# wdc3iii/legged_gym_dev

Hardware: AMD Instinct MI355X
Metric: env-steps/sec (whole node), ANYmal-C flat 4096 envs per GPU (higher is better)
Workload: dtype f32

## Files before the change

### legged_gym_dev_amd/csrc/ppo_api.hip

```cpp
#include <cstdlib>
#include <cstring>
#include <string>
#include <vector>

#include "ppo_device.h"
#include "ppo_mlp_args.h"
#include "ppo_rnn.h"

void lg_set_error(const std::string &s);

extern "C" {
void ppok_gemm_fwd(const GemmArgs *g, int nz, hipStream_t s);
void ppok_gemm_dx(const GemmArgs *g, int nz, hipStream_t s);
void ppok_sync_planes(const PpoDev *P, hipStream_t s);
int ppok_mlp_fwd(const MlpArgs *g, const PpoDev *P, int mask, hipStream_t s);
int ppok_mlp_supported(const MlpArgs *g);
int64_t ppok_mlp_frag_elems(int K, int N);
void ppok_mlp_frag_build(const MlpArgs *g, hipStream_t s);
void ppok_gemm_dw(const GemmArgs *g, int nz, int splits, hipStream_t s);
void ppok_debug_set_xcd_remap(int v);
void ppok_act_sample(const PpoDev *P, const float *obs, const float *cobs, const float *mu, const float *val, int t,
                     int64_t cnt, int inject, hipStream_t s);
void ppok_process_step(const PpoDev *P, const float *rew, const uint8_t *dones, const uint8_t *tos, int t, hipStream_t s);
void ppok_gae(const PpoDev *P, const float *last_values, hipStream_t s);
void ppok_det_fold(const PpoDev *P, hipStream_t s);
void ppok_adv_normalize(const PpoDev *P, hipStream_t s);
void ppok_gather(const PpoDev *P, int mb, hipStream_t s);
void ppok_randperm(const PpoDev *P, int n, uint64_t update_idx, hipStream_t s);
void ppok_loss(const PpoDev *P, const float *mu, const float *v, float *dmu, float *dval, hipStream_t s);
int ppok_step(const PpoDev *P, int par, const PpoDev *G, int gather_mb, hipStream_t s);
size_t ppok_head_part_floats();
int ppok_head_fused(const PpoDev *P, int H3, const float *xa, const float *xc, float *dza, float *dzc, int64_t w_a, int64_t b_a,
                    int64_t w_c, int64_t b_c, int64_t b_prev_a, int64_t b_prev_c, hipStream_t s);
void ppok_lstm_fwd(const RnnStepArgs *a, int nz, hipStream_t s);
void ppok_lstm_bwd(const RnnBwdArgs *a, int nz, hipStream_t s);
void ppok_lstm_bias_grad(const PpoDev *P, const RnnBiasArgs *a, hipStream_t s);
void ppok_lstm_reset(float *h0, float *c0, float *h1, float *c1, const uint8_t *done, int N, int H, hipStream_t s);
}

struct Rnn {
    int H, mbs;
    int in_dim[2];
    int64_t w_ih[2], w_hh[2], b_ih[2], b_hh[2];
    float *h[2], *c[2];
    float *sv_h[2], *sv_c[2];
    float *tmp_h[2], *tmp_c[2];
    float *pg[2];
    float *hout[2], *cout[2], *hused[2], *cused[2], *dh[2];
    float *gates[2];
    float *dc[2];
};

struct Net {
    int nl;
    int dims[LG_PPO_MAX_LAYERS + 1];
    int64_t w_off[LG_PPO_MAX_LAYERS], b_off[LG_PPO_MAX_LAYERS];
    int64_t pl_off[LG_PPO_MAX_LAYERS];
    int pl_ld0;
    float *act[LG_PPO_MAX_LAYERS + 1];
    float *dz[LG_PPO_MAX_LAYERS + 1];
};

struct lg_comm;
struct lg_ctx;
extern "C" {
void lg_internal_defer_finalize(lg_ctx *c, int on);
hipStream_t lg_internal_stream(lg_ctx *c);
int lg_internal_finalize_pending(lg_ctx *c);
const DevParams *lg_internal_take_finalize(lg_ctx *c, int64_t *counter);
const DevParams *lg_internal_host_params(lg_ctx *c);
int lg_finalize(lg_ctx *c);
hipStream_t lg_comm_stream_(lg_comm *c);
hipEvent_t lg_comm_event_(lg_comm *c);
int lg_comm_group_allreduce_(lg_comm *c, float *const *bufs, const int64_t *counts, int n, hipStream_t s);
int lg_comm_allreduce_sum(lg_comm *c, float *buf, int64_t n, void *stream);
int lg_comm_broadcast(lg_comm *c, float *buf, int64_t n, int root, void *stream);
}

struct lg_ppo {
    lg_comm *comm;
    hipEvent_t ev_bucket;
    int comm_rc;
    int comm_timing;
    std::vector<hipEvent_t> comm_ev;
    size_t comm_ev_used;
    lg_ppo_cfg cfg;
    PpoDev dev;
    Net net[2];
    hipStream_t stream;
    hipStream_t side;
    hipEvent_t ev_dz, ev_side;
    int overlap;
    long long *det_buf;
    int act_code;
    int grads_dirty;
    lg_ctx *env;
    int pp_pending, pp_t, pp_use_tos;
    int params_dirty;
    int fused_act;
    MlpArgs mlp;
    int step, inject;
    int64_t act_count, update_count;
    int Mmax;
    std::vector<void *> allocs;
    int64_t perm_count;
    struct MbSet { float *obs, *critic_obs, *actions, *mu, *scalars; } mbset[2];
    int mb_cur, mb_ready, mb_last;
    lg_ppo_buffers pub;
    Rnn rnn;
};

template <typename T>
static bool palloc(lg_ppo *p, T **out, size_t n) {
    void *q = nullptr;
    size_t bytes = (n ? n : 1) * sizeof(T);
    if (hipMalloc(&q, bytes) != hipSuccess || hipMemset(q, 0, bytes) != hipSuccess) return false;
    p->allocs.push_back(q);
    *out = (T *)q;
    return true;
}
#define PA(ptr, n) do { if (!palloc(p, &(ptr), (n))) { lg_set_error("hipMalloc failed in lg_ppo_create"); lg_ppo_destroy(p); return -100; } } while (0)

static int launch_ok() {
    hipError_t e = hipGetLastError();
    if (e != hipSuccess) { lg_set_error(std::string("ppo kernel launch: ") + hipGetErrorString(e)); return -100; }
    return 0;
}

static void forward(lg_ppo *p, int M, const float *in0, const float *in1, int mask, int skip_head = 0, bool planes = false,
                    bool in_pad = false, hipStream_t on = nullptr, int l_begin = 0, int l_end = 1 << 30) {
    const hipStream_t fs = on ? on : p->stream;
    const float *in[2] = {in0, in1};
    const int in_ld[2] = {in_pad ? p->dev.Op : p->net[0].dims[0], in_pad ? p->dev.OCp : p->net[1].dims[0]};
    int sel[2], nz = 0;
    for (int z = 0; z < 2; ++z) if (mask & (1 << z)) sel[nz++] = z;
    const int nl = p->net[sel[0]].nl;
    for (int l = l_begin; l < nl - skip_head && l < l_end; ++l) {
        GemmArgs g;
        memset(&g, 0, sizeof(g));
        for (int k = 0; k < nz; ++k) {
            Net &n = p->net[sel[k]];
            g.A[k] = l == 0 ? in[sel[k]] : n.act[l];
            g.B[k] = p->dev.params + n.w_off[l];
            g.bias[k] = p->dev.params + n.b_off[l];
            g.Bpl[k] = planes ? p->dev.wpl + n.pl_off[l] : nullptr;
            g.C[k] = n.act[l + 1];
            g.M[k] = M; g.N[k] = n.dims[l + 1]; g.K[k] = n.dims[l];
            g.lda[k] = l == 0 ? in_ld[sel[k]] : n.dims[l]; g.ldb[k] = n.dims[l]; g.ldc[k] = n.dims[l + 1];
            if (l == 0 && in_pad && planes && n.pl_ld0 != n.dims[0]) { g.Kpl[k] = n.pl_ld0; g.ldbpl[k] = n.pl_ld0; }
            else if (l == 0 && n.pl_ld0 != n.dims[0]) g.Bpl[k] = nullptr;
        }
        g.elu = l < nl - 1 ? p->act_code : 0;
        g.pl_stride = p->dev.pl_stride;
        ppok_gemm_fwd(&g, nz, fs);
    }
}

static int bucket_extents(lg_ppo *p, int l, float **bufs, int64_t *counts) {
    int n = 0;
    for (int z = 0; z < 2; ++z) {
        Net &net = p->net[z];
        bufs[n] = p->dev.grads + net.w_off[l];
        counts[n++] = (int64_t)net.dims[l + 1] * net.dims[l] + net.dims[l + 1];
    }
    if (l == p->net[0].nl - 1) {
        bufs[n] = p->dev.grads + p->dev.off_std; counts[n++] = p->cfg.num_actions;
        bufs[n] = p->dev.grads + p->dev.num_params; counts[n++] = 2;
    }
    return n;
}
static void reduce_layer_bucket(lg_ppo *p, int l, hipStream_t ready_on) {
    float *bufs[4];
    int64_t counts[4];
    const int n = bucket_extents(p, l, bufs, counts);
    hipStream_t cs = lg_comm_stream_(p->comm);
    (void)hipEventRecord(p->ev_bucket, ready_on);
    (void)hipStreamWaitEvent(cs, p->ev_bucket, 0);
    const int rc = lg_comm_group_allreduce_(p->comm, bufs, counts, n, cs);
    if (rc && !p->comm_rc) p->comm_rc = rc;
}

static void backward(lg_ppo *p, int M, const float *in0, const float *in1, int skip_head = 0) {
    const float *in[2] = {in0, in1};
    auto det_args = [&](GemmArgs &g) {
        g.det_base = p->dev.grads; g.det64 = p->dev.det64; g.det_n = p->dev.num_params + 2;
    };
    const int nl = p->net[0].nl;
    for (int l = nl - 1 - skip_head; l >= 0; --l) {
        GemmArgs g;
        memset(&g, 0, sizeof(g));
        det_args(g);
        long tiles = 0;
        for (int z = 0; z < 2; ++z) {
            Net &n = p->net[z];
            g.A[z] = n.dz[l + 1]; g.lda[z] = n.dims[l + 1];
            g.B[z] = l == 0 ? in[z] : n.act[l]; g.ldb[z] = n.dims[l];
            g.C[z] = p->dev.grads + n.w_off[l]; g.ldc[z] = n.dims[l];
            g.M[z] = n.dims[l + 1]; g.N[z] = n.dims[l]; g.K[z] = M;
            if (l == 0 && !p->rnn.H) {
                const int ldp = z == 0 ? p->dev.Op : p->dev.OCp;
                g.ldb[z] = ldp;
                if (ldp != n.dims[0]) { g.N[z] = ldp; g.nstore[z] = n.dims[0]; }
            }
            const int tile = (g.M[z] > 64 && g.N[z] > 64) ? 128 : 64;
            long t = (long)((g.M[z] + tile - 1) / tile) * ((g.N[z] + tile - 1) / tile);
            tiles = t > tiles ? t : tiles;
        }
        constexpr int dw_target = 384;
        int splits = (int)((dw_target + tiles - 1) / tiles);
        int max_splits = M / 256 > 0 ? M / 256 : 1;
        if (splits > max_splits) splits = max_splits;
        if (splits >= 8) splits &= ~7;
        if (splits < 1) splits = 1;
        const bool on_side = p->overlap && l > 0;
        hipStream_t dw_stream = on_side ? p->side : p->stream;
        if (on_side) {
            (void)hipEventRecord(p->ev_dz, p->stream);
            (void)hipStreamWaitEvent(p->side, p->ev_dz, 0);
        }
        ppok_gemm_dw(&g, 2, splits, dw_stream);
        if (p->comm) reduce_layer_bucket(p, l, dw_stream);
        if (l > 0) {
            memset(&g, 0, sizeof(g));
            det_args(g);
            for (int z = 0; z < 2; ++z) {
                Net &n = p->net[z];
                g.A[z] = n.dz[l + 1]; g.lda[z] = n.dims[l + 1];
                g.B[z] = p->dev.params + n.w_off[l]; g.ldb[z] = n.dims[l];
                g.Bpl[z] = p->dev.wpl + n.pl_off[l];
                g.C[z] = n.dz[l]; g.ldc[z] = n.dims[l];
                g.aux[z] = n.act[l]; g.ldaux[z] = n.dims[l];
                g.colsum[z] = p->dev.grads + n.b_off[l - 1];
                g.M[z] = M; g.N[z] = n.dims[l]; g.K[z] = n.dims[l + 1];
            }
            g.elu = p->act_code;
            g.pl_stride = p->dev.pl_stride;
            ppok_gemm_dx(&g, 2, p->stream);
        }
    }
    if (p->rnn.H) {
        GemmArgs g;
        memset(&g, 0, sizeof(g));
        for (int z = 0; z < 2; ++z) {
            Net &n = p->net[z];
            g.A[z] = n.dz[1]; g.lda[z] = n.dims[1];
            g.B[z] = p->dev.params + n.w_off[0]; g.ldb[z] = n.dims[0];
            g.Bpl[z] = p->dev.wpl + n.pl_off[0];
            g.C[z] = p->rnn.dh[z]; g.ldc[z] = n.dims[0];
            g.aux[z] = p->rnn.dh[z]; g.ldaux[z] = n.dims[0];
            g.M[z] = M; g.N[z] = n.dims[0]; g.K[z] = n.dims[1];
        }
        g.elu = 0;
        g.pl_stride = p->dev.pl_stride;
        ppok_gemm_dx(&g, 2, p->stream);
    }
    if (p->overlap) {
        (void)hipEventRecord(p->ev_side, p->side);
        (void)hipStreamWaitEvent(p->stream, p->ev_side, 0);
    }
    if (p->comm) {
        const bool rec = p->comm_timing && p->comm_ev_used + 2 <= 2 * 4096;
        if (rec) {
            while (p->comm_ev.size() < p->comm_ev_used + 2) { hipEvent_t e; (void)hipEventCreate(&e); p->comm_ev.push_back(e); }
            (void)hipEventRecord(p->comm_ev[p->comm_ev_used], p->stream);
        }
        (void)hipEventRecord(lg_comm_event_(p->comm), lg_comm_stream_(p->comm));
        (void)hipStreamWaitEvent(p->stream, lg_comm_event_(p->comm), 0);
        if (rec) { (void)hipEventRecord(p->comm_ev[p->comm_ev_used + 1], p->stream); p->comm_ev_used += 2; }
    }
}

static void flush_rollout_epilogue(lg_ppo *p) {
    if (!p->env) return;
    (void)lg_finalize(p->env);
    if (p->pp_pending) {
        const lg_buffers &b = lg_internal_host_params(p->env)->buf;
        ppok_process_step(&p->dev, b.rew, b.reset, p->pp_use_tos ? b.extras_time_outs : nullptr, p->pp_t, p->stream);
        p->pp_pending = 0;
    }
}

static void rnn_net_params(lg_ppo *p, int z, RnnNetArgs &n) {
    const Rnn &q = p->rnn;
    n.Wih = p->dev.params + q.w_ih[z]; n.Whh = p->dev.params + q.w_hh[z];
    n.bih = p->dev.params + q.b_ih[z]; n.bhh = p->dev.params + q.b_hh[z];
}

static void rnn_live_step(lg_ppo *p, int mask, const float *x0, const float *x1, int t) {
    Rnn &q = p->rnn;
    const int N = p->cfg.num_envs, H = q.H;
    RnnStepArgs a;
    memset(&a, 0, sizeof(a));
    a.M = N; a.H = H; a.reload_all = 1;
    const float *x[2] = {x0, x1};
    int nz = 0;
    for (int z = 0; z < 2; ++z) {
        if (!(mask & (1 << z))) continue;
        RnnNetArgs &n = a.n[nz++];
        rnn_net_params(p, z, n);
        n.X = x[z]; n.ldx = q.in_dim[z]; n.K = q.in_dim[z];
        n.h_sv = t >= 0 ? q.sv_h[z] + (size_t)t * N * H : q.tmp_h[z];
        n.c_sv = t >= 0 ? q.sv_c[z] + (size_t)t * N * H : q.tmp_c[z];
        n.h_out = q.h[z]; n.c_out = q.c[z];
    }
    ppok_lstm_fwd(&a, nz, p->stream);
}

static void rnn_stash_live(lg_ppo *p, int mask, int t) {
    Rnn &q = p->rnn;
    const size_t nh = (size_t)p->cfg.num_envs * q.H;
    for (int z = 0; z < 2; ++z) {
        if (!(mask & (1 << z))) continue;
        float *dh = t >= 0 ? q.sv_h[z] + (size_t)t * nh : q.tmp_h[z];
        float *dc = t >= 0 ? q.sv_c[z] + (size_t)t * nh : q.tmp_c[z];
        (void)hipMemcpyAsync(dh, q.h[z], nh * sizeof(float), hipMemcpyDeviceToDevice, p->stream);
        (void)hipMemcpyAsync(dc, q.c[z], nh * sizeof(float), hipMemcpyDeviceToDevice, p->stream);
    }
}

static void rnn_forward_seq(lg_ppo *p, int mb) {
    Rnn &q = p->rnn;
    PpoDev &d = p->dev;
    const int T = d.T, N = d.N, mbs = q.mbs, H = q.H, R = d.mb_rows, e0 = mb * mbs;
    GemmArgs g;
    memset(&g, 0, sizeof(g));
    for (int z = 0; z < 2; ++z) {
        g.A[z] = z ? d.mb_critic_obs : d.mb_obs; g.lda[z] = z ? d.OCp : d.Op;
        g.B[z] = d.params + q.w_ih[z]; g.ldb[z] = q.in_dim[z];
        g.bias[z] = d.params + q.b_ih[z];
        g.C[z] = q.pg[z]; g.ldc[z] = 4 * H;
        g.M[z] = R; g.N[z] = 4 * H; g.K[z] = q.in_dim[z];
    }
    g.elu = 0;
    ppok_gemm_fwd(&g, 2, p->stream);
    for (int t = 0; t < T; ++t) {
        RnnStepArgs a;
        memset(&a, 0, sizeof(a));
        a.M = mbs; a.H = H;
        a.reload_all = t == 0;
        a.reload = t ? d.st_dones + (size_t)(t - 1) * N + e0 : nullptr;
        for (int z = 0; z < 2; ++z) {
            RnnNetArgs &n = a.n[z];
            rnn_net_params(p, z, n);
            const size_t r0 = (size_t)t * mbs, rp = (size_t)(t ? t - 1 : 0) * mbs;
            n.P = q.pg[z] + r0 * 4 * H; n.ldp = 4 * H;
            n.h_prev = t ? q.hout[z] + rp * H : nullptr; n.c_prev = t ? q.cout[z] + rp * H : nullptr;
            n.h_sv = q.sv_h[z] + ((size_t)t * N + e0) * H; n.c_sv = q.sv_c[z] + ((size_t)t * N + e0) * H;
            n.h_out = q.hout[z] + r0 * H; n.c_out = q.cout[z] + r0 * H;
            n.gates = q.gates[z] + r0 * 4 * H;
            n.h_used = q.hused[z] + r0 * H; n.c_used = q.cused[z] + r0 * H;
        }
        ppok_lstm_fwd(&a, 2, p->stream);
    }
}

static void rnn_backward_seq(lg_ppo *p, int mb) {
    Rnn &q = p->rnn;
    PpoDev &d = p->dev;
    const int T = d.T, N = d.N, mbs = q.mbs, H = q.H, R = d.mb_rows, e0 = mb * mbs;
    for (int z = 0; z < 2; ++z) (void)hipMemsetAsync(q.dc[z], 0, (size_t)mbs * H * sizeof(float), p->stream);
    for (int t = T - 1; t >= 0; --t) {
        RnnBwdArgs a;
        memset(&a, 0, sizeof(a));
        a.M = mbs; a.H = H;
        a.cut_next = t < T - 1 ? d.st_dones + (size_t)t * N + e0 : nullptr;
        a.cut = t ? d.st_dones + (size_t)(t - 1) * N + e0 : nullptr;
        a.cut_all = t == 0;
        for (int z = 0; z < 2; ++z) {
            RnnBwdNet &n = a.n[z];
            const size_t r0 = (size_t)t * mbs;
            n.dG_next = t < T - 1 ? q.pg[z] + (r0 + mbs) * 4 * H : nullptr;
            n.Whh = d.params + q.w_hh[z];
            n.dh_mlp = q.dh[z] + r0 * H;
            n.dc = q.dc[z];
            n.gates = q.gates[z] + r0 * 4 * H; n.c_t = q.cout[z] + r0 * H; n.c_used = q.cused[z] + r0 * H;
            n.dG = q.pg[z] + r0 * 4 * H;
        }
        ppok_lstm_bwd(&a, 2, p->stream);
    }
    for (int w = 0; w < 2; ++w) {
        GemmArgs g;
        memset(&g, 0, sizeof(g));
        g.det_base = d.grads; g.det64 = d.det64; g.det_n = d.num_params + 2;
        long tiles = 0;
        for (int z = 0; z < 2; ++z) {
            g.A[z] = q.pg[z]; g.lda[z] = 4 * H;
            g.M[z] = 4 * H; g.K[z] = R;
            if (w == 0) {
                const int ldp = z ? d.OCp : d.Op;
                g.B[z] = z ? d.mb_critic_obs : d.mb_obs; g.ldb[z] = ldp;
                g.C[z] = d.grads + q.w_ih[z]; g.ldc[z] = q.in_dim[z];
                g.N[z] = ldp;
                if (ldp != q.in_dim[z]) g.nstore[z] = q.in_dim[z];
            } else {
                g.B[z] = q.hused[z]; g.ldb[z] = H;
                g.C[z] = d.grads + q.w_hh[z]; g.ldc[z] = H;
                g.N[z] = H;
            }
            const int tile = (g.M[z] > 64 && g.N[z] > 64) ? 128 : 64;
            const long tz = (long)((g.M[z] + tile - 1) / tile) * ((g.N[z] + tile - 1) / tile);
            tiles = tz > tiles ? tz : tiles;
        }
        int splits = (int)((384 + tiles - 1) / tiles);
        const int max_splits = R / 256 > 0 ? R / 256 : 1;
        if (splits > max_splits) splits = max_splits;
        if (splits >= 8) splits &= ~7;
        if (splits < 1) splits = 1;
        ppok_gemm_dw(&g, 2, splits, p->stream);
    }
    RnnBiasArgs b;
    memset(&b, 0, sizeof(b));
    b.M = R; b.H = H;
    for (int z = 0; z < 2; ++z) { b.dG[z] = q.pg[z]; b.db_ih[z] = d.grads + q.b_ih[z]; b.db_hh[z] = d.grads + q.b_hh[z]; }
    ppok_lstm_bias_grad(&d, &b, p->stream);
}

extern "C" {

int lg_ppo_destroy(lg_ppo *p) {
    if (!p) return 0;
    if (p->env) { flush_rollout_epilogue(p); lg_internal_defer_finalize(p->env, 0); p->env = nullptr; }
    if (p->side) { (void)hipStreamSynchronize(p->side); (void)hipStreamDestroy(p->side); }
    if (p->ev_dz) (void)hipEventDestroy(p->ev_dz);
    if (p->ev_side) (void)hipEventDestroy(p->ev_side);
    if (p->ev_bucket) (void)hipEventDestroy(p->ev_bucket);
    for (hipEvent_t e : p->comm_ev) (void)hipEventDestroy(e);
    for (void *q : p->allocs) (void)hipFree(q);
    delete p;
    return 0;
}

static int ppo_create(const lg_ppo_cfg *cfg, const lg_ppo_rnn_cfg *rc, lg_ppo **out) {
    if (!cfg || !out) { lg_set_error("null argument"); return -1; }
    int ndev = 0;
    if (hipGetDeviceCount(&ndev) != hipSuccess || ndev == 0) { lg_set_error("no HIP device: no CPU fallback"); return -2; }
    if (cfg->activation < 0 || cfg->activation > 5) { lg_set_error("activation must be one of 0 elu, 1 selu, 2 relu (also rsl_rl's crelu), 3 lrelu, 4 tanh, 5 sigmoid"); return -3; }
    if (cfg->num_hidden < 1 || cfg->num_hidden > LG_MAX_HIDDEN || cfg->num_actions > LG_PPO_MAX_A) {
        lg_set_error("unsupported network size"); return -4;
    }
    const int N = cfg->num_envs, T = cfg->num_steps, A = cfg->num_actions, O = cfg->num_obs;
    const int OC = cfg->num_critic_obs > 0 ? cfg->num_critic_obs : O;
    if ((long)N * T % cfg->num_mini_batches != 0 && (long)N * T / cfg->num_mini_batches == 0) { lg_set_error("bad minibatch count"); return -5; }
    const int H = rc ? rc->hidden : 0;
    if (rc) {
        if (rc->type != 0) { lg_set_error("recurrent policy: only rnn_type 'lstm' (0) is implemented"); return -6; }
        if (rc->layers != 1) { lg_set_error("recurrent policy: only rnn_num_layers = 1 is implemented"); return -6; }
        if (H < 32 || H > 512 || H % 32) { lg_set_error("recurrent policy: rnn_hidden_size must be a multiple of 32 in [32, 512]"); return -6; }
    }
    lg_ppo *p = new lg_ppo();
    p->cfg = *cfg;
    memset(&p->rnn, 0, sizeof(p->rnn));
    p->stream = nullptr;
    p->act_code = cfg->activation + 1;
    p->fused_act = getenv("LG_FUSED_ACT") ? atoi(getenv("LG_FUSED_ACT")) : 1;
    p->overlap = getenv("LG_PPO_OVERLAP") ? atoi(getenv("LG_PPO_OVERLAP")) : 1;
    if (hipStreamCreateWithFlags(&p->side, hipStreamNonBlocking) != hipSuccess ||
        hipEventCreateWithFlags(&p->ev_dz, hipEventDisableTiming) != hipSuccess ||
        hipEventCreateWithFlags(&p->ev_side, hipEventDisableTiming) != hipSuccess ||
        hipEventCreateWithFlags(&p->ev_bucket, hipEventDisableTiming) != hipSuccess) {
        lg_set_error("stream/event creation failed"); delete p; return -100;
    }
    p->step = 0; p->inject = 0; p->act_count = 0; p->update_count = 0; p->params_dirty = 1;
    p->comm = nullptr; p->comm_rc = 0; p->comm_timing = 0; p->comm_ev_used = 0;
    p->env = nullptr; p->pp_pending = 0;
    if (getenv("LG_XCD_REMAP")) ppok_debug_set_xcd_remap(atoi(getenv("LG_XCD_REMAP")));
    p->perm_count = 0;
    const int R = (int)((long)N * T / cfg->num_mini_batches);
    p->Mmax = R > N ? R : N;

    int64_t off = 0;
    PpoDev &d = p->dev;
    memset(&d, 0, sizeof(d));
    d.off_std = (int)off; off += A;
    for (int z = 0; z < 2; ++z) {
        Net &n = p->net[z];
        n.nl = cfg->num_hidden + 1;
        n.dims[0] = H ? H : z == 0 ? O : OC;
        for (int l = 0; l < cfg->num_hidden; ++l) n.dims[l + 1] = z == 0 ? cfg->actor_hidden[l] : cfg->critic_hidden[l];
        n.dims[n.nl] = z == 0 ? A : 1;
        for (int l = 0; l < n.nl; ++l) {
            n.w_off[l] = off; off += (int64_t)n.dims[l + 1] * n.dims[l];
            n.b_off[l] = off; off += n.dims[l + 1];
        }
    }
    if (H) {
        Rnn &q = p->rnn;
        q.H = H; q.mbs = N / cfg->num_mini_batches;
        for (int z = 0; z < 2; ++z) {
            q.in_dim[z] = z == 0 ? O : OC;
            q.w_ih[z] = off; off += (int64_t)4 * H * q.in_dim[z];
            q.w_hh[z] = off; off += (int64_t)4 * H * H;
            q.b_ih[z] = off; off += 4 * H;
            q.b_hh[z] = off; off += 4 * H;
        }
        p->fused_act = 0;
    }
    d.num_params = off;
    int seg_ld[LG_PPO_MAX_SEG];
    {
        int64_t po = 0;
        d.nseg = 0;
        for (int z = 0; z < 2; ++z)
            for (int l = 0; l < p->net[z].nl; ++l) {
                Net &n = p->net[z];
                n.pl_off[l] = po;
                d.seg_off[d.nseg] = n.w_off[l]; d.seg_pl[d.nseg] = po;
                d.seg_rows[d.nseg] = n.dims[l + 1]; d.seg_cols[d.nseg] = n.dims[l];
                const int ld = l == 0 ? (n.dims[0] + 31) / 32 * 32 : n.dims[l];
                if (l == 0) n.pl_ld0 = ld;
                seg_ld[d.nseg] = ld;
                ++d.nseg;
                po += ((int64_t)n.dims[l + 1] * ld + 7) / 8 * 8;
            }
        d.pl_stride = po;
    }
    d.off_bias_actor_head = (int)p->net[0].b_off[p->net[0].nl - 1];
    d.off_bias_critic_head = (int)p->net[1].b_off[p->net[1].nl - 1];
    d.N = N; d.T = T; d.A = A; d.O = O; d.OC = OC; d.mb_rows = R;
    d.Op = (O + 31) / 32 * 32; d.OCp = (OC + 31) / 32 * 32;
    d.world = cfg->world_size > 0 ? cfg->world_size : 1;
    d.env_offset = 0;
    d.adaptive = cfg->adaptive_schedule; d.clipped_value = cfg->use_clipped_value_loss;
    d.seed = cfg->seed;
    d.gamma = cfg->gamma; d.lam = cfg->lam; d.clip = cfg->clip_param; d.value_coef = cfg->value_loss_coef;
    d.entropy_coef = cfg->entropy_coef; d.desired_kl = cfg->desired_kl; d.max_grad_norm = cfg->max_grad_norm;

    PA(d.params, off + 2); PA(d.grads, off + 2); PA(d.adam_m, off + 2); PA(d.adam_v, off + 2);
    {
        const int64_t pls = d.pl_stride;
        PA(d.wpl, (size_t)3 * pls + 8);
        PA(d.pl_dest, (size_t)off + 2);
        std::vector<int32_t> dest((size_t)off + 2, -1);
        for (int sg = 0; sg < d.nseg; ++sg)
            for (int64_t e = 0; e < (int64_t)d.seg_rows[sg] * d.seg_cols[sg]; ++e)
                dest[d.seg_off[sg] + e] = (int32_t)(d.seg_pl[sg] + (e / d.seg_cols[sg]) * seg_ld[sg] + e % d.seg_cols[sg]);
        (void)hipMemcpy(d.pl_dest, dest.data(), dest.size() * sizeof(int32_t), hipMemcpyHostToDevice);
    }
    const size_t TN = (size_t)T * N;
    PA(d.st_obs, TN * O);
    if (cfg->num_critic_obs > 0) PA(d.st_critic_obs, TN * OC); else d.st_critic_obs = d.st_obs;
    PA(d.st_actions, TN * A); PA(d.st_rewards, TN); PA(d.st_values, TN); PA(d.st_returns, TN); PA(d.st_adv, TN);
    PA(d.st_log_prob, TN); PA(d.st_mu, TN * A); PA(d.st_sigma, A); PA(d.st_dones, TN);
    PA(d.act_actions, (size_t)N * A); PA(d.act_values, N); PA(d.act_log_prob, N); PA(d.act_mu, (size_t)N * A);
    PA(d.stats, 8); PA(d.loss_acc, 4); PA(d.noise, (size_t)N * A); PA(d.perm, TN); PA(d.adv_partial, 4);
    for (int k = 0; k < 2; ++k) {
        lg_ppo::MbSet &m = p->mbset[k];
        PA(m.obs, (size_t)R * d.Op);
        if (cfg->num_critic_obs > 0) PA(m.critic_obs, (size_t)R * d.OCp); else m.critic_obs = m.obs;
        PA(m.actions, (size_t)R * A); PA(m.mu, (size_t)R * A); PA(m.scalars, (size_t)R * 4);
    }
    p->mb_cur = 0; p->mb_ready = -1; p->mb_last = -1;
    d.mb_obs = p->mbset[0].obs; d.mb_critic_obs = p->mbset[0].critic_obs; d.mb_actions = p->mbset[0].actions;
    d.mb_mu = p->mbset[0].mu; d.mb_scalars = p->mbset[0].scalars;
    PA(d.head_part, ppok_head_part_floats());
    PA(d.cur_reward_sum, N); PA(d.cur_episode_len, N); PA(d.ep_stats, 4); PA(d.ep_ring, 200); PA(d.ep_ring_count, 1);
    for (int z = 0; z < 2; ++z) {
        Net &n = p->net[z];
        n.act[0] = nullptr; n.dz[0] = nullptr;
        for (int l = 1; l <= n.nl; ++l) { PA(n.act[l], (size_t)p->Mmax * n.dims[l]); PA(n.dz[l], (size_t)p->Mmax * n.dims[l]); }
    }
    if (H) {
        Rnn &q = p->rnn;
        const size_t NH = (size_t)N * H, Rr = (size_t)R;
        for (int z = 0; z < 2; ++z) {
            PA(q.h[z], NH); PA(q.c[z], NH); PA(q.sv_h[z], TN * H); PA(q.sv_c[z], TN * H); PA(q.tmp_h[z], NH); PA(q.tmp_c[z], NH);
            PA(q.pg[z], Rr * 4 * H); PA(q.gates[z], Rr * 4 * H);
            PA(q.hout[z], Rr * H); PA(q.cout[z], Rr * H); PA(q.hused[z], Rr * H); PA(q.cused[z], Rr * H); PA(q.dh[z], Rr * H);
            PA(q.dc[z], (size_t)q.mbs * H);
        }
        std::vector<int32_t> perm(TN);
        for (int mb = 0; N % cfg->num_mini_batches == 0 && mb < cfg->num_mini_batches; ++mb)
            for (int t = 0; t < T; ++t)
                for (int e = 0; e < q.mbs; ++e) perm[(size_t)mb * R + (size_t)t * q.mbs + e] = (int32_t)((size_t)t * N + (size_t)mb * q.mbs + e);
        (void)hipMemcpy(d.perm, perm.data(), TN * sizeof(int32_t), hipMemcpyHostToDevice);
    }
    if (p->fused_act) {
        MlpArgs &g = p->mlp;
        memset(&g, 0, sizeof(g));
        g.params = d.params; g.M = N; g.nl = p->net[0].nl; g.act = p->act_code;
        int64_t tot = 0;
        if (p->net[0].nl != p->net[1].nl) p->fused_act = 0;
        for (int z = 0; z < 2 && p->fused_act; ++z) {
            Net &n = p->net[z];
            for (int l = 0; l <= n.nl; ++l) g.dims[z][l] = n.dims[l];
            for (int l = 0; l < n.nl; ++l) {
                g.w_off[z][l] = n.w_off[l]; g.b_off[z][l] = n.b_off[l]; g.frag_off[z][l] = tot;
                tot += ppok_mlp_frag_elems(n.dims[l], n.dims[l + 1]);
            }
        }
        if (p->fused_act && ppok_mlp_supported(&g) != 0) p->fused_act = 0;
        if (p->fused_act) { uint16_t *wf = nullptr; PA(wf, (size_t)tot); g.wfrag = wf; }
    }
    {
        std::vector<float> h(A, cfg->init_noise_std);
        (void)hipMemcpy(d.params + d.off_std, h.data(), sizeof(float) * A, hipMemcpyHostToDevice);
        float lr = cfg->learning_rate;
        (void)hipMemcpy(d.stats, &lr, sizeof(float), hipMemcpyHostToDevice);
    }
    lg_ppo_buffers &b = p->pub;
    memset(&b, 0, sizeof(b));
    b.params = d.params; b.grads = d.grads; b.adam_m = d.adam_m; b.adam_v = d.adam_v;
    b.obs = d.st_obs; b.critic_obs = d.st_critic_obs; b.actions = d.st_actions; b.rewards = d.st_rewards;
    b.values = d.st_values; b.returns = d.st_returns; b.advantages = d.st_adv; b.log_prob = d.st_log_prob;
    b.mu = d.st_mu; b.sigma = d.st_sigma; b.dones = d.st_dones;
    b.act_actions = d.act_actions; b.act_values = d.act_values; b.act_log_prob = d.act_log_prob; b.act_mu = d.act_mu;
    b.stats = d.stats; b.noise = d.noise; b.perm = d.perm; b.adv_partial = d.adv_partial;
    b.cur_reward_sum = d.cur_reward_sum; b.cur_episode_len = d.cur_episode_len; b.ep_stats = d.ep_stats;
    b.ep_ring = d.ep_ring; b.ep_ring_count = d.ep_ring_count;
    b.num_params = off; b.num_reduce = off + 2;
    if (hipDeviceSynchronize() != hipSuccess) { lg_set_error("device sync failed in lg_ppo_create"); lg_ppo_destroy(p); return -100; }
    *out = p;
    return 0;
}

int lg_ppo_create(const lg_ppo_cfg *cfg, lg_ppo **out) { return ppo_create(cfg, nullptr, out); }
int lg_ppo_create_recurrent(const lg_ppo_cfg *cfg, const lg_ppo_rnn_cfg *rnn, lg_ppo **out) {
    if (!rnn) { lg_set_error("null argument"); return -1; }
    return ppo_create(cfg, rnn, out);
}
int lg_ppo_get_rnn_buffers(lg_ppo *p, lg_ppo_rnn_buffers *out) {
    if (!p->rnn.H) { lg_set_error("lg_ppo_get_rnn_buffers: not a recurrent learner"); return -15; }
    for (int z = 0; z < 2; ++z) {
        out->h[z] = p->rnn.h[z]; out->c[z] = p->rnn.c[z]; out->saved_h[z] = p->rnn.sv_h[z]; out->saved_c[z] = p->rnn.sv_c[z];
    }
    out->hidden = p->rnn.H;
    return 0;
}
int lg_ppo_reset_hidden(lg_ppo *p, const uint8_t *dones) {
    if (!p->rnn.H) { lg_set_error("lg_ppo_reset_hidden: not a recurrent learner"); return -15; }
    flush_rollout_epilogue(p);
    const Rnn &q = p->rnn;
    ppok_lstm_reset(q.h[0], q.c[0], q.h[1], q.c[1], dones, p->cfg.num_envs, q.H, p->stream);
    return launch_ok();
}
int lg_ppo_get_buffers(lg_ppo *p, lg_ppo_buffers *out) { *out = p->pub; return 0; }
int lg_ppo_set_stream(lg_ppo *p, void *s) { p->stream = (hipStream_t)s; return 0; }
int lg_ppo_inject_noise(lg_ppo *p, int enable) { p->inject = enable; return 0; }
int lg_ppo_debug_set_overlap(lg_ppo *p, int v) { p->overlap = v; return 0; }
int lg_ppo_debug_set_fused_act(lg_ppo *p, int v) { p->fused_act = v && p->mlp.wfrag; return 0; }
int lg_ppo_debug_get_fused_act(lg_ppo *p) { return p->fused_act; }
int lg_ppo_debug_set_act_count(lg_ppo *p, long long v) { p->act_count = v; return 0; }

int lg_ppo_param_layout(lg_ppo *p, int64_t *offsets, int64_t *shapes, int max_entries) {
    int k = 0;
    auto put = [&](int64_t o, int64_t r, int64_t c) {
        if (k < max_entries) { offsets[k] = o; shapes[2 * k] = r; shapes[2 * k + 1] = c; }
        ++k;
    };
    put(p->dev.off_std, p->cfg.num_actions, 0);
    for (int z = 0; z < 2; ++z)
        for (int l = 0; l < p->net[z].nl; ++l) {
            put(p->net[z].w_off[l], p->net[z].dims[l + 1], p->net[z].dims[l]);
            put(p->net[z].b_off[l], p->net[z].dims[l + 1], 0);
        }
    const Rnn &q = p->rnn;
    for (int z = 0; q.H && z < 2; ++z) {
        put(q.w_ih[z], 4 * q.H, q.in_dim[z]);
        put(q.w_hh[z], 4 * q.H, q.H);
        put(q.b_ih[z], 4 * q.H, 0);
        put(q.b_hh[z], 4 * q.H, 0);
    }
    return k;
}

int lg_ppo_attach_env(lg_ppo *p, lg_ctx *env) {
    flush_rollout_epilogue(p);
    if (p->env) lg_internal_defer_finalize(p->env, 0);
    p->env = nullptr;
    if (env) {
        if (lg_internal_host_params(env)->cfg.num_envs != p->cfg.num_envs) { lg_set_error("lg_ppo_attach_env: env and learner differ in num_envs"); return -12; }
        if (lg_internal_stream(env) != p->stream) { lg_set_error("lg_ppo_attach_env: env and learner must run on the same stream (lg_set_stream / lg_ppo_set_stream)"); return -12; }
        p->env = env;
        lg_internal_defer_finalize(env, 1);
    }
    return launch_ok();
}

int lg_ppo_act(lg_ppo *p, const float *obs, const float *critic_obs) {
    if (p->step >= p->cfg.num_steps) { lg_set_error("Rollout buffer overflow"); return -10; }
    const float *cobs = critic_obs ? critic_obs : obs;
    int fused = -1;
    const bool dirty = p->params_dirty != 0 || p->step == 0;
    if (p->fused_act) {
        MlpArgs &g = p->mlp;
        g.in[0] = obs; g.in[1] = cobs;
        g.out[0] = p->net[0].act[p->net[0].nl]; g.out[1] = p->net[1].act[p->net[1].nl];
        if (dirty) ppok_mlp_frag_build(&g, p->stream);
        g.sample = 1; g.t = p->step; g.inject = p->inject; g.act_count = p->act_count;
        g.pp = 0;
        const int N = p->cfg.num_envs;
        const bool fits = (N + 255) / 256 + 1 <= (N + 31) / 32;
        if (p->env && p->pp_pending && fits) {
            g.pp = lg_internal_finalize_pending(p->env) ? 2 : 1;
            g.pp_t = p->pp_t; g.pp_use_tos = p->pp_use_tos;
            g.pp_env = lg_internal_take_finalize(p->env, &g.pp_counter);
            p->pp_pending = 0;
        } else flush_rollout_epilogue(p);
        fused = ppok_mlp_fwd(&g, &p->dev, 3, p->stream);
        if (fused != 0 && g.pp) { lg_set_error("fused act launch refused with a rollout epilogue attached"); return -13; }
        if (fused == 0) {
            p->act_count++;
            const int rc = launch_ok();
            if (rc == 0) p->params_dirty = 0;
            return rc;
        }
    }
    if (!p->fused_act) flush_rollout_epilogue(p);
    if (fused != 0) {
        if (dirty) ppok_sync_planes(&p->dev, p->stream);
        const float *in0 = obs, *in1 = cobs;
        if (p->rnn.H) {
            rnn_stash_live(p, 3, p->step);
            rnn_live_step(p, 3, obs, cobs, p->step);
            in0 = p->rnn.h[0]; in1 = p->rnn.h[1];
        }
        forward(p, p->cfg.num_envs, in0, in1, 3, 0, true);
    }
    ppok_act_sample(&p->dev, obs, cobs, p->net[0].act[p->net[0].nl], p->net[1].act[p->net[1].nl], p->step, p->act_count,
                    p->inject, p->stream);
    p->act_count++;
    const int rc = launch_ok();
    if (rc == 0) p->params_dirty = 0;
    return rc;
}

int lg_ppo_process_env_step(lg_ppo *p, const float *rew, const uint8_t *dones, const uint8_t *time_outs) {
    if (p->step >= p->cfg.num_steps) { lg_set_error("Rollout buffer overflow"); return -10; }
    if (p->env) {
        const lg_buffers &b = lg_internal_host_params(p->env)->buf;
        if (p->fused_act && !p->pp_pending && rew == b.rew && dones == b.reset && (!time_outs || time_outs == b.extras_time_outs)) {
            p->pp_pending = 1; p->pp_t = p->step; p->pp_use_tos = time_outs != nullptr;
            p->step++;
            return 0;
        }
        flush_rollout_epilogue(p);
    }
    ppok_process_step(&p->dev, rew, dones, time_outs, p->step, p->stream);
    if (p->rnn.H) ppok_lstm_reset(p->rnn.h[0], p->rnn.c[0], p->rnn.h[1], p->rnn.c[1], dones, p->cfg.num_envs, p->rnn.H, p->stream);
    p->step++;
    return launch_ok();
}

int lg_ppo_compute_returns(lg_ppo *p, const float *last_critic_obs) {
    flush_rollout_epilogue(p);
    if (p->rnn.H) {
        rnn_stash_live(p, 2, -1);
        rnn_live_step(p, 2, nullptr, last_critic_obs, -1);
        forward(p, p->cfg.num_envs, nullptr, p->rnn.h[1], 2);
    } else
        forward(p, p->cfg.num_envs, nullptr, last_critic_obs, 2);
    ppok_gae(&p->dev, p->net[1].act[p->net[1].nl], p->stream);
    return launch_ok();
}

int lg_ppo_normalize_advantages(lg_ppo *p) {
    ppok_adv_normalize(&p->dev, p->stream);
    return launch_ok();
}

static int rnn_update_refused(const lg_ppo *p) {
    if (!p->rnn.H || p->cfg.num_envs % p->cfg.num_mini_batches == 0) return 0;
    lg_set_error("recurrent policy: the update needs num_envs to be a multiple of num_mini_batches (its minibatches are whole envs)");
    return 1;
}

int lg_ppo_begin_update(lg_ppo *p) {
    if (rnn_update_refused(p)) return -6;
    flush_rollout_epilogue(p);
    const size_t n = (size_t)p->dev.mb_rows * p->cfg.num_mini_batches;
    if (!p->rnn.H) ppok_randperm(&p->dev, (int)n, (uint64_t)p->perm_count++, p->stream);
    p->mb_ready = -1;
    (void)hipMemsetAsync(p->dev.stats + 2, 0, 2 * sizeof(float), p->stream);
    (void)hipMemsetAsync(p->dev.stats + 5, 0, sizeof(float), p->stream);
    (void)hipMemsetAsync(p->dev.loss_acc, 0, 4 * sizeof(float), p->stream);
    p->grads_dirty = 1;
    ppok_sync_planes(&p->dev, p->stream);
    return launch_ok();
}

int lg_ppo_minibatch_backward(lg_ppo *p, int epoch, int mb) {
    (void)epoch;
    if (rnn_update_refused(p)) return -6;
    PpoDev &d = p->dev;
    const int R = d.mb_rows;
    if (p->grads_dirty) (void)hipMemsetAsync(d.grads, 0, (size_t)(d.num_params + 2) * sizeof(float), p->stream);
    p->grads_dirty = 1;
    auto use_set = [&](PpoDev &dev, int k) {
        const lg_ppo::MbSet &m = p->mbset[k];
        dev.mb_obs = m.obs; dev.mb_critic_obs = m.critic_obs; dev.mb_actions = m.actions; dev.mb_mu = m.mu; dev.mb_scalars = m.scalars;
    };
    if (p->mb_ready == mb) {
        p->mb_cur ^= 1;
        use_set(d, p->mb_cur);
    } else {
        ppok_gather(&d, mb, p->stream);
    }
    p->mb_ready = -1;
    p->mb_last = mb;
    Net &na = p->net[0], &nc = p->net[1];
    const int nl = na.nl, H3 = na.dims[nl - 1];
    const bool fuse = p->act_code == 1 && nl >= 2 && nc.dims[nl - 1] == H3 && (H3 == 128 || H3 == 64 || H3 == 32);
    if (p->rnn.H) {
        rnn_forward_seq(p, mb);
        forward(p, R, p->rnn.hout[0], p->rnn.hout[1], 3, fuse ? 1 : 0, true, false);
    } else
        forward(p, R, d.mb_obs, d.mb_critic_obs, 3, fuse ? 1 : 0, true, true);
    if (fuse) {
        ppok_head_fused(&d, H3, na.act[nl - 1], nc.act[nl - 1], na.dz[nl - 1], nc.dz[nl - 1], na.w_off[nl - 1], na.b_off[nl - 1],
                        nc.w_off[nl - 1], nc.b_off[nl - 1], na.b_off[nl - 2], nc.b_off[nl - 2], p->stream);
    } else {
        ppok_loss(&d, na.act[na.nl], nc.act[nc.nl], na.dz[na.nl], nc.dz[nc.nl], p->stream);
    }
    if (fuse && p->comm) reduce_layer_bucket(p, nl - 1, p->stream);
    if (p->rnn.H) {
        backward(p, R, p->rnn.hout[0], p->rnn.hout[1], fuse ? 1 : 0);
        rnn_backward_seq(p, mb);
    } else
        backward(p, R, d.mb_obs, d.mb_critic_obs, fuse ? 1 : 0);
    if (d.det64) ppok_det_fold(&d, p->stream);
    if (p->comm_rc) { const int rc = p->comm_rc; p->comm_rc = 0; return rc; }
    return launch_ok();
}

int lg_ppo_minibatch_step(lg_ppo *p) {
    int next = -1;
    PpoDev other = p->dev;
    if (p->cfg.num_mini_batches > 1 && p->mb_last >= 0) {
        next = (p->mb_last + 1) % p->cfg.num_mini_batches;
        const lg_ppo::MbSet &m = p->mbset[p->mb_cur ^ 1];
        other.mb_obs = m.obs; other.mb_critic_obs = m.critic_obs; other.mb_actions = m.actions; other.mb_mu = m.mu; other.mb_scalars = m.scalars;
    }
    if (ppok_step(&p->dev, (int)(p->update_count & 1), &other, next, p->stream)) p->mb_ready = next;
    p->mb_last = -1;
    p->grads_dirty = 0;
    p->params_dirty = 1;
    p->update_count++;
    return launch_ok();
}

int lg_ppo_end_update(lg_ppo *p) { p->step = 0; return 0; }

int lg_ppo_set_comm(lg_ppo *p, lg_comm *c) {
    if (c && p->rnn.H) { lg_set_error("lg_ppo_set_comm: the per-layer gradient buckets do not cover the LSTM of a recurrent learner; reduce the whole gradient buffer between lg_ppo_minibatch_backward and lg_ppo_minibatch_step instead"); return -14; }
    if (c && p->dev.det64) { lg_set_error("gradient buckets inside the backward pass cannot be combined with deterministic mode"); return -14; }
    p->comm = c;
    return 0;
}
int lg_ppo_comm_timing(lg_ppo *p, int enable) { p->comm_timing = enable ? 1 : 0; return 0; }
int lg_ppo_comm_wait_ms(lg_ppo *p, double *ms_total, int64_t *minibatches) {
    if (!ms_total || !minibatches) { lg_set_error("null argument"); return -1; }
    (void)hipStreamSynchronize(p->stream);
    double sum = 0.0;
    for (size_t k = 0; k + 1 < p->comm_ev_used; k += 2) {
        float ms = 0.f;
        if (hipEventElapsedTime(&ms, p->comm_ev[k], p->comm_ev[k + 1]) == hipSuccess) sum += ms;
    }
    *ms_total = sum; *minibatches = (int64_t)(p->comm_ev_used / 2);
    p->comm_ev_used = 0;
    return 0;
}
int lg_ppo_allreduce_adv_moments(lg_ppo *p, lg_comm *c) { return lg_comm_allreduce_sum(c, p->dev.adv_partial, 4, p->stream); }
int lg_ppo_broadcast_params(lg_ppo *p, lg_comm *c, int root) {
    p->params_dirty = 1;
    return lg_comm_broadcast(c, p->dev.params, p->dev.num_params + 2, root, p->stream);
}
int lg_ppo_params_changed(lg_ppo *p) { p->params_dirty = 1; return 0; }

int lg_ppo_set_deterministic(lg_ppo *p, int on) {
    if (on && p->comm) { lg_set_error("deterministic mode cannot be combined with gradient buckets reduced inside the backward pass (lg_ppo_set_comm)"); return -14; }
    if (on && !p->det_buf) {
        const size_t n = (size_t)p->dev.num_params + 10;
        void *q = nullptr;
        if (hipMalloc(&q, n * sizeof(long long)) != hipSuccess || hipMemset(q, 0, n * sizeof(long long)) != hipSuccess) {
            lg_set_error("hipMalloc failed in lg_ppo_set_deterministic"); return -100;
        }
        p->allocs.push_back(q);
        p->det_buf = (long long *)q;
    }
    if (!on && p->dev.det64) ppok_det_fold(&p->dev, p->stream);
    p->dev.det64 = on ? p->det_buf : nullptr;
    return launch_ok();
}

int lg_ppo_debug_bucket_extents(lg_ppo *p, int l, int64_t *offsets, int64_t *counts) {
    if (l < 0 || l >= p->net[0].nl) return -1;
    float *bufs[4];
    const int n = bucket_extents(p, l, bufs, counts);
    for (int k = 0; k < n; ++k) offsets[k] = bufs[k] - p->dev.grads;
    return n;
}

int lg_ppo_act_inference(lg_ppo *p, const float *obs, float *actions_out, int64_t rows) {
    if (rows > p->Mmax) { lg_set_error("too many rows for act_inference"); return -11; }
    if (p->rnn.H) {
        if (rows != p->cfg.num_envs) { lg_set_error("act_inference of a recurrent learner takes exactly num_envs rows"); return -11; }
        rnn_stash_live(p, 1, -1);
        rnn_live_step(p, 1, obs, nullptr, -1);
        obs = p->rnn.h[0];
    }
    forward(p, (int)rows, obs, nullptr, 1);
    Net &na = p->net[0];
    if (hipMemcpyAsync(actions_out, na.act[na.nl], (size_t)rows * p->cfg.num_actions * sizeof(float), hipMemcpyDeviceToDevice,
                       p->stream) != hipSuccess) { lg_set_error("copy failed"); return -100; }
    return launch_ok();
}

}
```

### legged_gym_dev_amd/csrc/ppo_device.h

```cpp
#pragma once
#include "lg_device.h"

#define LG_PPO_MAX_A 16
#define LG_PPO_MAX_LAYERS (LG_MAX_HIDDEN + 1)

struct GemmArgs {
    const float *A[2], *B[2], *bias[2], *aux[2];
    float *C[2], *colsum[2];
    int M[2], N[2], K[2], lda[2], ldb[2], ldc[2], ldaux[2];
    int elu;
    const uint16_t *Bpl[2];
    int64_t pl_stride;
    int Kpl[2], ldbpl[2];
    int nstore[2];
    const float *det_base;
    long long *det64;
    int64_t det_n;
};

#define LG_PPO_MAX_SEG (2 * LG_PPO_MAX_LAYERS)

struct PpoDev {
    int N, T, A, O, OC, mb_rows, world, env_offset;
    int adaptive, clipped_value;
    uint64_t seed;
    float gamma, lam, clip, value_coef, entropy_coef, desired_kl, max_grad_norm;
    int64_t num_params;
    int off_std, off_bias_actor_head, off_bias_critic_head;
    float *params, *grads, *adam_m, *adam_v;
    float *st_obs, *st_critic_obs, *st_actions, *st_rewards, *st_values, *st_returns, *st_adv, *st_log_prob, *st_mu, *st_sigma;
    uint8_t *st_dones;
    float *act_actions, *act_values, *act_log_prob, *act_mu;
    float *stats;
    float *loss_acc;
    float *noise;
    int32_t *perm;
    float *adv_partial;
    float *mb_obs, *mb_critic_obs, *mb_actions, *mb_mu, *mb_scalars;
    int Op, OCp;
    float *cur_reward_sum, *cur_episode_len, *ep_stats, *ep_ring;
    int32_t *ep_ring_count;
    float *head_part;
    uint16_t *wpl;
    int32_t *pl_dest;
    int64_t pl_stride;
    int nseg;
    int64_t seg_off[LG_PPO_MAX_SEG], seg_pl[LG_PPO_MAX_SEG];
    int seg_rows[LG_PPO_MAX_SEG], seg_cols[LG_PPO_MAX_SEG];
    long long *det64;
};

#define LG_DET_SCALE 1099511627776.0
__device__ __forceinline__ void det_add64(long long *q, float v) {
    atomicAdd(reinterpret_cast<unsigned long long *>(q), (unsigned long long)__double2ll_rn((double)v * LG_DET_SCALE));
}
__device__ __forceinline__ void acc_add(const PpoDev &P, float *p, float v) {
    if (!P.det64) { atomicAdd(p, v); return; }
    long long i;
    if (p >= P.grads && p < P.grads + P.num_params + 2) i = p - P.grads;
    else if (p >= P.loss_acc && p < P.loss_acc + 4) i = P.num_params + 2 + (p - P.loss_acc);
    else i = P.num_params + 6 + (p - P.adv_partial);
    det_add64(P.det64 + i, v);
}
__device__ __forceinline__ void acc_add(const GemmArgs &g, float *p, float v) {
    if (g.det64 && p >= g.det_base && p < g.det_base + g.det_n) det_add64(g.det64 + (p - g.det_base), v);
    else atomicAdd(p, v);
}

__device__ __forceinline__ void process_step_body(const PpoDev &P, float rew, bool done, bool to, int t, int i) {
    float r = rew;
    r += P.gamma * (P.st_values[(size_t)t * P.N + i] * (to ? 1.0f : 0.0f));
    P.st_rewards[(size_t)t * P.N + i] = r;
    P.st_dones[(size_t)t * P.N + i] = done ? 1 : 0;
    const float cr = P.cur_reward_sum[i] + rew, cl = P.cur_episode_len[i] + 1.0f;
    if (done) {
        atomicAdd(&P.ep_stats[0], cr);
        atomicAdd(&P.ep_stats[1], cl);
        atomicAdd(&P.ep_stats[2], 1.0f);
        const int slot = (int)((unsigned)atomicAdd(P.ep_ring_count, 1) % 100u);
        P.ep_ring[slot] = cr;
        P.ep_ring[100 + slot] = cl;
        P.cur_reward_sum[i] = 0.f;
        P.cur_episode_len[i] = 0.f;
    } else {
        P.cur_reward_sum[i] = cr;
        P.cur_episode_len[i] = cl;
    }
}

__device__ __forceinline__ float philox_normal(uint64_t seed, uint32_t env, uint64_t step, uint32_t a) {
    uint32_t c[4] = {env, (uint32_t)step, a, 0x5eedu};
    philox4x32((uint32_t)seed, (uint32_t)(seed >> 32), c);
    float u1 = ((float)(c[0] >> 8) + 1.0f) * (1.0f / 16777216.0f);
    float u2 = (float)(c[1] >> 8) * (1.0f / 16777216.0f);
    return sqrtf(-2.0f * logf(u1)) * cosf(6.283185307179586f * u2);
}
```

### legged_gym_dev_amd/csrc/ppo_kernels.hip

```cpp
#include <cstdlib>
#include <cstring>
#include <type_traits>

#include "ppo_device.h"

typedef float f32x16 __attribute__((ext_vector_type(16)));

#define SELU_L 1.0507009873554804934193349852946f
#define SELU_LA (1.0507009873554804934193349852946f * 1.6732632423543772848170429916717f)
__device__ __forceinline__ float act_fwd(int code, float v) {
    switch (code) {
    case 1: return v > 0.f ? v : __expf(v) - 1.0f;
    case 2: return v > 0.f ? SELU_L * v : SELU_LA * (__expf(v) - 1.0f);
    case 3: return fmaxf(v, 0.f);
    case 4: return v > 0.f ? v : 0.01f * v;
    case 5: return 2.0f * __frcp_rn(1.0f + __expf(-2.0f * v)) - 1.0f;
    case 6: return __frcp_rn(1.0f + __expf(-v));
    default: return v;
    }
}
__device__ __forceinline__ float act_bwd(int code, float a) {
    switch (code) {
    case 1: return a > 0.f ? 1.0f : a + 1.0f;
    case 2: return a > 0.f ? SELU_L : a + SELU_LA;
    case 3: return a > 0.f ? 1.0f : 0.f;
    case 4: return a > 0.f ? 1.0f : 0.01f;
    case 5: return 1.0f - a * a;
    case 6: return a * (1.0f - a);
    default: return 1.0f;
    }
}

static __device__ int g_xcd_remap = 1;
__device__ __forceinline__ void xcd_tile(int lin, int inner, int outer, int &o, int &i) {
    if (g_xcd_remap && (outer & 7) == 0) {
        const int c = lin & 7, j = lin >> 3;
        o = c + 8 * (j / inner);
        i = j % inner;
    } else {
        o = lin / inner;
        i = lin % inner;
    }
}

#define BK 32

template <bool RC, int ROWS, bool VEC, bool KSEQ = false, int NT = 256, bool FULL = false>
__device__ __forceinline__ void stage_load(const float *__restrict__ src, int ld, int row0, int red0, int nrows, int nred,
                                           float4 (&regs)[ROWS * BK / 4 / NT], unsigned &mask) {
    constexpr int NV = ROWS * BK / 4 / NT;
    const int tid = threadIdx.x & (NT - 1);
    const int row_lim = RC ? nrows : nred, col_lim = RC ? nred : nrows;
    mask = 0u;
#pragma unroll
    for (int v = 0; v < NV; ++v) {
        const int idx = tid + v * NT;
        int r, c;
        if (RC) { c = idx & (BK / 4 - 1); r = idx / (BK / 4); }
        else if (KSEQ) { c = tid & (ROWS / 4 - 1); r = NV * (tid / (ROWS / 4)) + v; }
        else { c = idx & (ROWS / 4 - 1); r = idx / (ROWS / 4); }
        const int grow = RC ? row0 + r : red0 + r;
        const int gcol = RC ? red0 + 4 * c : row0 + 4 * c;
        if (FULL) {
            regs[v] = *reinterpret_cast<const float4 *>(src + (size_t)grow * ld + gcol);
            mask = ~0u;
        } else if (VEC) {
            const int rc_ = min(grow, row_lim - 1), cc_ = min(gcol, col_lim - 4);
            regs[v] = *reinterpret_cast<const float4 *>(src + (size_t)rc_ * ld + cc_);
            mask |= (grow < row_lim && gcol < col_lim) ? (1u << v) : 0u;
        } else {
            const int rc_ = min(grow, row_lim - 1);
            const float *p = src + (size_t)rc_ * ld;
            const bool rin = grow < row_lim;
            float e[4];
#pragma unroll
            for (int q = 0; q < 4; ++q) {
                const int cc_ = min(gcol + q, col_lim - 1);
                const float x = p[cc_];
                e[q] = (rin && gcol + q < col_lim) ? x : 0.f;
            }
            regs[v] = make_float4(e[0], e[1], e[2], e[3]);
            mask |= 1u << v;
        }
    }
}
template <bool RC, int ROWS>
__device__ __forceinline__ void stage_store(float *__restrict__ lds, const float4 (&regs_in)[ROWS * BK / 4 / 256], unsigned mask) {
    constexpr int NV = ROWS * BK / 4 / 256;
    const int tid = threadIdx.x;
#pragma unroll
    for (int v = 0; v < NV; ++v) {
        int idx = tid + v * 256;
        const bool in = (mask >> v) & 1u;
        float4 regs[1];
        regs[0] = make_float4(in ? regs_in[v].x : 0.f, in ? regs_in[v].y : 0.f, in ? regs_in[v].z : 0.f, in ? regs_in[v].w : 0.f);
        if (RC) {
            int c = idx & (BK / 4 - 1), r = idx / (BK / 4);
            float *d = lds + r * (BK + 1) + 4 * c;
            d[0] = regs[0].x; d[1] = regs[0].y; d[2] = regs[0].z; d[3] = regs[0].w;
        } else {
            int c = idx & (ROWS / 4 - 1), r = idx / (ROWS / 4);
            *reinterpret_cast<float4 *>(lds + r * (ROWS + 4) + 4 * c) = regs[0];
        }
    }
}
template <bool RC, int ROWS>
__device__ __forceinline__ float frag(const float *__restrict__ lds, int row, int k) {
    return RC ? lds[row * (BK + 1) + k] : lds[k * (ROWS + 4) + row];
}
template <bool RC, int ROWS>
constexpr int tile_floats() { return RC ? ROWS * (BK + 1) : BK * (ROWS + 4); }

template <bool A_RC, bool B_RC, int TM, int TN, bool VEC, bool DBUF>
__device__ __forceinline__ void gemm_mainloop(const float *__restrict__ A, const float *__restrict__ B, int lda, int ldb, int m0, int n0,
                                              int M, int N, int k_begin, int k_end, float *__restrict__ lds, int wm, int wn, int li, int lk,
                                              f32x16 (&acc)[TM][TN]) {
    constexpr int BM = 64 * TM, BN = 64 * TN;
    constexpr int AF = tile_floats<A_RC, BM>(), BF = tile_floats<B_RC, BN>();
    float4 ra[BM * BK / 4 / 256], rb[BN * BK / 4 / 256];
    unsigned ma, mb_;
    stage_load<A_RC, BM, VEC>(A, lda, m0, k_begin, M, k_end, ra, ma);
    stage_load<B_RC, BN, VEC>(B, ldb, n0, k_begin, N, k_end, rb, mb_);
    stage_store<A_RC, BM>(lds, ra, ma);
    stage_store<B_RC, BN>(lds + AF, rb, mb_);
    __syncthreads();
    int cur = 0;
    for (int k0 = k_begin; k0 < k_end; k0 += BK) {
        const bool more = k0 + BK < k_end;
        if (more) {
            stage_load<A_RC, BM, VEC>(A, lda, m0, k0 + BK, M, k_end, ra, ma);
            stage_load<B_RC, BN, VEC>(B, ldb, n0, k0 + BK, N, k_end, rb, mb_);
        }
        const float *as = lds + (DBUF ? cur : 0) * (AF + BF), *bs = as + AF;
        constexpr int GS = 4, NG = BK / 2 / GS;
        float av[2][GS][TM], bv[2][GS][TN];
#pragma unroll
        for (int s = 0; s < GS; ++s) {
#pragma unroll
            for (int a = 0; a < TM; ++a) av[0][s][a] = frag<A_RC, BM>(as, wm + 32 * a + li, 2 * s + lk);
#pragma unroll
            for (int b = 0; b < TN; ++b) bv[0][s][b] = frag<B_RC, BN>(bs, wn + 32 * b + li, 2 * s + lk);
        }
#pragma unroll
        for (int gq = 0; gq < NG; ++gq) {
            if (gq + 1 < NG) {
#pragma unroll
                for (int s = 0; s < GS; ++s) {
                    const int ks = 2 * ((gq + 1) * GS + s) + lk;
#pragma unroll
                    for (int a = 0; a < TM; ++a) av[(gq + 1) & 1][s][a] = frag<A_RC, BM>(as, wm + 32 * a + li, ks);
#pragma unroll
                    for (int b = 0; b < TN; ++b) bv[(gq + 1) & 1][s][b] = frag<B_RC, BN>(bs, wn + 32 * b + li, ks);
                }
            }
#pragma unroll
            for (int s = 0; s < GS; ++s)
#pragma unroll
                for (int a = 0; a < TM; ++a)
#pragma unroll
                    for (int b = 0; b < TN; ++b)
                        acc[a][b] = __builtin_amdgcn_mfma_f32_32x32x2f32(av[gq & 1][s][a], bv[gq & 1][s][b], acc[a][b], 0, 0, 0);
        }
        if (!DBUF) __syncthreads();
        if (more) {
            stage_store<A_RC, BM>(lds + (DBUF ? (cur ^ 1) : 0) * (AF + BF), ra, ma);
            stage_store<B_RC, BN>(lds + (DBUF ? (cur ^ 1) : 0) * (AF + BF) + AF, rb, mb_);
        }
        __syncthreads();
        cur ^= 1;
    }

}


typedef __bf16 bf16x8 __attribute__((ext_vector_type(8)));
#define X6_ROWB 80
__device__ __forceinline__ void lds_barrier() { asm volatile("s_waitcnt lgkmcnt(0)\n\ts_barrier" ::: "memory"); }

__device__ __forceinline__ uint32_t cvt_pk_bf16(float a, float b) {
    uint32_t r;
    asm("v_cvt_pk_bf16_f32 %0, %1, %2" : "=v"(r) : "v"(a), "v"(b));
    return r;
}
__device__ __forceinline__ void split2(float x0, float x1, uint32_t &h, uint32_t &m, uint32_t &l) {
    typedef float f32x2 __attribute__((ext_vector_type(2)));
    h = cvt_pk_bf16(x0, x1);
    f32x2 r = f32x2{x0, x1} - f32x2{__uint_as_float(h << 16), __uint_as_float(h & 0xffff0000u)};
    m = cvt_pk_bf16(r.x, r.y);
    r -= f32x2{__uint_as_float(m << 16), __uint_as_float(m & 0xffff0000u)};
    l = cvt_pk_bf16(r.x, r.y);
}
template <int ROWS>
__device__ __forceinline__ int x6_prow(int r) { return (r & 3) * (ROWS / 4 + 4) + (r >> 2); }
template <int ROWS>
constexpr int x6_plane_bytes() { return (ROWS + 16) * X6_ROWB; }

template <bool RC, int ROWS, int NT, bool FULL = false>
__device__ __forceinline__ void stage_store_x6(unsigned char *__restrict__ lds, const float4 (&regs)[ROWS * BK / 4 / NT], unsigned mask) {
    constexpr int NV = ROWS * BK / 4 / NT;
    constexpr int PL = x6_plane_bytes<ROWS>();
    const int tid = threadIdx.x & (NT - 1);
    if constexpr (RC) {
#pragma unroll
        for (int v = 0; v < NV; ++v) {
            const int idx = tid + v * NT;
            const int c = idx & (BK / 4 - 1), r = idx / (BK / 4);
            const bool in = FULL || ((mask >> v) & 1u);
            const float x0 = in ? regs[v].x : 0.f, x1 = in ? regs[v].y : 0.f, x2 = in ? regs[v].z : 0.f, x3 = in ? regs[v].w : 0.f;
            uint32_t h0, m0, l0, h1, m1, l1;
            split2(x0, x1, h0, m0, l0);
            split2(x2, x3, h1, m1, l1);
            unsigned char *d = lds + x6_prow<ROWS>(r) * X6_ROWB + 8 * c;
            *reinterpret_cast<uint2 *>(d) = make_uint2(h0, h1);
            *reinterpret_cast<uint2 *>(d + PL) = make_uint2(m0, m1);
            *reinterpret_cast<uint2 *>(d + 2 * PL) = make_uint2(l0, l1);
        }
    } else {
        const int c = tid & (ROWS / 4 - 1), kg = tid / (ROWS / 4);
        float e[4][NV];
#pragma unroll
        for (int v = 0; v < NV; ++v) {
            const bool in = FULL || ((mask >> v) & 1u);
            e[0][v] = in ? regs[v].x : 0.f; e[1][v] = in ? regs[v].y : 0.f;
            e[2][v] = in ? regs[v].z : 0.f; e[3][v] = in ? regs[v].w : 0.f;
        }
#pragma unroll
        for (int q = 0; q < 4; ++q) {
            unsigned char *d = lds + (q * (ROWS / 4 + 4) + c) * X6_ROWB + 2 * NV * kg;
            if (NV == 4) {
                uint32_t h0, m0, l0, h1, m1, l1;
                split2(e[q][0], e[q][1], h0, m0, l0);
                split2(e[q][2 % NV], e[q][3 % NV], h1, m1, l1);
                *reinterpret_cast<uint2 *>(d) = make_uint2(h0, h1);
                *reinterpret_cast<uint2 *>(d + PL) = make_uint2(m0, m1);
                *reinterpret_cast<uint2 *>(d + 2 * PL) = make_uint2(l0, l1);
            } else {
                static_assert(NV == 4 || NV == 2, "tile/threads combination");
                uint32_t h0, m0, l0;
                split2(e[q][0], e[q][1 % NV], h0, m0, l0);
                *reinterpret_cast<uint32_t *>(d) = h0;
                *reinterpret_cast<uint32_t *>(d + PL) = m0;
                *reinterpret_cast<uint32_t *>(d + 2 * PL) = l0;
            }
        }
    }
}

template <int ROWS, int NT>
__device__ __forceinline__ void stage_load_pl(const uint16_t *__restrict__ src, int64_t pl_stride, int ld, int row0, int red0, int nrows,
                                              int nred, uint4 (&regs)[ROWS * 12 / NT], unsigned &mask) {
    constexpr int NV = ROWS * 12 / NT;
    mask = 0u;
#pragma unroll
    for (int v = 0; v < NV; ++v) {
        const int c = (threadIdx.x & (NT - 1)) + v * NT;
        const int pl = c / (ROWS * 4), r = (c >> 2) % ROWS, q = c & 3;
        const int grow = row0 + r, gk = red0 + 8 * q;
        const int rc_ = min(grow, nrows - 1), kc_ = min(gk, nred - 8);
        regs[v] = *reinterpret_cast<const uint4 *>(src + pl * pl_stride + (size_t)rc_ * ld + kc_);
        mask |= (grow < nrows && gk < nred) ? (1u << v) : 0u;
    }
}
template <int ROWS, int NT>
__device__ __forceinline__ void stage_store_pl(unsigned char *__restrict__ lds, const uint4 (&regs)[ROWS * 12 / NT], unsigned mask) {
    constexpr int NV = ROWS * 12 / NT;
    constexpr int PL = x6_plane_bytes<ROWS>();
#pragma unroll
    for (int v = 0; v < NV; ++v) {
        const int c = (threadIdx.x & (NT - 1)) + v * NT;
        const int pl = c / (ROWS * 4), r = (c >> 2) % ROWS, q = c & 3;
        const bool in = (mask >> v) & 1u;
        const uint4 x = in ? regs[v] : make_uint4(0u, 0u, 0u, 0u);
        *reinterpret_cast<uint4 *>(lds + pl * PL + x6_prow<ROWS>(r) * X6_ROWB + 16 * q) = x;
    }
}

constexpr int PLT_SUB = 576;
typedef short s16x4 __attribute__((ext_vector_type(4)));
template <int BN>
__device__ __forceinline__ int plt_off(int row, int ch) {
    return (BN / 32 * PLT_SUB) * (row >> 3) + PLT_SUB * (ch >> 2) + 64 * (row & 7) + 16 * ((ch & 3) ^ ((row >> 2) & 3));
}
template <int BN>
constexpr int plt_plane_bytes() { return BK / 8 * (BN / 32) * PLT_SUB; }

template <int BN, int NT>
__device__ __forceinline__ void stage_load_plt(const uint16_t *__restrict__ src, int64_t pl_stride, int ld, int n0, int red0, int ncols,
                                               int nred, uint4 (&regs)[BK * BN / 8 * 3 / NT], unsigned &mask) {
    constexpr int CPR = BN / 8, NV = BK * CPR * 3 / NT;
    mask = 0u;
#pragma unroll
    for (int v = 0; v < NV; ++v) {
        const int c = (threadIdx.x & (NT - 1)) + v * NT;
        const int pl = c / (BK * CPR), k = (c / CPR) % BK, ch = c % CPR;
        const int gk = red0 + k, gn = n0 + 8 * ch;
        const int kc_ = min(gk, nred - 1), nc_ = min(gn, ncols - 8);
        regs[v] = *reinterpret_cast<const uint4 *>(src + pl * pl_stride + (size_t)kc_ * ld + nc_);
        mask |= (gk < nred && gn < ncols) ? (1u << v) : 0u;
    }
}
template <int BN, int NT>
__device__ __forceinline__ void stage_store_plt(unsigned char *__restrict__ lds, const uint4 (&regs)[BK * BN / 8 * 3 / NT], unsigned mask) {
    constexpr int CPR = BN / 8, NV = BK * CPR * 3 / NT;
#pragma unroll
    for (int v = 0; v < NV; ++v) {
        const int c = (threadIdx.x & (NT - 1)) + v * NT;
        const int pl = c / (BK * CPR), k = (c / CPR) % BK, ch = c % CPR;
        const bool in = (mask >> v) & 1u;
        const uint4 x = in ? regs[v] : make_uint4(0u, 0u, 0u, 0u);
        *reinterpret_cast<uint4 *>(lds + pl * plt_plane_bytes<BN>() + plt_off<BN>(k, ch)) = x;
    }
}
__device__ __forceinline__ s16x4 lds_read_tr16(const unsigned char *p) {
    return __builtin_amdgcn_ds_read_tr16_b64_v4i16((s16x4 __attribute__((address_space(3))) *)p);
}

template <bool A_RC, bool B_RC, int TM, int TN, int WGM, int WGN, bool VEC, bool FULL = false, int B_PL = 0>
__device__ __forceinline__ void gemm_mainloop_x6(const float *__restrict__ A, const float *__restrict__ B, int lda, int ldb, int m0, int n0,
                                                 int M, int N, int k_begin, int k_end, unsigned char *__restrict__ lds, int wm, int wn, int li,
                                                 int lk, f32x16 (&acc)[TM][TN], const uint16_t *__restrict__ Bpl = nullptr,
                                                 int64_t pl_stride = 0) {
    constexpr int BM = 32 * TM * WGM, BN = 32 * TN * WGN, NT = 64 * WGM * WGN;
    constexpr int APL = x6_plane_bytes<BM>(), BPL = B_PL == 2 ? plt_plane_bytes<BN>() : x6_plane_bytes<BN>();
    constexpr int NVA = BM * BK / 4 / NT, NVB = BN * BK / 4 / NT;
    constexpr int PD = 2;
    constexpr int NVP = B_PL ? BN * 12 / NT : 1;
    struct Regs { float4 a[NVA], b[NVB]; uint4 p[NVP]; unsigned ma = 0, mb = 0; };
    Regs R[PD];
    unsigned char *lds_b = lds + 3 * APL;
    auto load_tile = [&](Regs &r, int k) {
        stage_load<A_RC, BM, VEC, true, NT, FULL>(A, lda, m0, k, M, k_end, r.a, r.ma);
        if constexpr (B_PL == 2) stage_load_plt<BN, NT>(Bpl, pl_stride, ldb, n0, k, N, k_end, r.p, r.mb);
        else if constexpr (B_PL == 1) stage_load_pl<BN, NT>(Bpl, pl_stride, ldb, n0, k, N, k_end, r.p, r.mb);
        else stage_load<B_RC, BN, VEC, true, NT, FULL>(B, ldb, n0, k, N, k_end, r.b, r.mb);
    };
    auto store_tile = [&](Regs &r) {
        stage_store_x6<A_RC, BM, NT, FULL>(lds, r.a, r.ma);
        if constexpr (B_PL == 2) stage_store_plt<BN, NT>(lds_b, r.p, r.mb);
        else if constexpr (B_PL == 1) stage_store_pl<BN, NT>(lds_b, r.p, r.mb);
        else stage_store_x6<B_RC, BN, NT, FULL>(lds_b, r.b, r.mb);
    };
    load_tile(R[0], k_begin);
#pragma unroll
    for (int d = 1; d < PD; ++d)
        if (k_begin + d * BK < k_end) load_tile(R[d], k_begin + d * BK);
    store_tile(R[0]);
    lds_barrier();
    const unsigned char *fa = lds + x6_prow<BM>(wm + li) * X6_ROWB + 16 * lk;
    const unsigned char *fb = lds_b + x6_prow<BN>(wn + li) * X6_ROWB + 16 * lk;
    const int tg = (threadIdx.x >> 4) & 3, tq = (threadIdx.x >> 2) & 3, tp = threadIdx.x & 3;
    const unsigned char *ft[2];
#pragma unroll
    for (int h = 0; h < 2; ++h)
        ft[h] = lds_b + (BN / 32 * PLT_SUB) * (tg >> 1) + PLT_SUB * (wn / 32) + 64 * (4 * h + tq) +
                16 * ((2 * (tg & 1) + (tp >> 1)) ^ (2 * (tg >> 1) + h)) + 8 * (tp & 1);
    auto read_b = [&](int b, int p, int s) -> bf16x8 {
        if constexpr (B_PL == 2) {
            const int o = PLT_SUB * b + p * BPL + (BN / 32 * PLT_SUB) * 2 * s;
            const s16x4 lo = lds_read_tr16(ft[0] + o), hi = lds_read_tr16(ft[1] + o);
            typedef short s16x8 __attribute__((ext_vector_type(8)));
            const s16x8 v = {lo[0], lo[1], lo[2], lo[3], hi[0], hi[1], hi[2], hi[3]};
            return __builtin_bit_cast(bf16x8, v);
        } else {
            return *reinterpret_cast<const bf16x8 *>(fb + b * 8 * X6_ROWB + p * BPL + s * 32);
        }
    };

    auto body = [&](int k0, Regs &x, Regs &y) {
        if (k0 + PD * BK < k_end) load_tile(y, k0 + PD * BK);
        bf16x8 av[2][TM][3], bv[2][TN][3];
#pragma unroll
        for (int a = 0; a < TM; ++a)
#pragma unroll
            for (int p = 0; p < 3; ++p) av[0][a][p] = *reinterpret_cast<const bf16x8 *>(fa + a * 8 * X6_ROWB + p * APL);
#pragma unroll
        for (int b = 0; b < TN; ++b)
#pragma unroll
            for (int p = 0; p < 3; ++p) bv[0][b][p] = read_b(b, p, 0);
#pragma unroll
        for (int s = 0; s < BK / 16; ++s) {
            if (s + 1 < BK / 16) {
#pragma unroll
                for (int a = 0; a < TM; ++a)
#pragma unroll
                    for (int p = 0; p < 3; ++p)
                        av[(s + 1) & 1][a][p] = *reinterpret_cast<const bf16x8 *>(fa + a * 8 * X6_ROWB + p * APL + (s + 1) * 32);
#pragma unroll
                for (int b = 0; b < TN; ++b)
#pragma unroll
                    for (int p = 0; p < 3; ++p)
                        bv[(s + 1) & 1][b][p] = read_b(b, p, s + 1);
            }
#pragma unroll
            for (int a = 0; a < TM; ++a)
#pragma unroll
                for (int b = 0; b < TN; ++b) {
                    const bf16x8 *x = av[s & 1][a], *y = bv[s & 1][b];
                    f32x16 c = acc[a][b];
                    c = __builtin_amdgcn_mfma_f32_32x32x16_bf16(x[1], y[1], c, 0, 0, 0);
                    c = __builtin_amdgcn_mfma_f32_32x32x16_bf16(x[0], y[2], c, 0, 0, 0);
                    c = __builtin_amdgcn_mfma_f32_32x32x16_bf16(x[2], y[0], c, 0, 0, 0);
                    c = __builtin_amdgcn_mfma_f32_32x32x16_bf16(x[0], y[1], c, 0, 0, 0);
                    c = __builtin_amdgcn_mfma_f32_32x32x16_bf16(x[1], y[0], c, 0, 0, 0);
                    c = __builtin_amdgcn_mfma_f32_32x32x16_bf16(x[0], y[0], c, 0, 0, 0);
                    acc[a][b] = c;
                }
        }
        lds_barrier();
        if (k0 + BK < k_end) store_tile(x);
        lds_barrier();
    };
    for (int k0 = k_begin; k0 < k_end; k0 += PD * BK) {
#pragma unroll
        for (int d = 0; d < PD; ++d)
            if (d == 0 || k0 + d * BK < k_end) body(k0 + d * BK, R[(d + 1) % PD], R[d]);
    }
}

template <int EPI, int TM, int TN, int BM, int BN, int ACT>
__device__ __forceinline__ void gemm_epilogue(const GemmArgs &g, int z, int M, int N, int m0, int n0, int wm, int wn, int li, int lk, int ldc,
                                              f32x16 (&acc)[TM][TN]) {
    float *__restrict__ C = g.C[z];
    const bool interior = (m0 + BM <= M) && (n0 + BN <= N);
    const int elu = g.elu;
    if (interior) {
#pragma unroll
        for (int b = 0; b < TN; ++b) {
            const int n = n0 + wn + 32 * b + li;
            float csum = 0.f;
            const float bias = (EPI == 0 && g.bias[z]) ? g.bias[z][n] : 0.f;
#pragma unroll
            for (int a = 0; a < TM; ++a) {
                const int mb = m0 + wm + 32 * a + 4 * lk;
                float aux[16];
                if (EPI == 1) {
#pragma unroll
                    for (int r = 0; r < 16; ++r)
                        aux[r] = g.aux[z][(size_t)(mb + (r & 3) + 8 * (r >> 2)) * g.ldaux[z] + n];
                }
#pragma unroll
                for (int r = 0; r < 16; ++r) {
                    float *cp = &C[(size_t)(mb + (r & 3) + 8 * (r >> 2)) * ldc + n];
                    float v = acc[a][b][r];
                    if (EPI == 0) {
                        v += bias;
                        v = (ACT == 1 ? (v > 0.f ? v : __expf(v) - 1.0f) : ACT == 0 ? v : act_fwd(elu, v));
                        *cp = v;
                    } else if (EPI == 1) {
                        v *= (ACT == 1 ? (aux[r] > 0.f ? 1.0f : aux[r] + 1.0f) : ACT == 0 ? 1.0f : act_bwd(elu, aux[r]));
                        *cp = v;
                        csum += v;
                    } else {
                        acc_add(g, cp, v);
                    }
                }
            }
            if (EPI == 1 && g.colsum[z]) {
                csum += __shfl_xor(csum, 32);
                if (lk == 0) acc_add(g, &g.colsum[z][n], csum);
            }
        }
        return;
    }
#pragma unroll
    for (int b = 0; b < TN; ++b) {
        const int n = n0 + wn + 32 * b + li;
        float csum = 0.f;
        const float bias = (EPI == 0 && g.bias[z] && n < N) ? g.bias[z][n] : 0.f;
#pragma unroll
        for (int a = 0; a < TM; ++a)
#pragma unroll
            for (int r = 0; r < 16; ++r) {
                const int m = m0 + wm + 32 * a + (r & 3) + 8 * (r >> 2) + 4 * lk;
                if (m < M && n < N) {
                    float v = acc[a][b][r];
                    if (EPI == 0) {
                        v += bias;
                        v = (ACT == 1 ? (v > 0.f ? v : __expf(v) - 1.0f) : ACT == 0 ? v : act_fwd(elu, v));
                        C[(size_t)m * ldc + n] = v;
                    } else if (EPI == 1) {
                        const float act = g.aux[z][(size_t)m * g.ldaux[z] + n];
                        v *= (ACT == 1 ? (act > 0.f ? 1.0f : act + 1.0f) : ACT == 0 ? 1.0f : act_bwd(elu, act));
                        C[(size_t)m * ldc + n] = v;
                        csum += v;
                    } else {
                        acc_add(g, &C[(size_t)m * ldc + n], v);
                    }
                }
            }
        if (EPI == 1 && g.colsum[z]) {
            csum += __shfl_xor(csum, 32);
            if (lk == 0 && n < N) acc_add(g, &g.colsum[z][n], csum);
        }
    }
}

template <bool A_RC, bool B_RC, int EPI, int TM, int TN, bool DBUF, bool X6 = false, int WGM = 2, int WGN = 2, int B_PL = 0>
__global__ void __launch_bounds__(64 * WGM * WGN, X6 ? (WGM * WGN == 8 ? 4 : 2) : 1) k_gemm(GemmArgs g) {
    static_assert(B_PL == 0 || (X6 && (B_PL == 1) == B_RC), "weight planes feed the split-bf16 mainloop: [n][k] planes as the reduction-"
                  "contiguous operand (1), the same planes read along their rows through the transposing LDS read (2)");
    constexpr int BM = 32 * TM * WGM, BN = 32 * TN * WGN;
    static_assert(X6 || (WGM == 2 && WGN == 2), "the fp32-input mainloop is written for 2x2 waves");
    const int z = blockIdx.z;
    const int M = g.M[z], N = g.N[z], K = g.K[z];
    const int tiles_n = (N + BN - 1) / BN, tiles_m = (M + BM - 1) / BM;
    if ((int)blockIdx.x >= tiles_n * tiles_m) return;
    int tm, tn;
    if (EPI == 2) { tm = blockIdx.x / tiles_n; tn = blockIdx.x % tiles_n; }
    else xcd_tile((int)blockIdx.x, tiles_n, tiles_m, tm, tn);
    const int m0 = tm * BM, n0 = tn * BN;
    int k_begin = 0, k_end = K;
    if (EPI == 2) {
        int per = ((K + gridDim.y - 1) / gridDim.y + BK - 1) / BK * BK;
        k_begin = blockIdx.y * per;
        k_end = min(K, k_begin + per);
        if (k_begin >= k_end) return;
    }
    const float *__restrict__ A = g.A[z];
    const float *__restrict__ B = g.B[z];
    const int lda = g.lda[z], ldb = g.ldb[z], ldc = g.ldc[z];
    const bool a_vec = (lda & 3) == 0 && ((uintptr_t)A & 15) == 0 && (((A_RC ? k_end : M) & 3) == 0) && (A_RC ? k_end : M) >= 4;
    const bool b_vec = (ldb & 3) == 0 && ((uintptr_t)B & 15) == 0 && (((B_RC ? k_end : N) & 3) == 0) && (B_RC ? k_end : N) >= 4;

    constexpr int AF = tile_floats<A_RC, BM>(), BF = tile_floats<B_RC, BN>();
    constexpr int LDS_BYTES = X6 ? 3 * (x6_plane_bytes<BM>() + (B_PL == 2 ? plt_plane_bytes<BN>() : x6_plane_bytes<BN>()))
                                 : (DBUF ? 2 : 1) * (AF + BF) * 4;
    __shared__ __attribute__((aligned(16))) unsigned char lds_raw[LDS_BYTES];
    float *lds = reinterpret_cast<float *>(lds_raw);

    const int wave = threadIdx.x >> 6, lane = threadIdx.x & 63;
    const int wm = (wave / WGN) * 32 * TM, wn = (wave % WGN) * 32 * TN;
    const int li = lane & 31, lk = lane >> 5;

    f32x16 acc[TM][TN];
#pragma unroll
    for (int a = 0; a < TM; ++a)
#pragma unroll
        for (int b = 0; b < TN; ++b)
#pragma unroll
            for (int r = 0; r < 16; ++r) acc[a][b][r] = 0.f;

    if (X6) {
        const bool full = a_vec && b_vec && m0 + BM <= M && n0 + BN <= N && ((k_end - k_begin) % BK) == 0;
        if (B_PL) {
            const bool fullp = a_vec && m0 + BM <= M && n0 + BN <= N && ((k_end - k_begin) % BK) == 0;
            if (fullp) gemm_mainloop_x6<A_RC, B_RC, TM, TN, WGM, WGN, true, true, B_PL>(A, B, lda, ldb, m0, n0, M, N, k_begin, k_end, lds_raw, wm, wn, li, lk, acc, g.Bpl[z], g.pl_stride);
            else if (a_vec) gemm_mainloop_x6<A_RC, B_RC, TM, TN, WGM, WGN, true, false, B_PL>(A, B, lda, ldb, m0, n0, M, N, k_begin, k_end, lds_raw, wm, wn, li, lk, acc, g.Bpl[z], g.pl_stride);
            else gemm_mainloop_x6<A_RC, B_RC, TM, TN, WGM, WGN, false, false, B_PL>(A, B, lda, ldb, m0, n0, M, N, k_begin, k_end, lds_raw, wm, wn, li, lk, acc, g.Bpl[z], g.pl_stride);
        } else
        if (full) gemm_mainloop_x6<A_RC, B_RC, TM, TN, WGM, WGN, true, true>(A, B, lda, ldb, m0, n0, M, N, k_begin, k_end, lds_raw, wm, wn, li, lk, acc);
        else if (a_vec && b_vec) gemm_mainloop_x6<A_RC, B_RC, TM, TN, WGM, WGN, true>(A, B, lda, ldb, m0, n0, M, N, k_begin, k_end, lds_raw, wm, wn, li, lk, acc);
        else gemm_mainloop_x6<A_RC, B_RC, TM, TN, WGM, WGN, false>(A, B, lda, ldb, m0, n0, M, N, k_begin, k_end, lds_raw, wm, wn, li, lk, acc);
    } else {
        if (a_vec && b_vec) gemm_mainloop<A_RC, B_RC, TM, TN, true, DBUF>(A, B, lda, ldb, m0, n0, M, N, k_begin, k_end, lds, wm, wn, li, lk, acc);
        else gemm_mainloop<A_RC, B_RC, TM, TN, false, DBUF>(A, B, lda, ldb, m0, n0, M, N, k_begin, k_end, lds, wm, wn, li, lk, acc);
    }

    if (EPI == 2 || g.elu == 1) gemm_epilogue<EPI, TM, TN, BM, BN, 1>(g, z, M, N, m0, n0, wm, wn, li, lk, ldc, acc);
    else if (g.elu == 0) gemm_epilogue<EPI, TM, TN, BM, BN, 0>(g, z, M, N, m0, n0, wm, wn, li, lk, ldc, acc);
    else gemm_epilogue<EPI, TM, TN, BM, BN, -1>(g, z, M, N, m0, n0, wm, wn, li, lk, ldc, acc);
}

template <int ROWS, int NT>
__device__ __forceinline__ void stage_store_x6t(unsigned char *__restrict__ lds, const float4 (&regs)[ROWS * BK / 4 / NT], unsigned mask) {
    constexpr int NV = ROWS * BK / 4 / NT, PL = plt_plane_bytes<ROWS>();
#pragma unroll
    for (int v = 0; v < NV; ++v) {
        const int idx = threadIdx.x + v * NT;
        const int c = idx & (ROWS / 4 - 1), r = idx / (ROWS / 4);
        const bool in = (mask >> v) & 1u;
        const float x0 = in ? regs[v].x : 0.f, x1 = in ? regs[v].y : 0.f, x2 = in ? regs[v].z : 0.f, x3 = in ? regs[v].w : 0.f;
        uint32_t h0, m0, l0, h1, m1, l1;
        split2(x0, x1, h0, m0, l0);
        split2(x2, x3, h1, m1, l1);
        unsigned char *d = lds + plt_off<ROWS>(r, c >> 1) + 8 * (c & 1);
        *reinterpret_cast<uint2 *>(d) = make_uint2(h0, h1);
        *reinterpret_cast<uint2 *>(d + PL) = make_uint2(m0, m1);
        *reinterpret_cast<uint2 *>(d + 2 * PL) = make_uint2(l0, l1);
    }
}

template <int TM, int TN, int WGM, int WGN, int PD = 2>
__global__ void __launch_bounds__(64 * WGM * WGN, WGM * WGN == 8 ? 4 : 2) k_gemm_dw_t(GemmArgs g) {
    constexpr int BM = 32 * TM * WGM, BN = 32 * TN * WGN, NT = 64 * WGM * WGN;
    constexpr int APL = plt_plane_bytes<BM>(), BPL = plt_plane_bytes<BN>();
    constexpr int NVA = BM * BK / 4 / NT, NVB = BN * BK / 4 / NT;
    const int z = blockIdx.z;
    const int M = g.M[z], N = g.N[z], K = g.K[z];
    const int tiles_n = (N + BN - 1) / BN, tiles_m = (M + BM - 1) / BM;
    if ((int)blockIdx.x >= tiles_n * tiles_m) return;
    int slice, tile;
    xcd_tile((int)(blockIdx.x + gridDim.x * blockIdx.y), (int)gridDim.x, (int)gridDim.y, slice, tile);
    const int m0 = (tile / tiles_n) * BM, n0 = (tile % tiles_n) * BN;
    const int per = ((K + gridDim.y - 1) / gridDim.y + BK - 1) / BK * BK;
    const int k_begin = slice * per, k_end = min(K, k_begin + per);
    if (k_begin >= k_end) return;
    const float *__restrict__ A = g.A[z];
    const float *__restrict__ B = g.B[z];
    const int lda = g.lda[z], ldb = g.ldb[z], ldc = g.ldc[z];
    __shared__ __attribute__((aligned(16))) unsigned char lds[3 * (APL + BPL)];
    unsigned char *lds_b = lds + 3 * APL;
    const int wave = threadIdx.x >> 6, lane = threadIdx.x & 63;
    const int wm = (wave / WGN) * 32 * TM, wn = (wave % WGN) * 32 * TN;
    const int li = lane & 31, lk = lane >> 5;
    f32x16 acc[TM][TN];
#pragma unroll
    for (int a = 0; a < TM; ++a)
#pragma unroll
        for (int b = 0; b < TN; ++b)
#pragma unroll
            for (int r = 0; r < 16; ++r) acc[a][b][r] = 0.f;
    const int tg = (threadIdx.x >> 4) & 3, tq = (threadIdx.x >> 2) & 3, tp = threadIdx.x & 3;
    const unsigned char *fa[2], *fb[2];
#pragma unroll
    for (int h = 0; h < 2; ++h) {
        const int lane_off = 64 * (4 * h + tq) + 16 * ((2 * (tg & 1) + (tp >> 1)) ^ (2 * (tg >> 1) + h)) + 8 * (tp & 1);
        fa[h] = lds + (BM / 32 * PLT_SUB) * (tg >> 1) + PLT_SUB * (wm / 32) + lane_off;
        fb[h] = lds_b + (BN / 32 * PLT_SUB) * (tg >> 1) + PLT_SUB * (wn / 32) + lane_off;
    }
    auto frag = [&](const unsigned char *const (&f)[2], int o) -> bf16x8 {
        const s16x4 lo = lds_read_tr16(f[0] + o), hi = lds_read_tr16(f[1] + o);
        typedef short s16x8 __attribute__((ext_vector_type(8)));
        const s16x8 v = {lo[0], lo[1], lo[2], lo[3], hi[0], hi[1], hi[2], hi[3]};
        return __builtin_bit_cast(bf16x8, v);
    };
    const bool a_vec = (lda & 3) == 0 && ((uintptr_t)A & 15) == 0 && (M & 3) == 0 && M >= 4;
    const bool b_vec = (ldb & 3) == 0 && ((uintptr_t)B & 15) == 0 && (N & 3) == 0 && N >= 4;
    auto run = [&](auto vec) {
        constexpr bool VEC = decltype(vec)::value;
        float4 ra[PD][NVA], rb[PD][NVB];
        unsigned ma[PD], mb[PD];
    #pragma unroll
        for (int d = 0; d < PD; ++d) { ma[d] = 0u; mb[d] = 0u; }
        auto load = [&](int k0, float4 (&xa)[NVA], float4 (&xb)[NVB], unsigned &xma, unsigned &xmb) {
            stage_load<false, BM, VEC, false, NT>(A, lda, m0, k0, M, k_end, xa, xma);
            stage_load<false, BN, VEC, false, NT>(B, ldb, n0, k0, N, k_end, xb, xmb);
        };
    #pragma unroll
        for (int d = 0; d < PD; ++d)
            if (d == 0 || k_begin + d * BK < k_end) load(k_begin + d * BK, ra[d], rb[d], ma[d], mb[d]);
        stage_store_x6t<BM, NT>(lds, ra[0], ma[0]);
        stage_store_x6t<BN, NT>(lds_b, rb[0], mb[0]);
        lds_barrier();
        auto body = [&](int k0, float4 (&ca)[NVA], float4 (&cb)[NVB], unsigned &cma, unsigned &cmb, float4 (&na)[NVA], float4 (&nb)[NVB],
                        unsigned &nma, unsigned &nmb) {
            if (k0 + PD * BK < k_end) load(k0 + PD * BK, ca, cb, cma, cmb);
    #pragma unroll
            for (int s = 0; s < BK / 16; ++s) {
                bf16x8 av[TM][3], bv[TN][3];
    #pragma unroll
                for (int a = 0; a < TM; ++a)
    #pragma unroll
                    for (int p = 0; p < 3; ++p) av[a][p] = frag(fa, PLT_SUB * a + p * APL + (BM / 32 * PLT_SUB) * 2 * s);
    #pragma unroll
                for (int b = 0; b < TN; ++b)
    #pragma unroll
                    for (int p = 0; p < 3; ++p) bv[b][p] = frag(fb, PLT_SUB * b + p * BPL + (BN / 32 * PLT_SUB) * 2 * s);
    #pragma unroll
                for (int a = 0; a < TM; ++a)
    #pragma unroll
                    for (int b = 0; b < TN; ++b) {
                        const bf16x8 *x = av[a], *y = bv[b];
                        f32x16 c = acc[a][b];
                        c = __builtin_amdgcn_mfma_f32_32x32x16_bf16(x[1], y[1], c, 0, 0, 0);
                        c = __builtin_amdgcn_mfma_f32_32x32x16_bf16(x[0], y[2], c, 0, 0, 0);
                        c = __builtin_amdgcn_mfma_f32_32x32x16_bf16(x[2], y[0], c, 0, 0, 0);
                        c = __builtin_amdgcn_mfma_f32_32x32x16_bf16(x[0], y[1], c, 0, 0, 0);
                        c = __builtin_amdgcn_mfma_f32_32x32x16_bf16(x[1], y[0], c, 0, 0, 0);
                        c = __builtin_amdgcn_mfma_f32_32x32x16_bf16(x[0], y[0], c, 0, 0, 0);
                        acc[a][b] = c;
                    }
            }
            lds_barrier();
            if (k0 + BK < k_end) {
                stage_store_x6t<BM, NT>(lds, na, nma);
                stage_store_x6t<BN, NT>(lds_b, nb, nmb);
            }
            lds_barrier();
        };
        for (int k0 = k_begin; k0 < k_end; k0 += PD * BK) {
    #pragma unroll
            for (int d = 0; d < PD; ++d)
                if (d == 0 || k0 + d * BK < k_end)
                    body(k0 + d * BK, ra[d], rb[d], ma[d], mb[d], ra[(d + 1) % PD], rb[(d + 1) % PD], ma[(d + 1) % PD], mb[(d + 1) % PD]);
        }
    };
    if (a_vec && b_vec) run(std::true_type{});
    else run(std::false_type{});
    gemm_epilogue<2, TM, TN, BM, BN, 1>(g, z, M, g.nstore[z] ? g.nstore[z] : N, m0, n0, wm, wn, li, lk, ldc, acc);
}

extern "C" void ppok_debug_set_xcd_remap(int v) { (void)hipMemcpyToSymbol(HIP_SYMBOL(g_xcd_remap), &v, sizeof(int)); }
static int g_gemm_x6 = 1;
extern "C" void ppok_debug_set_x6(int v) { g_gemm_x6 = v != 0; }

#include "ppo_gemm_glds.h"

template <int EPI, bool B_RC = true, int PL = 1>
static void launch_gemm_pl(const GemmArgs &g, int nz, hipStream_t s) {
    int maxM = 0, maxN = 0;
    for (int z = 0; z < nz; ++z) { maxM = g.M[z] > maxM ? g.M[z] : maxM; maxN = g.N[z] > maxN ? g.N[z] : maxN; }
    if constexpr (EPI == 0) {
        if (maxM > 64 && glds_ok<PL>(g, nz)) {
            dim3 grid((unsigned)(((maxM + GLDS_BM - 1) / GLDS_BM) * (maxN / GLDS_BN)), 1, nz);
            hipLaunchKernelGGL((k_gemm_glds<EPI, PL>), grid, dim3(256), 0, s, g);
            return;
        }
    }
    const long big_tiles = (long)((maxM + 127) / 128) * ((maxN + 127) / 128);
    if (big_tiles >= 192 && maxN > 64 && maxM > 64) {
        dim3 grid((unsigned)big_tiles, 1, nz);
        hipLaunchKernelGGL((k_gemm<true, B_RC, EPI, 2, 1, false, true, 2, 4, PL>), grid, dim3(512), 0, s, g);
    } else {
        dim3 grid((unsigned)(((maxM + 63) / 64) * ((maxN + 63) / 64)), 1, nz);
        hipLaunchKernelGGL((k_gemm<true, B_RC, EPI, 1, 1, false, true, 2, 2, PL>), grid, dim3(256), 0, s, g);
    }
}
static bool planes_ok(const GemmArgs &g, int nz) {
    if (!g_gemm_x6) return false;
    for (int z = 0; z < nz; ++z)
        if (!g.Bpl[z] || (g.ldb[z] & 7) || (g.K[z] & 7) || g.K[z] < 8 || ((uintptr_t)g.Bpl[z] & 15) || (g.pl_stride & 7)) return false;
    return true;
}

template <bool A_RC, bool B_RC, int EPI, bool X6>
static void launch_gemm(const GemmArgs &g, int nz, int splits, hipStream_t s) {
    int maxM = 0, maxN = 0;
    for (int z = 0; z < nz; ++z) { maxM = g.M[z] > maxM ? g.M[z] : maxM; maxN = g.N[z] > maxN ? g.N[z] : maxN; }
    const long big_tiles = (long)((maxM + 127) / 128) * ((maxN + 127) / 128);
    if (big_tiles * splits >= 192 && maxN > 64 && maxM > 64) {
        dim3 grid((unsigned)big_tiles, splits, nz);
        if constexpr (X6) hipLaunchKernelGGL((k_gemm<A_RC, B_RC, EPI, 2, 1, false, true, 2, 4>), grid, dim3(512), 0, s, g);
        else hipLaunchKernelGGL((k_gemm<A_RC, B_RC, EPI, 2, 2, false>), grid, dim3(256), 0, s, g);
    } else {
        dim3 grid((unsigned)(((maxM + 63) / 64) * ((maxN + 63) / 64)), splits, nz);
        if constexpr (X6) hipLaunchKernelGGL((k_gemm<A_RC, B_RC, EPI, 1, 1, false, true>), grid, dim3(256), 0, s, g);
        else hipLaunchKernelGGL((k_gemm<A_RC, B_RC, EPI, 1, 1, true>), grid, dim3(256), 0, s, g);
    }
}
static bool planes_t_ok(const GemmArgs &g, int nz) {
    if (!g_gemm_x6) return false;
    for (int z = 0; z < nz; ++z)
        if (!g.Bpl[z] || (g.ldb[z] & 7) || (g.N[z] & 7) || g.N[z] < 8 || ((uintptr_t)g.Bpl[z] & 15) || (g.pl_stride & 7)) return false;
    return true;
}
extern "C" void ppok_gemm_fwd(const GemmArgs *g, int nz, hipStream_t s) {
    GemmArgs gp = *g;
    for (int z = 0; z < nz; ++z) {
        if (g->Kpl[z]) gp.K[z] = g->Kpl[z];
        if (g->ldbpl[z]) gp.ldb[z] = g->ldbpl[z];
    }
    if (planes_ok(gp, nz)) launch_gemm_pl<0>(gp, nz, s);
    else if (g_gemm_x6) launch_gemm<true, true, 0, true>(*g, nz, 1, s);
    else launch_gemm<true, true, 0, false>(*g, nz, 1, s);
}
extern "C" void ppok_gemm_dx(const GemmArgs *g, int nz, hipStream_t s) {
    if (planes_t_ok(*g, nz)) launch_gemm_pl<1, false, 2>(*g, nz, s);
    else if (g_gemm_x6) launch_gemm<true, false, 1, true>(*g, nz, 1, s);
    else launch_gemm<true, false, 1, false>(*g, nz, 1, s);
}
extern "C" void ppok_gemm_dw(const GemmArgs *g, int nz, int splits, hipStream_t s) {
    if (!g_gemm_x6) {
        GemmArgs gt = *g;
        for (int z = 0; z < nz; ++z) if (g->nstore[z]) gt.N[z] = g->nstore[z];
        launch_gemm<false, false, 2, false>(gt, nz, splits, s);
        return;
    }
    int maxM = 0, maxN = 0;
    for (int z = 0; z < nz; ++z) { maxM = g->M[z] > maxM ? g->M[z] : maxM; maxN = g->N[z] > maxN ? g->N[z] : maxN; }
    const long big_tiles = (long)((maxM + 127) / 128) * ((maxN + 127) / 128);
    if (big_tiles * splits >= 192 && maxN > 64 && maxM > 64) {
        hipLaunchKernelGGL((k_gemm_dw_t<2, 1, 2, 4>), dim3((unsigned)big_tiles, splits, nz), dim3(512), 0, s, *g);
    } else {
        const unsigned tiles = ((maxM + 63) / 64) * ((maxN + 63) / 64);
        hipLaunchKernelGGL((k_gemm_dw_t<1, 1, 2, 2>), dim3(tiles, splits, nz), dim3(256), 0, s, *g);
    }
}

__global__ void k_act_sample(PpoDev P, const float *__restrict__ obs, const float *__restrict__ critic_obs,
                             const float *__restrict__ mu, const float *__restrict__ val, int t, int64_t act_count, int inject) {
    const int i = blockIdx.x * blockDim.x + threadIdx.x;
    const int N = P.N, A = P.A, O = P.O;
    if (t >= 0) {
        const size_t tot = (size_t)N * O, step = (size_t)gridDim.x * blockDim.x;
        for (size_t k = i; k < tot; k += step) P.st_obs[(size_t)t * tot + k] = obs[k];
        if (P.st_critic_obs != P.st_obs) {
            const size_t totc = (size_t)N * P.OC;
            for (size_t k = i; k < totc; k += step) P.st_critic_obs[(size_t)t * totc + k] = critic_obs[k];
        }
    }
    const float *std = P.params + P.off_std;
    if (i < A && t == 0) P.st_sigma[i] = std[i];
    if (i >= N) return;
    float lp = 0.f;
    for (int a = 0; a < A; ++a) {
        float m = mu[(size_t)i * A + a], s = std[a];
        float z = inject ? P.noise[(size_t)i * A + a] : philox_normal(P.seed, (uint32_t)(P.env_offset + i), (uint64_t)act_count, a);
        float act = m + s * z;
        lp += -((act - m) * (act - m)) / (2.0f * s * s) - logf(s) - 0.9189385332046727f;
        P.act_actions[(size_t)i * A + a] = act;
        P.act_mu[(size_t)i * A + a] = m;
        if (t >= 0) {
            P.st_actions[((size_t)t * N + i) * A + a] = act;
            P.st_mu[((size_t)t * N + i) * A + a] = m;
        }
    }
    const float v = val[i];
    P.act_values[i] = v;
    P.act_log_prob[i] = lp;
    if (t >= 0) {
        P.st_values[(size_t)t * N + i] = v;
        P.st_log_prob[(size_t)t * N + i] = lp;
    }
}

__global__ void k_process_step(PpoDev P, const float *__restrict__ rew, const uint8_t *__restrict__ dones,
                               const uint8_t *__restrict__ time_outs, int t) {
    const int i = blockIdx.x * blockDim.x + threadIdx.x;
    if (i >= P.N) return;
    process_step_body(P, rew[i], dones[i] != 0, time_outs && time_outs[i], t, i);
}

__global__ void __launch_bounds__(256) k_gae(PpoDev P, const float *__restrict__ last_values) {
    const int i = blockIdx.x * blockDim.x + threadIdx.x;
    const int N = P.N, T = P.T;
    float s1 = 0.f, s2 = 0.f;
    if (i < N) {
        float adv = 0.f, next_v = last_values[i];
        for (int t = T - 1; t >= 0; --t) {
            const size_t k = (size_t)t * N + i;
            const float nnt = 1.0f - (P.st_dones[k] ? 1.0f : 0.0f);
            const float v = P.st_values[k];
            const float delta = P.st_rewards[k] + nnt * P.gamma * next_v - v;
            adv = delta + nnt * P.gamma * P.lam * adv;
            const float ret = adv + v;
            P.st_returns[k] = ret;
            const float a = ret - v;
            P.st_adv[k] = a;
            s1 += a; s2 += a * a;
            next_v = v;
        }
    }
    __shared__ float r1[256], r2[256];
    r1[threadIdx.x] = s1; r2[threadIdx.x] = s2;
    __syncthreads();
    for (int w = 128; w > 0; w >>= 1) {
        if ((int)threadIdx.x < w) { r1[threadIdx.x] += r1[threadIdx.x + w]; r2[threadIdx.x] += r2[threadIdx.x + w]; }
        __syncthreads();
    }
    if (threadIdx.x == 0) {
        acc_add(P, &P.adv_partial[0], r1[0]);
        acc_add(P, &P.adv_partial[1], r2[0]);
        if (blockIdx.x == 0) P.adv_partial[2] = (float)((size_t)N * T);
    }
}
__global__ void k_adv_normalize(PpoDev P) {
    const size_t n = (size_t)P.N * P.T;
    const float cnt = P.adv_partial[2], mean = P.adv_partial[0] / cnt;
    const float var = fmaxf((P.adv_partial[1] - cnt * mean * mean) / fmaxf(cnt - 1.0f, 1.0f), 0.f);
    const float inv = 1.0f / (sqrtf(var) + 1e-8f);
    for (size_t k = blockIdx.x * (size_t)blockDim.x + threadIdx.x; k < n; k += (size_t)gridDim.x * blockDim.x)
        P.st_adv[k] = (P.st_adv[k] - mean) * inv;
    if (blockIdx.x == 0 && threadIdx.x == 0) { P.stats[6] = mean; P.stats[7] = sqrtf(var); }
}

__global__ void __launch_bounds__(256) k_randperm(PpoDev P, int n, int half_bits, uint64_t update_idx) {
    const int i = blockIdx.x * 256 + threadIdx.x;
    if (i >= n) return;
    const uint32_t mask = (1u << half_bits) - 1u;
    uint32_t x = (uint32_t)i;
    do {
        uint32_t l = x >> half_bits, r = x & mask;
#pragma unroll 1
        for (int round = 0; round < 6; ++round) {
            uint32_t c[4] = {r, (uint32_t)round, (uint32_t)update_idx, (uint32_t)(update_idx >> 32) ^ 0x9e3779b9u};
            philox4x32((uint32_t)P.seed, (uint32_t)(P.seed >> 32), c);
            const uint32_t t = l ^ (c[0] & mask);
            l = r; r = t;
        }
        x = (l << half_bits) | r;
    } while (x >= (uint32_t)n);
    P.perm[i] = (int32_t)x;
}

__global__ void k_gather(PpoDev P, int mb) {
    const int R = P.mb_rows, A = P.A, O = P.O;
    const int r = blockIdx.x;
    if (r >= R) return;
    const int src = P.perm[(size_t)mb * R + r];
    for (int k = threadIdx.x; k < O; k += blockDim.x) P.mb_obs[(size_t)r * P.Op + k] = P.st_obs[(size_t)src * O + k];
    if (P.st_critic_obs != P.st_obs)
        for (int k = threadIdx.x; k < P.OC; k += blockDim.x) P.mb_critic_obs[(size_t)r * P.OCp + k] = P.st_critic_obs[(size_t)src * P.OC + k];
    if ((int)threadIdx.x < A) {
        P.mb_actions[(size_t)r * A + threadIdx.x] = P.st_actions[(size_t)src * A + threadIdx.x];
        P.mb_mu[(size_t)r * A + threadIdx.x] = P.st_mu[(size_t)src * A + threadIdx.x];
    }
    if (threadIdx.x == 0) {
        P.mb_scalars[(size_t)r * 4 + 0] = P.st_values[src];
        P.mb_scalars[(size_t)r * 4 + 1] = P.st_returns[src];
        P.mb_scalars[(size_t)r * 4 + 2] = P.st_adv[src];
        P.mb_scalars[(size_t)r * 4 + 3] = P.st_log_prob[src];
    }
}

__device__ __forceinline__ void gather4_block(const PpoDev &P, int mb, int vblock) {
    const int R = P.mb_rows, A4 = P.A / 4;
    const int gid = vblock * 256 + threadIdx.x;
    const int r = gid >> 5, j = gid & 31;
    if (r >= R) return;
    const int src = P.perm[(size_t)mb * R + r];
    const bool own_critic = P.st_critic_obs != P.st_obs;
    const int O4 = (P.O & 3) ? 0 : P.O / 4, OC4 = (own_critic && !(P.OC & 3)) ? P.OC / 4 : 0;
    auto row_copy = [&](const float *__restrict__ from, float *__restrict__ to, int n) {
        for (int k0 = j; k0 < n; k0 += 256) {
            float v[8];
#pragma unroll
            for (int u = 0; u < 8; ++u) v[u] = from[min(k0 + 32 * u, n - 1)];
#pragma unroll
            for (int u = 0; u < 8; ++u)
                if (k0 + 32 * u < n) to[k0 + 32 * u] = v[u];
        }
    };
    if (P.O & 3) row_copy(P.st_obs + (size_t)src * P.O, P.mb_obs + (size_t)r * P.Op, P.O);
    if (own_critic && (P.OC & 3)) row_copy(P.st_critic_obs + (size_t)src * P.OC, P.mb_critic_obs + (size_t)r * P.OCp, P.OC);
    for (int k = j; k < O4 + OC4 + 2 * A4 + 1; k += 32) {
        if (k < O4) reinterpret_cast<float4 *>(P.mb_obs)[(size_t)r * (P.Op / 4) + k] = reinterpret_cast<const float4 *>(P.st_obs)[(size_t)src * O4 + k];
        else if (k < O4 + OC4) reinterpret_cast<float4 *>(P.mb_critic_obs)[(size_t)r * (P.OCp / 4) + (k - O4)] = reinterpret_cast<const float4 *>(P.st_critic_obs)[(size_t)src * OC4 + (k - O4)];
        else if (k < O4 + OC4 + A4) reinterpret_cast<float4 *>(P.mb_actions)[(size_t)r * A4 + (k - O4 - OC4)] = reinterpret_cast<const float4 *>(P.st_actions)[(size_t)src * A4 + (k - O4 - OC4)];
        else if (k < O4 + OC4 + 2 * A4) reinterpret_cast<float4 *>(P.mb_mu)[(size_t)r * A4 + (k - O4 - OC4 - A4)] = reinterpret_cast<const float4 *>(P.st_mu)[(size_t)src * A4 + (k - O4 - OC4 - A4)];
        else reinterpret_cast<float4 *>(P.mb_scalars)[r] = make_float4(P.st_values[src], P.st_returns[src], P.st_adv[src], P.st_log_prob[src]);
    }
}
__global__ void __launch_bounds__(256) k_gather4(PpoDev P, int mb) { gather4_block(P, mb, blockIdx.x); }

__global__ void __launch_bounds__(256) k_loss(PpoDev P, const float *__restrict__ mu_new, const float *__restrict__ v_new,
                                              float *__restrict__ dmu, float *__restrict__ dval) {
    const int R = P.mb_rows, A = P.A;
    const int r = blockIdx.x * blockDim.x + threadIdx.x;
    const float *std = P.params + P.off_std;
    const float invR = 1.0f / (float)R;
    constexpr int MA = LG_PPO_MAX_A;
    float part[2 * MA + 4];
#pragma unroll
    for (int k = 0; k < 2 * MA + 4; ++k) part[k] = 0.f;
    __shared__ float s_logs[MA], s_logr[MA];
    if ((int)threadIdx.x < A) {
        const float s = std[threadIdx.x], so = P.st_sigma[threadIdx.x];
        s_logs[threadIdx.x] = logf(s);
        s_logr[threadIdx.x] = logf(s / so + 1.e-5f);
    }
    __syncthreads();
    if (r < R) {
        const float4 sc = reinterpret_cast<const float4 *>(P.mb_scalars)[r];
        const float v_old = sc.x, ret = sc.y, adv = sc.z, lp_old = sc.w;
        float lp = 0.f, kl = 0.f, dd[MA];
#pragma unroll
        for (int a = 0; a < MA; ++a) {
            dd[a] = 0.f;
            if (a < A) {
                const float s = std[a], so = P.st_sigma[a];
                const float m = mu_new[(size_t)r * A + a], mo = P.mb_mu[(size_t)r * A + a];
                const float d = P.mb_actions[(size_t)r * A + a] - m;
                dd[a] = d;
                lp += -(d * d) / (2.0f * s * s) - s_logs[a] - 0.9189385332046727f;
                kl += s_logr[a] + (so * so + (mo - m) * (mo - m)) / (2.0f * s * s) - 0.5f;
            }
        }
        const float ratio = expf(lp - lp_old);
        const float rc = fminf(fmaxf(ratio, 1.0f - P.clip), 1.0f + P.clip);
        const float s1 = -adv * ratio, s2 = -adv * rc;
        const float dl_dlp = (s1 >= s2 ? -adv : 0.0f) * ratio * invR;
#pragma unroll
        for (int a = 0; a < MA; ++a)
            if (a < A) {
                const float s = std[a], d = dd[a];
                const float g = dl_dlp * d / (s * s);
                dmu[(size_t)r * A + a] = g;
                part[MA + a] = g;
                part[a] = dl_dlp * (d * d / (s * s * s) - 1.0f / s) - P.entropy_coef * invR / s;
            }
        const float v = v_new[r];
        float lv, dv;
        if (P.clipped_value) {
            const float dvv = v - v_old;
            const float vc = v_old + fminf(fmaxf(dvv, -P.clip), P.clip);
            const float l1 = (v - ret) * (v - ret), l2 = (vc - ret) * (vc - ret);
            const float inside = (dvv >= -P.clip && dvv <= P.clip) ? 1.0f : 0.0f;
            lv = fmaxf(l1, l2);
            if (l1 > l2) dv = 2.0f * (v - ret);
            else if (l1 < l2) dv = 2.0f * (vc - ret) * inside;
            else dv = (v - ret) + (vc - ret) * inside;
        } else {
            lv = (ret - v) * (ret - v);
            dv = 2.0f * (v - ret);
        }
        dv *= P.value_coef * invR;
        dval[r] = dv;
        part[2 * MA] = dv;
        part[2 * MA + 1] = kl;
        part[2 * MA + 2] = lv;
        part[2 * MA + 3] = fmaxf(s1, s2);
    }
    __shared__ float red[4][2 * MA + 4];
#pragma unroll
    for (int k = 0; k < 2 * MA + 4; ++k) {
        if (k >= 2 * MA || (k % MA) < A) {
            float v = part[k];
#pragma unroll
            for (int m = 32; m > 0; m >>= 1) v += __shfl_xor(v, m);
            if ((threadIdx.x & 63) == 0) red[threadIdx.x >> 6][k] = v;
        }
    }
    __syncthreads();
    const int k = threadIdx.x;
    if (k < 2 * MA + 4 && (k >= 2 * MA || (k % MA) < A)) {
        const float v = ((red[0][k] + red[1][k]) + red[2][k]) + red[3][k];
        if (k < MA) acc_add(P, &P.grads[P.off_std + k], v);
        else if (k < 2 * MA) acc_add(P, &P.grads[P.off_bias_actor_head + (k - MA)], v);
        else if (k == 2 * MA) acc_add(P, &P.grads[P.off_bias_critic_head], v);
        else if (k == 2 * MA + 1) acc_add(P, &P.grads[P.num_params], v);
        else if (k == 2 * MA + 2) acc_add(P, &P.loss_acc[0], v);
        else acc_add(P, &P.loss_acc[1], v);
    }
}

#define HEAD_ROWS 64
#define HEAD_GRID 192
#define HEAD_NET_GRID 384
#define HEAD_PART_STRIDE(H3) ((LG_PPO_MAX_A + 1) * (H3) + 2 * LG_PPO_MAX_A + 4)
template <int H3>
__global__ void __launch_bounds__(256) k_head_fused(PpoDev P, const float *__restrict__ xa_g, const float *__restrict__ xc_g,
                                                    float *__restrict__ dza_g, float *__restrict__ dzc_g, int64_t w_a, int64_t b_a,
                                                    int64_t w_c, int64_t b_c, int64_t b_prev_a, int64_t b_prev_c) {
    constexpr int MA = LG_PPO_MAX_A, LDX = H3 + 1, NH = 256 / H3;
    const int R = P.mb_rows, A = P.A, tid = threadIdx.x;
    __shared__ float xa[HEAD_ROWS * LDX], xc[HEAD_ROWS * LDX];
    __shared__ float wa[MA * H3], wc[H3];
    __shared__ float mus[HEAD_ROWS][MA + 1], dmus[HEAD_ROWS][MA + 1];
    __shared__ float red[2 * MA + 4], s_so2[MA], s_i2s2[MA], s_is2[MA], s_is[MA], s_lgs[MA], s_klc[MA];
    if (tid < MA) {
        const float sg = tid < A ? P.params[P.off_std + tid] : 1.f, so = tid < A ? P.st_sigma[tid] : 1.f;
        s_so2[tid] = so * so; s_i2s2[tid] = 1.0f / (2.0f * sg * sg); s_is2[tid] = 1.0f / (sg * sg); s_is[tid] = 1.0f / sg;
        s_lgs[tid] = logf(sg) + 0.9189385332046727f; s_klc[tid] = logf(sg / so + 1.e-5f) - 0.5f;
    }
    for (int i = tid; i < A * H3; i += 256) wa[i] = P.params[w_a + i];
    for (int i = tid; i < H3; i += 256) wc[i] = P.params[w_c + i];
    if (tid < 2 * MA + 4) red[tid] = 0.f;
    const int c = tid % H3, half = tid / H3;
    float dwa[MA], dwc = 0.f, dba = 0.f, dbc = 0.f, part[2 * MA + 4];
#pragma unroll
    for (int a = 0; a < MA; ++a) dwa[a] = 0.f;
#pragma unroll
    for (int k = 0; k < 2 * MA + 4; ++k) part[k] = 0.f;
    const int ntiles = (R + HEAD_ROWS - 1) / HEAD_ROWS;
    for (int tile = blockIdx.x; tile < ntiles; tile += gridDim.x) {
        const int r0 = tile * HEAD_ROWS;
        __syncthreads();
        {
            constexpr int NV = HEAD_ROWS * H3 / 4 / 256;
            float4 va[NV], vc[NV];
#pragma unroll
            for (int v = 0; v < NV; ++v) {
                const int i = tid + v * 256, r = i / (H3 / 4), c4 = i % (H3 / 4);
                const size_t row = (size_t)min(r0 + r, R - 1);
                va[v] = *reinterpret_cast<const float4 *>(xa_g + row * H3 + 4 * c4);
                vc[v] = *reinterpret_cast<const float4 *>(xc_g + row * H3 + 4 * c4);
            }
            __builtin_amdgcn_sched_barrier(0);
#pragma unroll
            for (int v = 0; v < NV; ++v) {
                const int i = tid + v * 256, r = i / (H3 / 4), c4 = i % (H3 / 4);
                float *da = xa + r * LDX + 4 * c4, *dc = xc + r * LDX + 4 * c4;
                da[0] = va[v].x; da[1] = va[v].y; da[2] = va[v].z; da[3] = va[v].w;
                dc[0] = vc[v].x; dc[1] = vc[v].y; dc[2] = vc[v].z; dc[3] = vc[v].w;
            }
        }
        __syncthreads();
        {
            const int r = tid & 63, w = tid >> 6;
            const float *x = xa + r * LDX;
            float o0 = 0.f, o1 = 0.f, o2 = 0.f, o3 = 0.f;
            const float *w0 = wa + (w < A ? w : 0) * H3, *w1 = wa + (w + 4 < A ? w + 4 : 0) * H3;
            const float *w2 = wa + (w + 8 < A ? w + 8 : 0) * H3, *w3 = wa + (w + 12 < A ? w + 12 : 0) * H3;
#pragma unroll 8
            for (int k = 0; k < H3; ++k) {
                const float xv = x[k];
                o0 += xv * w0[k]; o1 += xv * w1[k]; o2 += xv * w2[k]; o3 += xv * w3[k];
            }
            if (w < A) mus[r][w] = o0 + P.params[b_a + w];
            if (w + 4 < A) mus[r][w + 4] = o1 + P.params[b_a + w + 4];
            if (w + 8 < A) mus[r][w + 8] = o2 + P.params[b_a + w + 8];
            if (w + 12 < A) mus[r][w + 12] = o3 + P.params[b_a + w + 12];
            if (w == 3) {
                float sacc = P.params[b_c];
                const float *y = xc + r * LDX;
#pragma unroll 8
                for (int k = 0; k < H3; ++k) sacc += y[k] * wc[k];
                mus[r][MA] = sacc;
            }
        }
        __syncthreads();
        if (tid < HEAD_ROWS) {
            const int r = r0 + tid;
            const float invR = 1.0f / (float)R;
            float dvl = 0.f;
#pragma unroll
            for (int a = 0; a < MA; ++a) dmus[tid][a] = 0.f;
            const size_t rr = (size_t)min(r, R - 1);
            const float4 sc = reinterpret_cast<const float4 *>(P.mb_scalars)[rr];
            float act_r[MA], mo_r[MA];
#pragma unroll
            for (int a = 0; a < MA; ++a) {
                const int ac = min(a, A - 1);
                act_r[a] = P.mb_actions[rr * A + ac];
                mo_r[a] = P.mb_mu[rr * A + ac];
            }
            if (r < R) {
                const float v_old = sc.x, ret = sc.y, adv = sc.z, lp_old = sc.w;
                float lp = 0.f, kl = 0.f, dd[MA];
#pragma unroll
                for (int a = 0; a < MA; ++a) {
                    dd[a] = 0.f;
                    if (a < A) {
                        const float m = mus[tid][a], mo = mo_r[a];
                        const float d = act_r[a] - m;
                        dd[a] = d;
                        lp += -(d * d) * s_i2s2[a] - s_lgs[a];
                        kl += s_klc[a] + (s_so2[a] + (mo - m) * (mo - m)) * s_i2s2[a];
                    }
                }
                const float ratio = expf(lp - lp_old);
                const float rc = fminf(fmaxf(ratio, 1.0f - P.clip), 1.0f + P.clip);
                const float s1 = -adv * ratio, s2 = -adv * rc;
                const float dl_dlp = (s1 >= s2 ? -adv : 0.0f) * ratio * invR;
#pragma unroll
                for (int a = 0; a < MA; ++a)
                    if (a < A) {
                        const float d = dd[a];
                        const float g = dl_dlp * d * s_is2[a];
                        dmus[tid][a] = g;
                        part[MA + a] += g;
                        part[a] += dl_dlp * (d * d * s_is2[a] * s_is[a] - s_is[a]) - P.entropy_coef * invR * s_is[a];
                    }
                const float v = mus[tid][MA];
                float lv, dv;
                if (P.clipped_value) {
                    const float dvv = v - v_old;
                    const float vc = v_old + fminf(fmaxf(dvv, -P.clip), P.clip);
                    const float l1 = (v - ret) * (v - ret), l2 = (vc - ret) * (vc - ret);
                    const float inside = (dvv >= -P.clip && dvv <= P.clip) ? 1.0f : 0.0f;
                    lv = fmaxf(l1, l2);
                    if (l1 > l2) dv = 2.0f * (v - ret);
                    else if (l1 < l2) dv = 2.0f * (vc - ret) * inside;
                    else dv = (v - ret) + (vc - ret) * inside;
                } else {
                    lv = (ret - v) * (ret - v);
                    dv = 2.0f * (v - ret);
                }
                dvl = dv * P.value_coef * invR;
                part[2 * MA] += dvl;
                part[2 * MA + 1] += kl;
                part[2 * MA + 2] += lv;
                part[2 * MA + 3] += fmaxf(s1, s2);
            }
            dmus[tid][MA] = dvl;
        }
        __syncthreads();
        if (half < NH) {
            float wcol[MA];
#pragma unroll
            for (int a = 0; a < MA; ++a) wcol[a] = a < A ? wa[a * H3 + c] : 0.f;
            const float wcc = wc[c];
            for (int r = half; r < HEAD_ROWS && r0 + r < R; r += NH) {
                float g = 0.f;
                const float x = xa[r * LDX + c], y = xc[r * LDX + c];
#pragma unroll
                for (int a = 0; a < MA; ++a) {
                    const float dm = dmus[r][a];
                    g += dm * wcol[a];
                    dwa[a] += dm * x;
                }
                const float dz = g * (x > 0.f ? 1.0f : x + 1.0f);
                const float dv = dmus[r][MA];
                const float dzc = dv * wcc * (y > 0.f ? 1.0f : y + 1.0f);
                dza_g[(size_t)(r0 + r) * H3 + c] = dz;
                dzc_g[(size_t)(r0 + r) * H3 + c] = dzc;
                dwc += dv * y;
                dba += dz;
                dbc += dzc;
            }
        }
    }
    __shared__ float ptmp[(2 * MA + 4) * HEAD_ROWS];
    if (tid < HEAD_ROWS) {
#pragma unroll
        for (int k = 0; k < 2 * MA + 4; ++k) ptmp[k * HEAD_ROWS + tid] = part[k];
    }
    __syncthreads();
    if (tid < 2 * MA + 4 && (tid >= 2 * MA || (tid % MA) < A)) {
        const int k = tid;
        float v = 0.f;
        for (int r = 0; r < HEAD_ROWS; ++r) v += ptmp[k * HEAD_ROWS + r];
        if (k < MA) acc_add(P, &P.grads[P.off_std + k], v);
        else if (k < 2 * MA) acc_add(P, &P.grads[b_a + (k - MA)], v);
        else if (k == 2 * MA) acc_add(P, &P.grads[b_c], v);
        else if (k == 2 * MA + 1) acc_add(P, &P.grads[P.num_params], v);
        else if (k == 2 * MA + 2) acc_add(P, &P.loss_acc[0], v);
        else acc_add(P, &P.loss_acc[1], v);
    }
    float *acc = xa;
    __syncthreads();
    if (half < NH) {
#pragma unroll
        for (int a = 0; a < MA; ++a) acc[(a * NH + half) * H3 + c] = dwa[a];
        acc[((MA + 0) * NH + half) * H3 + c] = dwc;
        acc[((MA + 1) * NH + half) * H3 + c] = dba;
        acc[((MA + 2) * NH + half) * H3 + c] = dbc;
    }
    __syncthreads();
    for (int i = tid; i < (MA + 3) * H3; i += 256) {
        const int q = i / H3, cc = i % H3;
        float v = 0.f;
        for (int h = 0; h < NH; ++h) v += acc[(q * NH + h) * H3 + cc];
        if (q < MA) { if (q < A) acc_add(P, &P.grads[w_a + (int64_t)q * H3 + cc], v); }
        else if (q == MA) acc_add(P, &P.grads[w_c + cc], v);
        else if (q == MA + 1) acc_add(P, &P.grads[b_prev_a + cc], v);
        else acc_add(P, &P.grads[b_prev_c + cc], v);
    }
}

template <int H3, int NA>
__global__ void __launch_bounds__(256, 3) k_head_net(PpoDev P, const float *__restrict__ xa_g, const float *__restrict__ xc_g,
                                                     float *__restrict__ dza_g, float *__restrict__ dzc_g, const float *__restrict__ wa_g,
                                                     const float *__restrict__ wc_g, int64_t b_a, int64_t b_c) {
    static_assert(H3 == 128, "lane = columns (lane, lane + 64); wave = a quarter of k");
    static_assert(NA <= LG_PPO_MAX_A, "NA = the action count the register arrays are sized for (>= P.A); the scratch row keeps LG_PPO_MAX_A slots");
    constexpr int MA = LG_PPO_MAX_A, LDX = H3 + 1, NWV = 4, KQ = H3 / NWV;
    const int R = P.mb_rows, A = P.A, tid = threadIdx.x, lane = tid & 63;
    const int wv = __builtin_amdgcn_readfirstlane(tid >> 6);
    const bool actor = blockIdx.y == 0;
    const float *__restrict__ x_g = actor ? xa_g : xc_g;
    const float *__restrict__ w_g = actor ? wa_g : wc_g;
    float *__restrict__ dz_g = actor ? dza_g : dzc_g;
    const int nout = actor ? A : 1;
    constexpr int OP = NA + 1, NBUF = HEAD_ROWS * LDX + NWV * HEAD_ROWS * OP;
    __shared__ float buf[NBUF];
    __shared__ float s_am[2 * HEAD_ROWS * NA];
    __shared__ float s_so2[MA], s_i2s2[MA], s_is2[MA], s_is[MA], s_lgs[MA], s_klc[MA], s_bias[MA];
    float *x = buf, *outs_p = buf + HEAD_ROWS * LDX;
    if (tid < MA) {
        const float sg = tid < A ? P.params[P.off_std + tid] : 1.f, so = tid < A ? P.st_sigma[tid] : 1.f;
        s_so2[tid] = so * so; s_i2s2[tid] = 1.0f / (2.0f * sg * sg); s_is2[tid] = 1.0f / (sg * sg); s_is[tid] = 1.0f / sg;
        s_lgs[tid] = logf(sg) + 0.9189385332046727f; s_klc[tid] = logf(sg / so + 1.e-5f) - 0.5f;
        s_bias[tid] = tid < nout ? P.params[(actor ? b_a : b_c) + tid] : 0.f;
    }
    float wcol0[NA], wcol1[NA];
#pragma unroll
    for (int a = 0; a < NA; ++a) {
        wcol0[a] = a < nout ? w_g[a * H3 + lane] : 0.f;
        wcol1[a] = a < nout ? w_g[a * H3 + lane + 64] : 0.f;
    }
    float dw0[NA], dw1[NA], db0 = 0.f, db1 = 0.f, part[2 * MA + 4];
#pragma unroll
    for (int a = 0; a < NA; ++a) { dw0[a] = 0.f; dw1[a] = 0.f; }
#pragma unroll
    for (int k = 0; k < 2 * MA + 4; ++k) part[k] = 0.f;
    const int ntiles = (R + HEAD_ROWS - 1) / HEAD_ROWS;
    const float invR = 1.0f / (float)R;
#ifdef LG_HEAD_STAMPS
    unsigned long long ts[8]; ts[0] = __builtin_amdgcn_s_memrealtime();
#define HSTAMP(k) ts[k] = __builtin_amdgcn_s_memrealtime()
#else
#define HSTAMP(k) do { } while (0)
#endif
    for (int tile = blockIdx.x; tile < ntiles; tile += gridDim.x) {
        const int r0 = tile * HEAD_ROWS;
        const int r = r0 + lane;
        const size_t rr = (size_t)min(r, R - 1);
        const float4 sc = reinterpret_cast<const float4 *>(P.mb_scalars)[rr];
        __syncthreads();
        if (actor) {
            const size_t base = (size_t)r0 * A, lim = (size_t)R * A;
            for (int i = tid; i < HEAD_ROWS * A; i += 256) {
                const size_t g = base + i < lim ? base + i : lim - 1;
                s_am[i] = P.mb_actions[g];
                s_am[HEAD_ROWS * NA + i] = P.mb_mu[g];
            }
        }
        {
            constexpr int NV = HEAD_ROWS * H3 / 4 / 256;
            float4 vx[NV];
#pragma unroll
            for (int v = 0; v < NV; ++v) {
                const int i = tid + v * 256, rw = i / (H3 / 4), c4 = i % (H3 / 4);
                vx[v] = *reinterpret_cast<const float4 *>(x_g + (size_t)min(r0 + rw, R - 1) * H3 + 4 * c4);
            }
            __builtin_amdgcn_sched_barrier(0);
#pragma unroll
            for (int v = 0; v < NV; ++v) {
                const int i = tid + v * 256, rw = i / (H3 / 4), c4 = i % (H3 / 4);
                float *d = x + rw * LDX + 4 * c4;
                d[0] = vx[v].x; d[1] = vx[v].y; d[2] = vx[v].z; d[3] = vx[v].w;
            }
        }
        __syncthreads();
        HSTAMP(1);
        {
            const float *xr = x + lane * LDX + KQ * wv;
            const float *__restrict__ wq = w_g + KQ * wv;
            float xv[KQ];
#pragma unroll
            for (int j = 0; j < KQ; ++j) xv[j] = xr[j];
#pragma unroll
            for (int a = 0; a < NA; ++a)
                if (a < nout) {
                    float o = 0.f;
#pragma unroll
                    for (int j = 0; j < KQ; ++j) o = __builtin_fmaf(xv[j], wq[a * H3 + j], o);
                    outs_p[(wv * HEAD_ROWS + lane) * OP + a] = o;
                }
        }
        __syncthreads();
        HSTAMP(2);
        float dout[NA];
#pragma unroll
        for (int a = 0; a < NA; ++a) dout[a] = 0.f;
        {
            float outv[NA];
#pragma unroll
            for (int a = 0; a < NA; ++a) {
                outv[a] = 0.f;
                if (a < nout) {
                    const float *op = outs_p + lane * OP + a;
                    constexpr int QS = HEAD_ROWS * OP;
                    outv[a] = (op[0] + op[QS]) + (op[2 * QS] + op[3 * QS]);
                }
            }
            const bool sums = wv == 0;
            if (actor) {
                if (r < R) {
                    const float adv = sc.z, lp_old = sc.w;
                    float lp = 0.f, kl = 0.f, dd[NA];
#pragma unroll
                    for (int a = 0; a < NA; ++a) {
                        dd[a] = 0.f;
                        if (a < A) {
                            const float m = outv[a] + s_bias[a], mo = s_am[HEAD_ROWS * NA + lane * A + a];
                            const float d = s_am[lane * A + a] - m;
                            dd[a] = d;
                            lp += -(d * d) * s_i2s2[a] - s_lgs[a];
                            kl += s_klc[a] + (s_so2[a] + (mo - m) * (mo - m)) * s_i2s2[a];
                        }
                    }
                    const float ratio = expf(lp - lp_old);
                    const float rc = fminf(fmaxf(ratio, 1.0f - P.clip), 1.0f + P.clip);
                    const float s1 = -adv * ratio, s2 = -adv * rc;
                    const float dl_dlp = (s1 >= s2 ? -adv : 0.0f) * ratio * invR;
#pragma unroll
                    for (int a = 0; a < NA; ++a)
                        if (a < A) {
                            const float d = dd[a];
                            const float g = dl_dlp * d * s_is2[a];
                            dout[a] = g;
                            if (sums) {
                                part[MA + a] += g;
                                part[a] += dl_dlp * (d * d * s_is2[a] * s_is[a] - s_is[a]) - P.entropy_coef * invR * s_is[a];
                            }
                        }
                    if (sums) { part[2 * MA + 1] += kl; part[2 * MA + 3] += fmaxf(s1, s2); }
                }
            } else if (r < R) {
                const float v_old = sc.x, ret = sc.y;
                const float v = s_bias[0] + outv[0];
                float lv, dv;
                if (P.clipped_value) {
                    const float dvv = v - v_old;
                    const float vc = v_old + fminf(fmaxf(dvv, -P.clip), P.clip);
                    const float l1 = (v - ret) * (v - ret), l2 = (vc - ret) * (vc - ret);
                    const float inside = (dvv >= -P.clip && dvv <= P.clip) ? 1.0f : 0.0f;
                    lv = fmaxf(l1, l2);
                    if (l1 > l2) dv = 2.0f * (v - ret);
                    else if (l1 < l2) dv = 2.0f * (vc - ret) * inside;
                    else dv = (v - ret) + (vc - ret) * inside;
                } else {
                    lv = (ret - v) * (ret - v);
                    dv = 2.0f * (v - ret);
                }
                const float dvl = dv * P.value_coef * invR;
                dout[0] = dvl;
                if (sums) { part[2 * MA] += dvl; part[2 * MA + 2] += lv; }
            }
        }
        HSTAMP(3);
        auto backward = [&](auto full) {
            for (int rw = wv; rw < HEAD_ROWS && r0 + rw < R; rw += NWV) {
                const float xv0 = x[rw * LDX + lane], xv1 = x[rw * LDX + lane + 64];
                float g0 = 0.f, g1 = 0.f;
#pragma unroll
                for (int a = 0; a < NA; ++a)
                    if (decltype(full)::value || a < nout) {
                        const float sa = __builtin_bit_cast(float, __builtin_amdgcn_readlane(__builtin_bit_cast(int, dout[a]), rw));
                        g0 = __builtin_fmaf(sa, wcol0[a], g0); g1 = __builtin_fmaf(sa, wcol1[a], g1);
                        dw0[a] = __builtin_fmaf(sa, xv0, dw0[a]); dw1[a] = __builtin_fmaf(sa, xv1, dw1[a]);
                    }
                const float dz0 = g0 * (xv0 > 0.f ? 1.0f : xv0 + 1.0f), dz1 = g1 * (xv1 > 0.f ? 1.0f : xv1 + 1.0f);
                float *dzr = dz_g + (size_t)(r0 + rw) * H3;
                dzr[lane] = dz0; dzr[lane + 64] = dz1;
                db0 += dz0; db1 += dz1;
            }
        };
        if (nout == NA) backward(std::true_type{}); else backward(std::false_type{});
        HSTAMP(4);
    }
    float *acc = buf, *ptmp = buf + (MA + 1) * NWV * H3;
    static_assert((MA + 1) * NWV * H3 + (2 * MA + 4) * HEAD_ROWS <= NBUF, "sums fit in the tile buffer");
    __syncthreads();
#pragma unroll
    for (int a = 0; a < MA; ++a) {
        acc[(a * NWV + wv) * H3 + lane] = a < NA ? dw0[a < NA ? a : 0] : 0.f;
        acc[(a * NWV + wv) * H3 + lane + 64] = a < NA ? dw1[a < NA ? a : 0] : 0.f;
    }
    acc[(MA * NWV + wv) * H3 + lane] = db0;
    acc[(MA * NWV + wv) * H3 + lane + 64] = db1;
    if (tid < HEAD_ROWS) {
#pragma unroll
        for (int k = 0; k < 2 * MA + 4; ++k) ptmp[k * HEAD_ROWS + tid] = part[k];
    }
    float *__restrict__ prow = P.head_part + ((size_t)blockIdx.y * gridDim.x + blockIdx.x) * HEAD_PART_STRIDE(H3);
    __syncthreads();
    if (tid < 2 * MA + 4) {
        float v = 0.f;
        for (int rw = 0; rw < HEAD_ROWS; ++rw) v += ptmp[tid * HEAD_ROWS + rw];
        prow[(MA + 1) * H3 + tid] = v;
    }
    for (int i = tid; i < (MA + 1) * H3; i += 256) {
        const int q = i / H3, cc = i % H3;
        const float *ap = acc + q * NWV * H3 + cc;
        prow[i] = (ap[0] + ap[H3]) + (ap[2 * H3] + ap[3 * H3]);
    }
#ifdef LG_HEAD_STAMPS
    HSTAMP(5);
    if (tid == 0 && (blockIdx.x % 97) == 0)
        printf("head wg %d net %d: stage %llu fwd %llu loss %llu bwd %llu sums %llu (x10 ns) start %llu\n", blockIdx.x, blockIdx.y, ts[1] - ts[0], ts[2] - ts[1],
               ts[3] - ts[2], ts[4] - ts[3], ts[5] - ts[4], ts[0] % 100000ull);
#endif
}

#define HEAD_FIN_CHUNKS 16
template <int H3>
__global__ void __launch_bounds__(256) k_head_finish(PpoDev P, int nrows, int64_t w_a, int64_t b_a, int64_t w_c, int64_t b_c, int64_t b_prev_a,
                                                     int64_t b_prev_c) {
    constexpr int MA = LG_PPO_MAX_A, NW = (MA + 1) * H3, NTOT = NW + 2 * MA + 4;
    const int i = blockIdx.x * 256 + threadIdx.x, A = P.A;
    if (i >= NTOT) return;
    const bool actor = blockIdx.z == 0;
    const int nout = actor ? A : 1;
    if (i < NW) { if (i / H3 < MA && i / H3 >= nout) return; }
    else {
        const int k = i - NW;
        const bool used = actor ? ((k < MA && k < A) || (k >= MA && k < 2 * MA && k - MA < A) || k == 2 * MA + 1 || k == 2 * MA + 3)
                                : (k == 2 * MA || k == 2 * MA + 2);
        if (!used) return;
    }
    const int r0 = (int)((long)nrows * blockIdx.y / HEAD_FIN_CHUNKS), r1 = (int)((long)nrows * (blockIdx.y + 1) / HEAD_FIN_CHUNKS);
    const float *__restrict__ src = P.head_part + ((size_t)blockIdx.z * nrows + r0) * HEAD_PART_STRIDE(H3) + i;
    float v = 0.f;
#pragma unroll 8
    for (int r = r0; r < r1; ++r, src += HEAD_PART_STRIDE(H3)) v += *src;
    if (i < NW) {
        const int q = i / H3, cc = i % H3;
        if (q < MA) acc_add(P, &P.grads[(actor ? w_a : w_c) + (int64_t)q * H3 + cc], v);
        else acc_add(P, &P.grads[(actor ? b_prev_a : b_prev_c) + cc], v);
    } else {
        const int k = i - NW;
        if (actor) {
            if (k < MA) acc_add(P, &P.grads[P.off_std + k], v);
            else if (k < 2 * MA) acc_add(P, &P.grads[b_a + (k - MA)], v);
            else if (k == 2 * MA + 1) acc_add(P, &P.grads[P.num_params], v);
            else acc_add(P, &P.loss_acc[1], v);
        } else {
            if (k == 2 * MA) acc_add(P, &P.grads[b_c], v);
            else acc_add(P, &P.loss_acc[0], v);
        }
    }
}

__global__ void __launch_bounds__(256) k_opt_prepare(PpoDev P, int par, int prep_blocks, PpoDev G, int gather_mb) {
    if ((int)blockIdx.x >= prep_blocks) { gather4_block(G, gather_mb, (int)blockIdx.x - prep_blocks); return; }
    if (blockIdx.x == 0 && threadIdx.x == 0) {
        const float kl = P.grads[P.num_params] / ((float)P.mb_rows * (float)P.world);
        float lr = P.stats[0];
        if (P.adaptive) {
            if (kl > P.desired_kl * 2.0f) lr = fmaxf(1e-5f, lr / 1.5f);
            else if (kl < P.desired_kl / 2.0f && kl > 0.0f) lr = fminf(1e-2f, lr * 1.5f);
        }
        P.stats[0] = lr;
        P.stats[1] = kl;
        P.stats[2] += P.loss_acc[0] / (float)P.mb_rows;
        P.stats[3] += P.loss_acc[1] / (float)P.mb_rows;
        P.stats[4] += 1.0f;
        P.stats[5] += 1.0f;
        P.loss_acc[0] = 0.f; P.loss_acc[1] = 0.f;
    }
    float s = 0.f;
    const float inv_world = 1.0f / (float)P.world;
    for (int64_t k = blockIdx.x * (int64_t)blockDim.x + threadIdx.x; k < P.num_params; k += (int64_t)prep_blocks * blockDim.x) {
        float g = P.grads[k] * inv_world;
        s += g * g;
    }
    __shared__ float red[256];
    red[threadIdx.x] = s;
    __syncthreads();
    for (int w = 128; w > 0; w >>= 1) {
        if ((int)threadIdx.x < w) red[threadIdx.x] += red[threadIdx.x + w];
        __syncthreads();
    }
    if (threadIdx.x == 0) acc_add(P, &P.loss_acc[2 + par], red[0]);
}
__global__ void __launch_bounds__(256) k_det_fold(PpoDev P) {
    const int64_t n = P.num_params + 10;
    for (int64_t i = blockIdx.x * (int64_t)blockDim.x + threadIdx.x; i < n; i += (int64_t)gridDim.x * blockDim.x) {
        const long long q = P.det64[i];
        if (q == 0) continue;
        float *t = i < P.num_params + 2 ? P.grads + i : i < P.num_params + 6 ? P.loss_acc + (i - P.num_params - 2) : P.adv_partial + (i - P.num_params - 6);
        *t += (float)((double)q * (1.0 / LG_DET_SCALE));
        P.det64[i] = 0;
    }
}
__device__ __forceinline__ void write_planes(const PpoDev &P, int64_t k, float x) {
    const int d = P.pl_dest[k];
    if (d < 0) return;
    uint32_t h, m, l;
    split2(x, 0.f, h, m, l);
    P.wpl[d] = (uint16_t)h; P.wpl[P.pl_stride + d] = (uint16_t)m; P.wpl[2 * P.pl_stride + d] = (uint16_t)l;
}
__global__ void __launch_bounds__(256) k_sync_planes(PpoDev P) {
    for (int64_t k = blockIdx.x * (int64_t)blockDim.x + threadIdx.x; k < P.num_params; k += (int64_t)gridDim.x * blockDim.x)
        write_planes(P, k, P.params[k]);
}
__global__ void __launch_bounds__(256) k_opt_adam(PpoDev P, int par) {
    const float total = sqrtf(P.loss_acc[2 + par]);
    const float coef = fminf(P.max_grad_norm / (total + 1e-6f), 1.0f);
    const float lr = P.stats[0], t = P.stats[4];
    const float bc1 = 1.0f - powf(0.9f, t), bc2 = 1.0f - powf(0.999f, t);
    const float inv_world = 1.0f / (float)P.world;
    for (int64_t k = blockIdx.x * (int64_t)blockDim.x + threadIdx.x; k < P.num_params; k += (int64_t)gridDim.x * blockDim.x) {
        const float g = P.grads[k] * inv_world * coef;
        const float m = 0.9f * P.adam_m[k] + 0.1f * g;
        const float v = 0.999f * P.adam_v[k] + 0.001f * g * g;
        P.adam_m[k] = m;
        P.adam_v[k] = v;
        const float pn = P.params[k] - (lr / bc1) * m / (sqrtf(v) / sqrtf(bc2) + 1e-8f);
        P.params[k] = pn;
        P.grads[k] = 0.f;
        write_planes(P, k, pn);
    }
    if (blockIdx.x == 0 && threadIdx.x == 0) {
        P.grads[P.num_params] = 0.f; P.grads[P.num_params + 1] = 0.f;
        P.loss_acc[2 + (par ^ 1)] = 0.f;
    }
}

extern "C" {
void ppok_act_sample(const PpoDev *P, const float *obs, const float *cobs, const float *mu, const float *val, int t,
                     int64_t cnt, int inject, hipStream_t s) {
    const int blocks = (P->N + 63) / 64;
    hipLaunchKernelGGL(k_act_sample, dim3(blocks > 256 ? blocks : 256), dim3(64), 0, s, *P, obs, cobs, mu, val, t, cnt, inject);
}
void ppok_process_step(const PpoDev *P, const float *rew, const uint8_t *dones, const uint8_t *tos, int t, hipStream_t s) {
    hipLaunchKernelGGL(k_process_step, dim3((P->N + 255) / 256), dim3(256), 0, s, *P, rew, dones, tos, t);
}
void ppok_det_fold(const PpoDev *P, hipStream_t s) { hipLaunchKernelGGL(k_det_fold, dim3(512), dim3(256), 0, s, *P); }
void ppok_gae(const PpoDev *P, const float *last_values, hipStream_t s) {
    (void)hipMemsetAsync(P->adv_partial, 0, 3 * sizeof(float), s);
    hipLaunchKernelGGL(k_gae, dim3((P->N + 255) / 256), dim3(256), 0, s, *P, last_values);
    if (P->det64) ppok_det_fold(P, s);
}
void ppok_adv_normalize(const PpoDev *P, hipStream_t s) {
    hipLaunchKernelGGL(k_adv_normalize, dim3(256), dim3(256), 0, s, *P);
}
void ppok_randperm(const PpoDev *P, int n, uint64_t update_idx, hipStream_t s) {
    int bits = 2;
    while ((1ll << bits) < n) ++bits;
    bits += bits & 1;
    hipLaunchKernelGGL(k_randperm, dim3((n + 255) / 256), dim3(256), 0, s, *P, n, bits / 2, update_idx);
}
void ppok_gather(const PpoDev *P, int mb, hipStream_t s) {
    if ((P->A & 3) == 0)
        hipLaunchKernelGGL(k_gather4, dim3((P->mb_rows * 32 + 255) / 256), dim3(256), 0, s, *P, mb);
    else
        hipLaunchKernelGGL(k_gather, dim3(P->mb_rows), dim3(64), 0, s, *P, mb);
}
size_t ppok_head_part_floats() { return (size_t)2 * HEAD_NET_GRID * HEAD_PART_STRIDE(128); }
int ppok_head_fused(const PpoDev *P, int H3, const float *xa, const float *xc, float *dza, float *dzc, int64_t w_a, int64_t b_a,
                    int64_t w_c, int64_t b_c, int64_t b_prev_a, int64_t b_prev_c, hipStream_t s) {
    const int ntiles = (P->mb_rows + HEAD_ROWS - 1) / HEAD_ROWS;
    dim3 grid(ntiles < HEAD_GRID ? ntiles : HEAD_GRID), block(256);
    if (H3 == 128) {
        const int nrows = ntiles < HEAD_NET_GRID ? ntiles : HEAD_NET_GRID;
        if (P->A <= 12)
            hipLaunchKernelGGL((k_head_net<128, 12>), dim3(nrows, 2), block, 0, s, *P, xa, xc, dza, dzc, P->params + w_a, P->params + w_c, b_a, b_c);
        else
            hipLaunchKernelGGL((k_head_net<128, LG_PPO_MAX_A>), dim3(nrows, 2), block, 0, s, *P, xa, xc, dza, dzc, P->params + w_a, P->params + w_c, b_a, b_c);
        constexpr int NTOT = HEAD_PART_STRIDE(128);
        hipLaunchKernelGGL((k_head_finish<128>), dim3((NTOT + 255) / 256, HEAD_FIN_CHUNKS, 2), block, 0, s, *P, nrows, w_a, b_a, w_c, b_c,
                           b_prev_a, b_prev_c);
    } else if (H3 == 64) hipLaunchKernelGGL((k_head_fused<64>), grid, block, 0, s, *P, xa, xc, dza, dzc, w_a, b_a, w_c, b_c, b_prev_a, b_prev_c);
    else if (H3 == 32) hipLaunchKernelGGL((k_head_fused<32>), grid, block, 0, s, *P, xa, xc, dza, dzc, w_a, b_a, w_c, b_c, b_prev_a, b_prev_c);
    else return -1;
    return 0;
}
void ppok_loss(const PpoDev *P, const float *mu, const float *v, float *dmu, float *dval, hipStream_t s) {
    hipLaunchKernelGGL(k_loss, dim3((P->mb_rows + 255) / 256), dim3(256), 0, s, *P, mu, v, dmu, dval);
}
void ppok_sync_planes(const PpoDev *P, hipStream_t s) { hipLaunchKernelGGL(k_sync_planes, dim3(256), dim3(256), 0, s, *P); }
int ppok_step(const PpoDev *P, int par, const PpoDev *G, int gather_mb, hipStream_t s) {
    const bool g4 = gather_mb >= 0 && (P->A & 3) == 0;
    const int gblocks = g4 ? (P->mb_rows * 32 + 255) / 256 : 0;
    hipLaunchKernelGGL(k_opt_prepare, dim3(128 + gblocks), dim3(256), 0, s, *P, par, 128, g4 ? *G : *P, gather_mb);
    if (P->det64) ppok_det_fold(P, s);
    constexpr int adam_max = 1024;
    const long want = (P->num_params + 255) / 256;
    hipLaunchKernelGGL(k_opt_adam, dim3((unsigned)(want < adam_max ? (want > 0 ? want : 1) : adam_max)), dim3(256), 0, s, *P, par);
    return g4 ? 1 : 0;
}
}

extern "C" void ppok_debug_gemm(const float *A, const float *B, float *C, int M, int N, int K, int mode, int splits, void *stream) {
    GemmArgs g;
    memset(&g, 0, sizeof(g));
    g.A[0] = A; g.B[0] = B; g.C[0] = C; g.M[0] = M; g.N[0] = N; g.K[0] = K; g.ldc[0] = N;
    if (mode == 0) { g.lda[0] = K; g.ldb[0] = K; ppok_gemm_fwd(&g, 1, (hipStream_t)stream); }
    else if (mode == 1) { g.lda[0] = K; g.ldb[0] = N; g.aux[0] = C; g.ldaux[0] = N; g.elu = 1; ppok_gemm_dx(&g, 1, (hipStream_t)stream); }
    else { g.lda[0] = M; g.ldb[0] = N; ppok_gemm_dw(&g, 1, splits, (hipStream_t)stream); }
}

__global__ void __launch_bounds__(256) k_debug_split(const float *__restrict__ W, uint16_t *__restrict__ pl, int64_t n, int64_t stride) {
    for (int64_t k = blockIdx.x * (int64_t)blockDim.x + threadIdx.x; k < n; k += (int64_t)gridDim.x * blockDim.x) {
        uint32_t h, m, l;
        split2(W[k], 0.f, h, m, l);
        pl[k] = (uint16_t)h; pl[stride + k] = (uint16_t)m; pl[2 * stride + k] = (uint16_t)l;
    }
}
extern "C" int ppok_debug_gemm_planes(const float *A, const float *W, float *C, uint16_t *planes, int64_t plane_stride, int M, int rows,
                                      int cols, int mode, void *stream) {
    hipStream_t s = (hipStream_t)stream;
    hipLaunchKernelGGL(k_debug_split, dim3(256), dim3(256), 0, s, W, planes, (int64_t)rows * cols, plane_stride);
    GemmArgs g;
    memset(&g, 0, sizeof(g));
    g.A[0] = A; g.B[0] = W; g.C[0] = C; g.M[0] = M; g.Bpl[0] = planes; g.pl_stride = plane_stride; g.ldb[0] = cols;
    if (mode == 0) {
        g.N[0] = rows; g.K[0] = cols; g.lda[0] = cols; g.ldc[0] = rows;
        if (!planes_ok(g, 1)) return -1;
        launch_gemm_pl<0>(g, 1, s);
    } else {
        g.N[0] = cols; g.K[0] = rows; g.lda[0] = rows; g.ldc[0] = cols; g.aux[0] = C; g.ldaux[0] = cols; g.elu = 0;
        if (!planes_t_ok(g, 1)) return -1;
        launch_gemm_pl<1, false, 2>(g, 1, s);
    }
    return 0;
}
```

Baseline: 7.317 million.

## Store backward layer gradients as split-bf16 planes consumed directly by dW/dX GEMMs

The backward pass now has the fused head kernel and the input-gradient GEMM epilogue write layer gradients (dz) directly as three bf16 planes (hi/mid/lo) instead of fp32. Downstream weight-gradient and input-gradient GEMMs load these planes straight into the split-bf16 mainloop, so they no longer re-split fp32 operands while staging. This removes fp32 dz traffic and per-tile split work. It costs extra plane buffers, new kernel template variants, and error paths that fail when planes cannot be launched.

```diff
diff --git a/legged_gym_dev_amd/csrc/ppo_api.hip b/legged_gym_dev_amd/csrc/ppo_api.hip
--- a/legged_gym_dev_amd/csrc/ppo_api.hip
+++ b/legged_gym_dev_amd/csrc/ppo_api.hip
@@ -11,13 +11,13 @@
 
 extern "C" {
 void ppok_gemm_fwd(const GemmArgs *g, int nz, hipStream_t s);
-void ppok_gemm_dx(const GemmArgs *g, int nz, hipStream_t s);
+int ppok_gemm_dx(const GemmArgs *g, int nz, hipStream_t s);
 void ppok_sync_planes(const PpoDev *P, hipStream_t s);
 int ppok_mlp_fwd(const MlpArgs *g, const PpoDev *P, int mask, hipStream_t s);
 int ppok_mlp_supported(const MlpArgs *g);
 int64_t ppok_mlp_frag_elems(int K, int N);
 void ppok_mlp_frag_build(const MlpArgs *g, hipStream_t s);
-void ppok_gemm_dw(const GemmArgs *g, int nz, int splits, hipStream_t s);
+int ppok_gemm_dw(const GemmArgs *g, int nz, int splits, hipStream_t s);
 void ppok_debug_set_xcd_remap(int v);
 void ppok_act_sample(const PpoDev *P, const float *obs, const float *cobs, const float *mu, const float *val, int t,
                      int64_t cnt, int inject, hipStream_t s);
@@ -31,7 +31,8 @@
 int ppok_step(const PpoDev *P, int par, const PpoDev *G, int gather_mb, hipStream_t s);
 size_t ppok_head_part_floats();
 int ppok_head_fused(const PpoDev *P, int H3, const float *xa, const float *xc, float *dza, float *dzc, int64_t w_a, int64_t b_a,
-                    int64_t w_c, int64_t b_c, int64_t b_prev_a, int64_t b_prev_c, hipStream_t s);
+                    int64_t w_c, int64_t b_c, int64_t b_prev_a, int64_t b_prev_c, uint16_t *dzpa, uint16_t *dzpc, int64_t dzps_a,
+                    int64_t dzps_c, hipStream_t s);
 void ppok_lstm_fwd(const RnnStepArgs *a, int nz, hipStream_t s);
 void ppok_lstm_bwd(const RnnBwdArgs *a, int nz, hipStream_t s);
 void ppok_lstm_bias_grad(const PpoDev *P, const RnnBiasArgs *a, hipStream_t s);
@@ -59,6 +60,8 @@
     int pl_ld0;
     float *act[LG_PPO_MAX_LAYERS + 1];
     float *dz[LG_PPO_MAX_LAYERS + 1];
+    uint16_t *dzpl[LG_PPO_MAX_LAYERS + 1];
+    int64_t dzpl_stride[LG_PPO_MAX_LAYERS + 1];
 };
 
 struct lg_comm;
@@ -102,6 +105,7 @@
     int step, inject;
     int64_t act_count, update_count;
     int Mmax;
+    int dz_is_pl[LG_PPO_MAX_LAYERS + 1];
     std::vector<void *> allocs;
     int64_t perm_count;
     struct MbSet { float *obs, *critic_obs, *actions, *mu, *scalars; } mbset[2];
@@ -180,7 +184,16 @@
     if (rc && !p->comm_rc) p->comm_rc = rc;
 }
 
-static void backward(lg_ppo *p, int M, const float *in0, const float *in1, int skip_head = 0) {
+static bool dz_planes_fit(const lg_ppo *p, int l, bool recurrent) {
+    if (recurrent && l == 1) return false;
+    for (int z = 0; z < 2; ++z) {
+        const Net &n = p->net[z];
+        if (l < 1 || l >= n.nl || (n.dims[l] & 7) || (l > 1 && (n.dims[l - 1] & 7))) return false;
+    }
+    return true;
+}
+
+static int backward(lg_ppo *p, int M, const float *in0, const float *in1, int skip_head = 0) {
     const float *in[2] = {in0, in1};
     auto det_args = [&](GemmArgs &g) {
         g.det_base = p->dev.grads; g.det64 = p->dev.det64; g.det_n = p->dev.num_params + 2;
@@ -202,6 +215,7 @@
                 g.ldb[z] = ldp;
                 if (ldp != n.dims[0]) { g.N[z] = ldp; g.nstore[z] = n.dims[0]; }
             }
+            if (p->dz_is_pl[l + 1]) { g.Apl[z] = n.dzpl[l + 1]; g.apl_stride[z] = n.dzpl_stride[l + 1]; }
             const int tile = (g.M[z] > 64 && g.N[z] > 64) ? 128 : 64;
             long t = (long)((g.M[z] + tile - 1) / tile) * ((g.N[z] + tile - 1) / tile);
             tiles = t > tiles ? t : tiles;
@@ -218,7 +232,7 @@
             (void)hipEventRecord(p->ev_dz, p->stream);
             (void)hipStreamWaitEvent(p->side, p->ev_dz, 0);
         }
-        ppok_gemm_dw(&g, 2, splits, dw_stream);
+        if (ppok_gemm_dw(&g, 2, splits, dw_stream) < 0) { lg_set_error("weight gradient: layer-gradient planes not launchable"); return -100; }
         if (p->comm) reduce_layer_bucket(p, l, dw_stream);
         if (l > 0) {
             memset(&g, 0, sizeof(g));
@@ -229,13 +243,17 @@
                 g.B[z] = p->dev.params + n.w_off[l]; g.ldb[z] = n.dims[l];
                 g.Bpl[z] = p->dev.wpl + n.pl_off[l];
                 g.C[z] = n.dz[l]; g.ldc[z] = n.dims[l];
+                g.Cpl[z] = n.dzpl[l]; g.cpl_stride[z] = n.dzpl_stride[l];
+                if (p->dz_is_pl[l + 1]) { g.Apl[z] = n.dzpl[l + 1]; g.apl_stride[z] = n.dzpl_stride[l + 1]; }
                 g.aux[z] = n.act[l]; g.ldaux[z] = n.dims[l];
                 g.colsum[z] = p->dev.grads + n.b_off[l - 1];
                 g.M[z] = M; g.N[z] = n.dims[l]; g.K[z] = n.dims[l + 1];
             }
             g.elu = p->act_code;
             g.pl_stride = p->dev.pl_stride;
-            ppok_gemm_dx(&g, 2, p->stream);
+            const int rc = ppok_gemm_dx(&g, 2, p->stream);
+            if (rc < 0) { lg_set_error("input gradient: layer-gradient planes not launchable"); return -100; }
+            p->dz_is_pl[l] = rc;
         }
     }
     if (p->rnn.H) {
@@ -268,6 +286,7 @@
         (void)hipStreamWaitEvent(p->stream, lg_comm_event_(p->comm), 0);
         if (rec) { (void)hipEventRecord(p->comm_ev[p->comm_ev_used + 1], p->stream); p->comm_ev_used += 2; }
     }
+    return 0;
 }
 
 static void flush_rollout_epilogue(lg_ppo *p) {
@@ -558,6 +577,15 @@
         Net &n = p->net[z];
         n.act[0] = nullptr; n.dz[0] = nullptr;
         for (int l = 1; l <= n.nl; ++l) { PA(n.act[l], (size_t)p->Mmax * n.dims[l]); PA(n.dz[l], (size_t)p->Mmax * n.dims[l]); }
+    }
+    for (int z = 0; z < 2; ++z) {
+        Net &n = p->net[z];
+        for (int l = 0; l <= n.nl; ++l) { n.dzpl[l] = nullptr; n.dzpl_stride[l] = 0; }
+        for (int l = 1; l < n.nl; ++l)
+            if (dz_planes_fit(p, l, H != 0)) {
+                n.dzpl_stride[l] = (int64_t)p->Mmax * n.dims[l];
+                PA(n.dzpl[l], (size_t)3 * n.dzpl_stride[l]);
+            }
     }
     if (H) {
         Rnn &q = p->rnn;
@@ -805,18 +833,20 @@
         forward(p, R, p->rnn.hout[0], p->rnn.hout[1], 3, fuse ? 1 : 0, true, false);
     } else
         forward(p, R, d.mb_obs, d.mb_critic_obs, 3, fuse ? 1 : 0, true, true);
+    for (int l = 0; l <= LG_PPO_MAX_LAYERS; ++l) p->dz_is_pl[l] = 0;
     if (fuse) {
-        ppok_head_fused(&d, H3, na.act[nl - 1], nc.act[nl - 1], na.dz[nl - 1], nc.dz[nl - 1], na.w_off[nl - 1], na.b_off[nl - 1],
-                        nc.w_off[nl - 1], nc.b_off[nl - 1], na.b_off[nl - 2], nc.b_off[nl - 2], p->stream);
+        const int rc = ppok_head_fused(&d, H3, na.act[nl - 1], nc.act[nl - 1], na.dz[nl - 1], nc.dz[nl - 1], na.w_off[nl - 1],
+                                       na.b_off[nl - 1], nc.w_off[nl - 1], nc.b_off[nl - 1], na.b_off[nl - 2], nc.b_off[nl - 2],
+                                       na.dzpl[nl - 1], nc.dzpl[nl - 1], na.dzpl_stride[nl - 1], nc.dzpl_stride[nl - 1], p->stream);
+        p->dz_is_pl[nl - 1] = rc == 1;
     } else {
         ppok_loss(&d, na.act[na.nl], nc.act[nc.nl], na.dz[na.nl], nc.dz[nc.nl], p->stream);
     }
     if (fuse && p->comm) reduce_layer_bucket(p, nl - 1, p->stream);
     if (p->rnn.H) {
-        backward(p, R, p->rnn.hout[0], p->rnn.hout[1], fuse ? 1 : 0);
+        if (const int rc = backward(p, R, p->rnn.hout[0], p->rnn.hout[1], fuse ? 1 : 0)) return rc;
         rnn_backward_seq(p, mb);
-    } else
-        backward(p, R, d.mb_obs, d.mb_critic_obs, fuse ? 1 : 0);
+    } else if (const int rc = backward(p, R, d.mb_obs, d.mb_critic_obs, fuse ? 1 : 0)) return rc;
     if (d.det64) ppok_det_fold(&d, p->stream);
     if (p->comm_rc) { const int rc = p->comm_rc; p->comm_rc = 0; return rc; }
     return launch_ok();
diff --git a/legged_gym_dev_amd/csrc/ppo_device.h b/legged_gym_dev_amd/csrc/ppo_device.h
--- a/legged_gym_dev_amd/csrc/ppo_device.h
+++ b/legged_gym_dev_amd/csrc/ppo_device.h
@@ -13,6 +13,10 @@
     int64_t pl_stride;
     int Kpl[2], ldbpl[2];
     int nstore[2];
+    const uint16_t *Apl[2];
+    int64_t apl_stride[2];
+    uint16_t *Cpl[2];
+    int64_t cpl_stride[2];
     const float *det_base;
     long long *det64;
     int64_t det_n;
diff --git a/legged_gym_dev_amd/csrc/ppo_kernels.hip b/legged_gym_dev_amd/csrc/ppo_kernels.hip
--- a/legged_gym_dev_amd/csrc/ppo_kernels.hip
+++ b/legged_gym_dev_amd/csrc/ppo_kernels.hip
@@ -315,27 +315,31 @@
     return __builtin_amdgcn_ds_read_tr16_b64_v4i16((s16x4 __attribute__((address_space(3))) *)p);
 }
 
-template <bool A_RC, bool B_RC, int TM, int TN, int WGM, int WGN, bool VEC, bool FULL = false, int B_PL = 0>
+template <bool A_RC, bool B_RC, int TM, int TN, int WGM, int WGN, bool VEC, bool FULL = false, int B_PL = 0, int A_PL = 0>
 __device__ __forceinline__ void gemm_mainloop_x6(const float *__restrict__ A, const float *__restrict__ B, int lda, int ldb, int m0, int n0,
                                                  int M, int N, int k_begin, int k_end, unsigned char *__restrict__ lds, int wm, int wn, int li,
                                                  int lk, f32x16 (&acc)[TM][TN], const uint16_t *__restrict__ Bpl = nullptr,
-                                                 int64_t pl_stride = 0) {
+                                                 int64_t pl_stride = 0, const uint16_t *__restrict__ Apl = nullptr, int64_t apl_stride = 0) {
+    static_assert(A_PL == 0 || A_RC, "A planes: the reduction-contiguous operand");
     constexpr int BM = 32 * TM * WGM, BN = 32 * TN * WGN, NT = 64 * WGM * WGN;
     constexpr int APL = x6_plane_bytes<BM>(), BPL = B_PL == 2 ? plt_plane_bytes<BN>() : x6_plane_bytes<BN>();
     constexpr int NVA = BM * BK / 4 / NT, NVB = BN * BK / 4 / NT;
     constexpr int PD = 2;
     constexpr int NVP = B_PL ? BN * 12 / NT : 1;
-    struct Regs { float4 a[NVA], b[NVB]; uint4 p[NVP]; unsigned ma = 0, mb = 0; };
+    constexpr int NVQ = A_PL ? BM * 12 / NT : 1, NVAF = A_PL ? 1 : NVA;
+    struct Regs { float4 a[NVAF], b[NVB]; uint4 p[NVP], q[NVQ]; unsigned ma = 0, mb = 0; };
     Regs R[PD];
     unsigned char *lds_b = lds + 3 * APL;
     auto load_tile = [&](Regs &r, int k) {
-        stage_load<A_RC, BM, VEC, true, NT, FULL>(A, lda, m0, k, M, k_end, r.a, r.ma);
+        if constexpr (A_PL) stage_load_pl<BM, NT>(Apl, apl_stride, lda, m0, k, M, k_end, r.q, r.ma);
+        else stage_load<A_RC, BM, VEC, true, NT, FULL>(A, lda, m0, k, M, k_end, r.a, r.ma);
         if constexpr (B_PL == 2) stage_load_plt<BN, NT>(Bpl, pl_stride, ldb, n0, k, N, k_end, r.p, r.mb);
         else if constexpr (B_PL == 1) stage_load_pl<BN, NT>(Bpl, pl_stride, ldb, n0, k, N, k_end, r.p, r.mb);
         else stage_load<B_RC, BN, VEC, true, NT, FULL>(B, ldb, n0, k, N, k_end, r.b, r.mb);
     };
     auto store_tile = [&](Regs &r) {
-        stage_store_x6<A_RC, BM, NT, FULL>(lds, r.a, r.ma);
+        if constexpr (A_PL) stage_store_pl<BM, NT>(lds, r.q, r.ma);
+        else stage_store_x6<A_RC, BM, NT, FULL>(lds, r.a, r.ma);
         if constexpr (B_PL == 2) stage_store_plt<BN, NT>(lds_b, r.p, r.mb);
         else if constexpr (B_PL == 1) stage_store_pl<BN, NT>(lds_b, r.p, r.mb);
         else stage_store_x6<B_RC, BN, NT, FULL>(lds_b, r.b, r.mb);
@@ -495,7 +499,84 @@
     }
 }
 
-template <bool A_RC, bool B_RC, int EPI, int TM, int TN, bool DBUF, bool X6 = false, int WGM = 2, int WGN = 2, int B_PL = 0>
+template <int TM, int TN, int BM, int BN, int ACT>
+__device__ __forceinline__ void gemm_epilogue_pl(const GemmArgs &g, int z, int M, int N, int m0, int n0, int wm, int wn, int li, int lk,
+                                                 f32x16 (&acc)[TM][TN]) {
+    uint16_t *__restrict__ P = g.Cpl[z];
+    const int64_t ps = g.cpl_stride[z];
+    const int ldc = g.ldc[z], ldaux = g.ldaux[z];
+    const float *__restrict__ aux = g.aux[z];
+    const bool interior = (m0 + BM <= M) && (n0 + BN <= N);
+    const int elu = g.elu, q = li & 3;
+#pragma unroll
+    for (int b = 0; b < TN; ++b) {
+        const int n = n0 + wn + 32 * b + li, nq = n - q;
+        float csum = 0.f;
+#pragma unroll
+        for (int a = 0; a < TM; ++a) {
+            const int mb = m0 + wm + 32 * a + 4 * lk;
+            float v[16];
+            if (interior) {
+                float ax[16];
+#pragma unroll
+                for (int r = 0; r < 16; ++r) ax[r] = aux[(size_t)(mb + (r & 3) + 8 * (r >> 2)) * ldaux + n];
+#pragma unroll
+                for (int r = 0; r < 16; ++r) {
+                    float x = acc[a][b][r];
+                    x *= (ACT == 1 ? (ax[r] > 0.f ? 1.0f : ax[r] + 1.0f) : ACT == 0 ? 1.0f : act_bwd(elu, ax[r]));
+                    v[r] = x;
+                    csum += x;
+                }
+            } else {
+#pragma unroll
+                for (int r = 0; r < 16; ++r) {
+                    const int m = mb + (r & 3) + 8 * (r >> 2);
+                    v[r] = 0.f;
+                    if (m < M && n < N) {
+                        float x = acc[a][b][r];
+                        const float act = aux[(size_t)m * ldaux + n];
+                        x *= (ACT == 1 ? (act > 0.f ? 1.0f : act + 1.0f) : ACT == 0 ? 1.0f : act_bwd(elu, act));
+                        v[r] = x;
+                        csum += x;
+                    }
+                }
+            }
+#pragma unroll
+            for (int i = 0; i < 4; ++i) {
+                float *e = v + 4 * i;
+                const bool q1 = q & 1, q2 = q & 2;
+#pragma unroll
+                for (int h = 0; h < 2; ++h) {
+                    const float y = quad_xor1(q1 ? e[2 * h] : e[2 * h + 1]);
+                    e[2 * h] = q1 ? y : e[2 * h];
+                    e[2 * h + 1] = q1 ? e[2 * h + 1] : y;
+                }
+#pragma unroll
+                for (int h = 0; h < 2; ++h) {
+                    const float y = quad_xor2(q2 ? e[h] : e[h + 2]);
+                    e[h] = q2 ? y : e[h];
+                    e[h + 2] = q2 ? e[h + 2] : y;
+                }
+                const int m = mb + q + 8 * i;
+                if (interior || (m < M && nq < N)) {
+                    uint32_t h0, m0_, l0, h1, m1_, l1;
+                    split2(e[0], e[1], h0, m0_, l0);
+                    split2(e[2], e[3], h1, m1_, l1);
+                    uint16_t *d = P + (size_t)m * ldc + nq;
+                    *reinterpret_cast<uint2 *>(d) = make_uint2(h0, h1);
+                    *reinterpret_cast<uint2 *>(d + ps) = make_uint2(m0_, m1_);
+                    *reinterpret_cast<uint2 *>(d + 2 * ps) = make_uint2(l0, l1);
+                }
+            }
+        }
+        if (g.colsum[z]) {
+            csum += __shfl_xor(csum, 32);
+            if (lk == 0 && n < N) acc_add(g, &g.colsum[z][n], csum);
+        }
+    }
+}
+
+template <bool A_RC, bool B_RC, int EPI, int TM, int TN, bool DBUF, bool X6 = false, int WGM = 2, int WGN = 2, int B_PL = 0, int A_PL = 0>
 __global__ void __launch_bounds__(64 * WGM * WGN, X6 ? (WGM * WGN == 8 ? 4 : 2) : 1) k_gemm(GemmArgs g) {
     static_assert(B_PL == 0 || (X6 && (B_PL == 1) == B_RC), "weight planes feed the split-bf16 mainloop: [n][k] planes as the reduction-"
                   "contiguous operand (1), the same planes read along their rows through the transposing LDS read (2)");
@@ -542,7 +623,10 @@
 
     if (X6) {
         const bool full = a_vec && b_vec && m0 + BM <= M && n0 + BN <= N && ((k_end - k_begin) % BK) == 0;
-        if (B_PL) {
+        if (A_PL) {
+            static_assert(A_PL == 0 || B_PL, "A planes are taken with B planes only");
+            gemm_mainloop_x6<A_RC, B_RC, TM, TN, WGM, WGN, true, false, B_PL, A_PL>(A, B, lda, ldb, m0, n0, M, N, k_begin, k_end, lds_raw, wm, wn, li, lk, acc, g.Bpl[z], g.pl_stride, g.Apl[z], g.apl_stride[z]);
+        } else if (B_PL) {
             const bool fullp = a_vec && m0 + BM <= M && n0 + BN <= N && ((k_end - k_begin) % BK) == 0;
             if (fullp) gemm_mainloop_x6<A_RC, B_RC, TM, TN, WGM, WGN, true, true, B_PL>(A, B, lda, ldb, m0, n0, M, N, k_begin, k_end, lds_raw, wm, wn, li, lk, acc, g.Bpl[z], g.pl_stride);
             else if (a_vec) gemm_mainloop_x6<A_RC, B_RC, TM, TN, WGM, WGN, true, false, B_PL>(A, B, lda, ldb, m0, n0, M, N, k_begin, k_end, lds_raw, wm, wn, li, lk, acc, g.Bpl[z], g.pl_stride);
@@ -556,6 +640,14 @@
         else gemm_mainloop<A_RC, B_RC, TM, TN, false, DBUF>(A, B, lda, ldb, m0, n0, M, N, k_begin, k_end, lds, wm, wn, li, lk, acc);
     }
 
+    if constexpr (EPI == 1 && X6) {
+        if (g.Cpl[z]) {
+            if (g.elu == 1) gemm_epilogue_pl<TM, TN, BM, BN, 1>(g, z, M, N, m0, n0, wm, wn, li, lk, acc);
+            else if (g.elu == 0) gemm_epilogue_pl<TM, TN, BM, BN, 0>(g, z, M, N, m0, n0, wm, wn, li, lk, acc);
+            else gemm_epilogue_pl<TM, TN, BM, BN, -1>(g, z, M, N, m0, n0, wm, wn, li, lk, acc);
+            return;
+        }
+    }
     if (EPI == 2 || g.elu == 1) gemm_epilogue<EPI, TM, TN, BM, BN, 1>(g, z, M, N, m0, n0, wm, wn, li, lk, ldc, acc);
     else if (g.elu == 0) gemm_epilogue<EPI, TM, TN, BM, BN, 0>(g, z, M, N, m0, n0, wm, wn, li, lk, ldc, acc);
     else gemm_epilogue<EPI, TM, TN, BM, BN, -1>(g, z, M, N, m0, n0, wm, wn, li, lk, ldc, acc);
@@ -580,11 +672,11 @@
     }
 }
 
-template <int TM, int TN, int WGM, int WGN, int PD = 2>
+template <int TM, int TN, int WGM, int WGN, int PD = 2, int A_PL = 0>
 __global__ void __launch_bounds__(64 * WGM * WGN, WGM * WGN == 8 ? 4 : 2) k_gemm_dw_t(GemmArgs g) {
     constexpr int BM = 32 * TM * WGM, BN = 32 * TN * WGN, NT = 64 * WGM * WGN;
     constexpr int APL = plt_plane_bytes<BM>(), BPL = plt_plane_bytes<BN>();
-    constexpr int NVA = BM * BK / 4 / NT, NVB = BN * BK / 4 / NT;
+    constexpr int NVA = A_PL ? 1 : BM * BK / 4 / NT, NVB = BN * BK / 4 / NT, NVQ = A_PL ? BK * BM / 8 * 3 / NT : 1;
     const int z = blockIdx.z;
     const int M = g.M[z], N = g.N[z], K = g.K[z];
     const int tiles_n = (N + BN - 1) / BN, tiles_m = (M + BM - 1) / BM;
@@ -624,29 +716,68 @@
         const s16x8 v = {lo[0], lo[1], lo[2], lo[3], hi[0], hi[1], hi[2], hi[3]};
         return __builtin_bit_cast(bf16x8, v);
     };
-    const bool a_vec = (lda & 3) == 0 && ((uintptr_t)A & 15) == 0 && (M & 3) == 0 && M >= 4;
+    const uint16_t *__restrict__ Apl = g.Apl[z];
+    const int64_t apl_stride = g.apl_stride[z];
+    const bool a_vec = A_PL || ((lda & 3) == 0 && ((uintptr_t)A & 15) == 0 && (M & 3) == 0 && M >= 4);
     const bool b_vec = (ldb & 3) == 0 && ((uintptr_t)B & 15) == 0 && (N & 3) == 0 && N >= 4;
     auto run = [&](auto vec) {
         constexpr bool VEC = decltype(vec)::value;
-        float4 ra[PD][NVA], rb[PD][NVB];
+        typedef std::conditional_t<A_PL != 0, uint4[NVQ], float4[NVA]> ARegs;
+        ARegs ra[PD];
+        float4 rb[PD][NVB];
         unsigned ma[PD], mb[PD];
     #pragma unroll
         for (int d = 0; d < PD; ++d) { ma[d] = 0u; mb[d] = 0u; }
-        auto load = [&](int k0, float4 (&xa)[NVA], float4 (&xb)[NVB], unsigned &xma, unsigned &xmb) {
-            stage_load<false, BM, VEC, false, NT>(A, lda, m0, k0, M, k_end, xa, xma);
+        auto load = [&](int k0, ARegs &xa, float4 (&xb)[NVB], unsigned &xma, unsigned &xmb) {
+            if constexpr (!A_PL) stage_load<false, BM, VEC, false, NT>(A, lda, m0, k0, M, k_end, xa, xma);
             stage_load<false, BN, VEC, false, NT>(B, ldb, n0, k0, N, k_end, xb, xmb);
         };
+        auto load_a = [&](int k0) {
+            if constexpr (A_PL) stage_load_plt<BM, NT>(Apl, apl_stride, lda, m0, k0, M, k_end, ra[0], ma[0]);
+        };
+        auto store_a = [&](ARegs &xa, unsigned xma) {
+            if constexpr (A_PL) stage_store_plt<BM, NT>(lds, xa, xma);
+            else stage_store_x6t<BM, NT>(lds, xa, xma);
+        };
+        load_a(k_begin);
     #pragma unroll
         for (int d = 0; d < PD; ++d)
             if (d == 0 || k_begin + d * BK < k_end) load(k_begin + d * BK, ra[d], rb[d], ma[d], mb[d]);
-        stage_store_x6t<BM, NT>(lds, ra[0], ma[0]);
+        store_a(ra[0], ma[0]);
         stage_store_x6t<BN, NT>(lds_b, rb[0], mb[0]);
+        if (k_begin + BK < k_end) load_a(k_begin + BK);
         lds_barrier();
-        auto body = [&](int k0, float4 (&ca)[NVA], float4 (&cb)[NVB], unsigned &cma, unsigned &cmb, float4 (&na)[NVA], float4 (&nb)[NVB],
+        auto body = [&](int k0, ARegs &ca, float4 (&cb)[NVB], unsigned &cma, unsigned &cmb, ARegs &na, float4 (&nb)[NVB],
                         unsigned &nma, unsigned &nmb) {
             if (k0 + PD * BK < k_end) load(k0 + PD * BK, ca, cb, cma, cmb);
     #pragma unroll
             for (int s = 0; s < BK / 16; ++s) {
+                if constexpr (A_PL) {
+                    bf16x8 bv[TN][3];
+    #pragma unroll
+                    for (int b = 0; b < TN; ++b)
+    #pragma unroll
+                        for (int p = 0; p < 3; ++p) bv[b][p] = frag(fb, PLT_SUB * b + p * BPL + (BN / 32 * PLT_SUB) * 2 * s);
+    #pragma unroll
+                    for (int a = 0; a < TM; ++a) {
+                        bf16x8 x[3];
+    #pragma unroll
+                        for (int p = 0; p < 3; ++p) x[p] = frag(fa, PLT_SUB * a + p * APL + (BM / 32 * PLT_SUB) * 2 * s);
+    #pragma unroll
+                        for (int b = 0; b < TN; ++b) {
+                            const bf16x8 *y = bv[b];
+                            f32x16 c = acc[a][b];
+                            c = __builtin_amdgcn_mfma_f32_32x32x16_bf16(x[1], y[1], c, 0, 0, 0);
+                            c = __builtin_amdgcn_mfma_f32_32x32x16_bf16(x[0], y[2], c, 0, 0, 0);
+                            c = __builtin_amdgcn_mfma_f32_32x32x16_bf16(x[2], y[0], c, 0, 0, 0);
+                            c = __builtin_amdgcn_mfma_f32_32x32x16_bf16(x[0], y[1], c, 0, 0, 0);
+                            c = __builtin_amdgcn_mfma_f32_32x32x16_bf16(x[1], y[0], c, 0, 0, 0);
+                            c = __builtin_amdgcn_mfma_f32_32x32x16_bf16(x[0], y[0], c, 0, 0, 0);
+                            acc[a][b] = c;
+                        }
+                    }
+                    continue;
+                }
                 bf16x8 av[TM][3], bv[TN][3];
     #pragma unroll
                 for (int a = 0; a < TM; ++a)
@@ -673,9 +804,11 @@
             }
             lds_barrier();
             if (k0 + BK < k_end) {
-                stage_store_x6t<BM, NT>(lds, na, nma);
+                if constexpr (A_PL) store_a(ra[0], ma[0]);
+                else store_a(na, nma);
                 stage_store_x6t<BN, NT>(lds_b, nb, nmb);
             }
+            if (A_PL && k0 + 2 * BK < k_end) load_a(k0 + 2 * BK);
             lds_barrier();
         };
         for (int k0 = k_begin; k0 < k_end; k0 += PD * BK) {
@@ -696,7 +829,7 @@
 
 #include "ppo_gemm_glds.h"
 
-template <int EPI, bool B_RC = true, int PL = 1>
+template <int EPI, bool B_RC = true, int PL = 1, int APL = 0>
 static void launch_gemm_pl(const GemmArgs &g, int nz, hipStream_t s) {
     int maxM = 0, maxN = 0;
     for (int z = 0; z < nz; ++z) { maxM = g.M[z] > maxM ? g.M[z] : maxM; maxN = g.N[z] > maxN ? g.N[z] : maxN; }
@@ -710,10 +843,10 @@
     const long big_tiles = (long)((maxM + 127) / 128) * ((maxN + 127) / 128);
     if (big_tiles >= 192 && maxN > 64 && maxM > 64) {
         dim3 grid((unsigned)big_tiles, 1, nz);
-        hipLaunchKernelGGL((k_gemm<true, B_RC, EPI, 2, 1, false, true, 2, 4, PL>), grid, dim3(512), 0, s, g);
+        hipLaunchKernelGGL((k_gemm<true, B_RC, EPI, 2, 1, false, true, 2, 4, PL, APL>), grid, dim3(512), 0, s, g);
     } else {
         dim3 grid((unsigned)(((maxM + 63) / 64) * ((maxN + 63) / 64)), 1, nz);
-        hipLaunchKernelGGL((k_gemm<true, B_RC, EPI, 1, 1, false, true, 2, 2, PL>), grid, dim3(256), 0, s, g);
+        hipLaunchKernelGGL((k_gemm<true, B_RC, EPI, 1, 1, false, true, 2, 2, PL, APL>), grid, dim3(256), 0, s, g);
     }
 }
 static bool planes_ok(const GemmArgs &g, int nz) {
@@ -754,27 +887,58 @@
     else if (g_gemm_x6) launch_gemm<true, true, 0, true>(*g, nz, 1, s);
     else launch_gemm<true, true, 0, false>(*g, nz, 1, s);
 }
-extern "C" void ppok_gemm_dx(const GemmArgs *g, int nz, hipStream_t s) {
-    if (planes_t_ok(*g, nz)) launch_gemm_pl<1, false, 2>(*g, nz, s);
-    else if (g_gemm_x6) launch_gemm<true, false, 1, true>(*g, nz, 1, s);
-    else launch_gemm<true, false, 1, false>(*g, nz, 1, s);
-}
-extern "C" void ppok_gemm_dw(const GemmArgs *g, int nz, int splits, hipStream_t s) {
+static bool pl_img_ok(const void *p, int ld, int width, int64_t stride) {
+    return p && !(ld & 7) && !(width & 7) && width >= 8 && !((uintptr_t)p & 15) && !(stride & 7);
+}
+static bool apl_ok(const GemmArgs &g, int nz) {
+    if (!g_gemm_x6) return false;
+    for (int z = 0; z < nz; ++z) if (!pl_img_ok(g.Apl[z], g.lda[z], g.K[z], g.apl_stride[z])) return false;
+    return true;
+}
+static bool apl_t_ok(const GemmArgs &g, int nz) {
+    if (!g_gemm_x6) return false;
+    for (int z = 0; z < nz; ++z) if (!pl_img_ok(g.Apl[z], g.lda[z], g.M[z], g.apl_stride[z])) return false;
+    return true;
+}
+static bool cpl_ok(const GemmArgs &g, int nz) {
+    if (!g_gemm_x6) return false;
+    for (int z = 0; z < nz; ++z) if (!pl_img_ok(g.Cpl[z], g.ldc[z], g.N[z], g.cpl_stride[z])) return false;
+    return true;
+}
+extern "C" int ppok_gemm_dx(const GemmArgs *g, int nz, hipStream_t s) {
+    GemmArgs gc = *g;
+    const bool cpl = g->Cpl[0] && cpl_ok(*g, nz);
+    if (!cpl) for (int z = 0; z < 2; ++z) gc.Cpl[z] = nullptr;
+    if (g->Apl[0]) {
+        if (!apl_ok(gc, nz) || !planes_t_ok(gc, nz)) return -1;
+        launch_gemm_pl<1, false, 2, 1>(gc, nz, s);
+    } else if (planes_t_ok(gc, nz)) launch_gemm_pl<1, false, 2>(gc, nz, s);
+    else if (g_gemm_x6) launch_gemm<true, false, 1, true>(gc, nz, 1, s);
+    else launch_gemm<true, false, 1, false>(gc, nz, 1, s);
+    return cpl ? 1 : 0;
+}
+extern "C" int ppok_gemm_dw(const GemmArgs *g, int nz, int splits, hipStream_t s) {
+    const bool apl = g->Apl[0] != nullptr;
+    if (apl && !apl_t_ok(*g, nz)) return -1;
     if (!g_gemm_x6) {
         GemmArgs gt = *g;
         for (int z = 0; z < nz; ++z) if (g->nstore[z]) gt.N[z] = g->nstore[z];
         launch_gemm<false, false, 2, false>(gt, nz, splits, s);
-        return;
+        return 0;
     }
     int maxM = 0, maxN = 0;
     for (int z = 0; z < nz; ++z) { maxM = g->M[z] > maxM ? g->M[z] : maxM; maxN = g->N[z] > maxN ? g->N[z] : maxN; }
     const long big_tiles = (long)((maxM + 127) / 128) * ((maxN + 127) / 128);
     if (big_tiles * splits >= 192 && maxN > 64 && maxM > 64) {
-        hipLaunchKernelGGL((k_gemm_dw_t<2, 1, 2, 4>), dim3((unsigned)big_tiles, splits, nz), dim3(512), 0, s, *g);
+        const dim3 grid((unsigned)big_tiles, splits, nz);
+        if (apl) hipLaunchKernelGGL((k_gemm_dw_t<2, 1, 2, 4, 2, 1>), grid, dim3(512), 0, s, *g);
+        else hipLaunchKernelGGL((k_gemm_dw_t<2, 1, 2, 4>), grid, dim3(512), 0, s, *g);
     } else {
-        const unsigned tiles = ((maxM + 63) / 64) * ((maxN + 63) / 64);
-        hipLaunchKernelGGL((k_gemm_dw_t<1, 1, 2, 2>), dim3(tiles, splits, nz), dim3(256), 0, s, *g);
-    }
+        const dim3 grid(((maxM + 63) / 64) * ((maxN + 63) / 64), splits, nz);
+        if (apl) hipLaunchKernelGGL((k_gemm_dw_t<1, 1, 2, 2, 2, 1>), grid, dim3(256), 0, s, *g);
+        else hipLaunchKernelGGL((k_gemm_dw_t<1, 1, 2, 2>), grid, dim3(256), 0, s, *g);
+    }
+    return 0;
 }
 
 __global__ void k_act_sample(PpoDev P, const float *__restrict__ obs, const float *__restrict__ critic_obs,
@@ -1229,10 +1393,11 @@
     }
 }
 
-template <int H3, int NA>
+template <int H3, int NA, bool DZPL = false>
 __global__ void __launch_bounds__(256, 3) k_head_net(PpoDev P, const float *__restrict__ xa_g, const float *__restrict__ xc_g,
                                                      float *__restrict__ dza_g, float *__restrict__ dzc_g, const float *__restrict__ wa_g,
-                                                     const float *__restrict__ wc_g, int64_t b_a, int64_t b_c) {
+                                                     const float *__restrict__ wc_g, int64_t b_a, int64_t b_c, uint16_t *__restrict__ dzpa_g,
+                                                     uint16_t *__restrict__ dzpc_g, int64_t dzps_a, int64_t dzps_c) {
     static_assert(H3 == 128, "lane = columns (lane, lane + 64); wave = a quarter of k");
     static_assert(NA <= LG_PPO_MAX_A, "NA = the action count the register arrays are sized for (>= P.A); the scratch row keeps LG_PPO_MAX_A slots");
     constexpr int MA = LG_PPO_MAX_A, LDX = H3 + 1, NWV = 4, KQ = H3 / NWV;
@@ -1242,6 +1407,8 @@
     const float *__restrict__ x_g = actor ? xa_g : xc_g;
     const float *__restrict__ w_g = actor ? wa_g : wc_g;
     float *__restrict__ dz_g = actor ? dza_g : dzc_g;
+    uint16_t *__restrict__ dzp_g = actor ? dzpa_g : dzpc_g;
+    const int64_t dzps = actor ? dzps_a : dzps_c;
     const int nout = actor ? A : 1;
     constexpr int OP = NA + 1, NBUF = HEAD_ROWS * LDX + NWV * HEAD_ROWS * OP;
     __shared__ float buf[NBUF];
@@ -1404,8 +1571,17 @@
                         dw0[a] = __builtin_fmaf(sa, xv0, dw0[a]); dw1[a] = __builtin_fmaf(sa, xv1, dw1[a]);
                     }
                 const float dz0 = g0 * (xv0 > 0.f ? 1.0f : xv0 + 1.0f), dz1 = g1 * (xv1 > 0.f ? 1.0f : xv1 + 1.0f);
-                float *dzr = dz_g + (size_t)(r0 + rw) * H3;
-                dzr[lane] = dz0; dzr[lane + 64] = dz1;
+                if constexpr (DZPL) {
+                    uint32_t h, m, l;
+                    split2(dz0, dz1, h, m, l);
+                    uint16_t *d = dzp_g + (size_t)(r0 + rw) * H3 + lane;
+                    d[0] = (uint16_t)h; d[64] = (uint16_t)(h >> 16);
+                    d[dzps] = (uint16_t)m; d[dzps + 64] = (uint16_t)(m >> 16);
+                    d[2 * dzps] = (uint16_t)l; d[2 * dzps + 64] = (uint16_t)(l >> 16);
+                } else {
+                    float *dzr = dz_g + (size_t)(r0 + rw) * H3;
+                    dzr[lane] = dz0; dzr[lane + 64] = dz1;
+                }
                 db0 += dz0; db1 += dz1;
             }
         };
@@ -1593,18 +1769,24 @@
 }
 size_t ppok_head_part_floats() { return (size_t)2 * HEAD_NET_GRID * HEAD_PART_STRIDE(128); }
 int ppok_head_fused(const PpoDev *P, int H3, const float *xa, const float *xc, float *dza, float *dzc, int64_t w_a, int64_t b_a,
-                    int64_t w_c, int64_t b_c, int64_t b_prev_a, int64_t b_prev_c, hipStream_t s) {
+                    int64_t w_c, int64_t b_c, int64_t b_prev_a, int64_t b_prev_c, uint16_t *dzpa, uint16_t *dzpc, int64_t dzps_a,
+                    int64_t dzps_c, hipStream_t s) {
     const int ntiles = (P->mb_rows + HEAD_ROWS - 1) / HEAD_ROWS;
     dim3 grid(ntiles < HEAD_GRID ? ntiles : HEAD_GRID), block(256);
     if (H3 == 128) {
         const int nrows = ntiles < HEAD_NET_GRID ? ntiles : HEAD_NET_GRID;
-        if (P->A <= 12)
-            hipLaunchKernelGGL((k_head_net<128, 12>), dim3(nrows, 2), block, 0, s, *P, xa, xc, dza, dzc, P->params + w_a, P->params + w_c, b_a, b_c);
-        else
-            hipLaunchKernelGGL((k_head_net<128, LG_PPO_MAX_A>), dim3(nrows, 2), block, 0, s, *P, xa, xc, dza, dzc, P->params + w_a, P->params + w_c, b_a, b_c);
+        const bool pl = g_gemm_x6 && dzpa && dzpc && !((uintptr_t)dzpa & 15) && !((uintptr_t)dzpc & 15) && !(dzps_a & 7) && !(dzps_c & 7);
+        if (!pl) { dzpa = nullptr; dzpc = nullptr; }
+        const dim3 grid2(nrows, 2);
+        const float *wa = P->params + w_a, *wc = P->params + w_c;
+        if (P->A <= 12 && pl) hipLaunchKernelGGL((k_head_net<128, 12, true>), grid2, block, 0, s, *P, xa, xc, dza, dzc, wa, wc, b_a, b_c, dzpa, dzpc, dzps_a, dzps_c);
+        else if (P->A <= 12) hipLaunchKernelGGL((k_head_net<128, 12>), grid2, block, 0, s, *P, xa, xc, dza, dzc, wa, wc, b_a, b_c, dzpa, dzpc, dzps_a, dzps_c);
+        else if (pl) hipLaunchKernelGGL((k_head_net<128, LG_PPO_MAX_A, true>), grid2, block, 0, s, *P, xa, xc, dza, dzc, wa, wc, b_a, b_c, dzpa, dzpc, dzps_a, dzps_c);
+        else hipLaunchKernelGGL((k_head_net<128, LG_PPO_MAX_A>), grid2, block, 0, s, *P, xa, xc, dza, dzc, wa, wc, b_a, b_c, dzpa, dzpc, dzps_a, dzps_c);
         constexpr int NTOT = HEAD_PART_STRIDE(128);
         hipLaunchKernelGGL((k_head_finish<128>), dim3((NTOT + 255) / 256, HEAD_FIN_CHUNKS, 2), block, 0, s, *P, nrows, w_a, b_a, w_c, b_c,
                            b_prev_a, b_prev_c);
+        return pl ? 1 : 0;
     } else if (H3 == 64) hipLaunchKernelGGL((k_head_fused<64>), grid, block, 0, s, *P, xa, xc, dza, dzc, w_a, b_a, w_c, b_c, b_prev_a, b_prev_c);
     else if (H3 == 32) hipLaunchKernelGGL((k_head_fused<32>), grid, block, 0, s, *P, xa, xc, dza, dzc, w_a, b_a, w_c, b_c, b_prev_a, b_prev_c);
     else return -1;
@@ -1660,3 +1842,28 @@
     }
     return 0;
 }
+
+extern "C" int ppok_debug_gemm_grad_planes(const float *A, const float *B, const float *aux, float *C, float *colsum, uint16_t *apl,
+                                           int64_t astride, uint16_t *wpl, int64_t wstride, uint16_t *cpl, int64_t cstride, long long *det64,
+                                           int M, int N, int K, int mode, int splits, void *stream) {
+    hipStream_t s = (hipStream_t)stream;
+    GemmArgs g;
+    memset(&g, 0, sizeof(g));
+    g.A[0] = A; g.B[0] = B; g.C[0] = C; g.M[0] = M; g.N[0] = N; g.K[0] = K; g.ldc[0] = N; g.ldb[0] = N;
+    if (apl) {
+        hipLaunchKernelGGL(k_debug_split, dim3(256), dim3(256), 0, s, A, apl, (int64_t)M * K, astride);
+        g.Apl[0] = apl; g.apl_stride[0] = astride;
+    }
+    if (mode == 1) {
+        if (!wpl) return -1;
+        hipLaunchKernelGGL(k_debug_split, dim3(256), dim3(256), 0, s, B, wpl, (int64_t)K * N, wstride);
+        g.lda[0] = K; g.Bpl[0] = wpl; g.pl_stride = wstride;
+        g.aux[0] = aux; g.ldaux[0] = N; g.elu = 1; g.colsum[0] = colsum;
+        g.Cpl[0] = cpl; g.cpl_stride[0] = cstride;
+        if (det64) { g.det_base = colsum; g.det64 = det64; g.det_n = N; }
+        return ppok_gemm_dx(&g, 1, s);
+    }
+    g.lda[0] = M;
+    if (det64) { g.det_base = C; g.det64 = det64; g.det_n = (int64_t)M * N; }
+    return ppok_gemm_dw(&g, 1, splits, s) < 0 ? -1 : 0;
+}
```

After: 6.826 million, median of 2. -6.7%, worse.
